# Diamondfan/CTC_pytorch

Measured on AMD Instinct MI355X. Metric: acoustic frames/sec/GPU (train) + utterances/sec beam-decode (`decode` object), TIMIT 4x320 BiLSTM, higher is better.
Workload: dtype f32 via bf16x3 split-operand MFMA (f32 accumulate); 1 GPU; cfg2: 4x320 BiLSTM + BN + Linear(62) + CTC, B=32/GPU, T=800, F=40, dropout 0.1, Adam; global_batch=32, seq_len=800, parallelism=dp1, full_length_utterances=True, sync_bn=False

## Files before the change

### ctc_pytorch_amd/_lib.py

```python
import ctypes
import glob
import os
import subprocess

import torch

_HERE = os.path.dirname(os.path.abspath(__file__))
_CSRC = os.path.join(_HERE, "csrc")
SO_PATH = os.environ.get("CTCN_LIBCTCN") or os.path.join(_HERE, "libctcn.so")
_lib = None

c_void_p, c_int, c_float, c_double, c_size_t, c_u64 = (ctypes.c_void_p, ctypes.c_int, ctypes.c_float,
                                                      ctypes.c_double, ctypes.c_size_t, ctypes.c_uint64)

P, I, F, D, Z, U = c_void_p, c_int, c_float, c_double, c_size_t, c_u64
_SIGS = {
    "ctcn_version": (I, []),
    "ctcn_last_error": (ctypes.c_char_p, []),
    "ctcn_device_cus": (I, []),
    "ctcn_device_xcds": (I, []),
    "ctcn_set_option": (I, [ctypes.c_char_p, I]),
    "ctcn_get_option": (I, [ctypes.c_char_p]),
    "ctcn_option_name": (ctypes.c_char_p, [I]),
    "ctcn_set_status_buffer": (I, [P]),
    "ctcn_gemm": (I, [I, I, I, I, I, P, I, P, I, P, I, F, I, P, Z, P]),
    "ctcn_transpose01": (I, [P, P, I, I, I, P]),
    "ctcn_copy_strided4": (I, [P, P, I, I, I, I, Z, Z, Z, Z, P]),
    "ctcn_relu_fwd": (I, [P, P, Z, P]),
    "ctcn_relu_bwd": (I, [P, P, P, Z, P]),
    "ctcn_maxpool2d_fwd": (I, [P, P, P, Z, I, I, I, I, P]),
    "ctcn_maxpool2d_bwd": (I, [P, P, P, Z, I, I, I, I, P]),
    "ctcn_rnn_scratch_bytes": (Z, [I, I, I, I]),
    "ctcn_rnn_fwd": (I, [I, I, I, I, I, I, P, P, P, P, P, P, P, P, I, P, Z, P]),
    "ctcn_rnn_fwd_dropout": (I, [I, I, I, I, I, I, P, P, P, P, P, P, P, P, P, F, U, U, I, P, Z, P]),
    "ctcn_rnn_bwd": (I, [I, I, I, I, I, I, P, P, P, P, P, P, P, P, P, P, P, P, P, P, F, I, P, P, Z, P]),
    "ctcn_rnn_bwd_dropout": (I, [I, I, I, I, I, I, P, P, P, P, P, P, P, P, P, P, P, P, P, P, F, I, P, P, Z, P, F, U, U, P]),
    "ctcn_rnn_bwd_weights": (I, [I, I, I, I, I, I, P, P, P, P, P, P, P, P, F, I, ctypes.c_uint, P, Z, P]),
    "ctcn_bn_ws_bytes": (Z, [I, I, I]),
    "ctcn_bn_fwd_train": (I, [P, P, P, P, P, P, P, P, I, I, I, F, F, I, P, Z, P, P]),
    "ctcn_bn_fwd_eval": (I, [P, P, P, P, P, P, I, I, I, F, I, P]),
    "ctcn_bn_fwd_sums": (I, [P, P, I, I, I, P, Z, P]),
    "ctcn_bn_fwd_finish": (I, [P, P, P, P, P, P, P, P, P, D, I, I, I, F, F, I, P, P]),
    "ctcn_bn_bwd_sums": (I, [P, P, P, P, P, P, I, I, I, I, P, Z, P]),
    "ctcn_bn_bwd_finish": (I, [P, P, P, P, P, P, P, P, P, P, P, D, I, I, I, I, F, P, Z, P]),
    "ctcn_bn_bwd": (I, [P, P, P, P, P, P, P, P, P, I, I, I, I, F, P, Z, P]),
    "ctcn_bn_fwd_train_dropout": (I, [P, P, P, P, P, P, P, P, I, I, I, F, F, I, P, Z, P, P, F, U, U]),
    "ctcn_bn_bwd_dropout": (I, [P, P, P, P, P, P, P, P, P, I, I, I, I, F, P, Z, P, F, U, U]),
    "ctcn_dropout": (I, [P, P, Z, F, U, U, P]),
    "ctcn_bn_masked_ws_bytes": (Z, [I, I, I]),
    "ctcn_mask_frames": (I, [P, P, P, I, I, I, I, I, P]),
    "ctcn_bn_fwd_train_masked": (I, [P, P, P, P, P, P, P, P, P, I, I, I, I, I, F, F, I, P, Z, P, P]),
    "ctcn_bn_fwd_eval_masked": (I, [P, P, P, P, P, P, P, I, I, I, I, I, F, I, P]),
    "ctcn_bn_bwd_masked": (I, [P, P, P, P, P, P, P, P, P, P, I, I, I, I, I, I, F, P, Z, P]),
    "ctcn_conv2d_ws_bytes": (Z, [I] * 11),
    "ctcn_conv2d_fwd": (I, [P, P, P, P] + [I] * 11 + [P]),
    "ctcn_conv2d_bwd": (I, [P, P, P, P, P, P] + [I] * 11 + [F, P, Z, P]),
    "ctcn_bctf_to_tbcf": (I, [P, P, I, I, I, I, P]),
    "ctcn_tbcf_to_bctf": (I, [P, P, I, I, I, I, P]),
    "ctcn_log_softmax_fwd": (I, [P, P, P, I, I, P]),
    "ctcn_log_softmax_bwd": (I, [P, P, P, I, I, P]),
    "ctcn_argmax": (I, [P, P, I, I, P]),
    "ctcn_rnn_fwd_ex": (I, [I, I, I, I, I, I, P, P, P, P, P, P, P, P, I, P, Z, P, P]),
    "ctcn_rnn_bwd_ex": (I, [I, I, I, I, I, I, P, P, P, P, P, P, P, P, P, P, P, P, P, P, F, I, P, P, Z, P, P]),
    "ctcn_ctc_fwd": (I, [P, P, P, P, P, P, I, I, I, I, P]),
    "ctcn_ctc_bwd": (I, [P, P, P, P, P, P, P, P, I, I, I, I, P]),
    "ctcn_ctc_fwd_both": (I, [P, P, P, P, P, P, P, I, I, I, I, P]),
    "ctcn_ctc_grad": (I, [P, P, P, P, P, P, P, P, P, I, I, I, I, P]),
    "ctcn_sum_f32": (I, [P, P, I, P]),
    "ctcn_ctc_fwd_ex": (I, [P, P, P, P, P, P, P, I, I, I, I, I, P]),
    "ctcn_ctc_grad_ex": (I, [P, P, P, P, P, P, P, P, I, I, I, I, P, I, I, I, I, P]),
    "ctcn_ctc_reduce": (I, [P, P, P, I, I, I, P]),
    "ctcn_ctc_pack_targets": (I, [P, ctypes.c_int64, P, P, I, I, P]),
    "ctcn_ctc_align_ws_bytes": (Z, [I, I, I]),
    "ctcn_ctc_align": (I, [P, P, P, P, P, P, P, P, P, P, I, I, I, I, I, P, Z, P]),
    "ctcn_adam_step": (I, [P, P, P, P, Z, F, F, F, F, F, I, P]),
    "ctcn_grad_norm_ws_bytes": (Z, [Z, I]),
    "ctcn_grad_norm": (I, [P, Z, I, P, I, P, P, P, I, P, Z, P]),
    "ctcn_clip_control": (I, [P, F, F, F, F, I, P]),
    "ctcn_adam_step_ex": (I, [P, P, P, P, Z, F, F, F, F, P, P]),
    "ctcn_scale_by_device_scalar": (I, [P, Z, P, P]),
    "ctcn_greedy_collapse": (I, [P, Z, Z, P, P, P, I, I, I, P]),
    "ctcn_edit_distance": (I, [P, P, P, P, P, I, I, I, I, P]),
    "ctcn_edit_ops_ws_bytes": (Z, [I, I, I]),
    "ctcn_edit_ops": (I, [P, P, P, P, P, I, P, P, P, P, I, I, I, I, P, Z, P]),
    "ctcn_step_stats": (I, [P, P, P, I, P, P, P]),
    "ctcn_comm_unique_id": (I, [P]),
    "ctcn_comm_init": (I, [P, I, I, ctypes.POINTER(ctypes.c_void_p)]),
    "ctcn_comm_allreduce_sum_f32": (I, [P, P, Z, P]),
    "ctcn_comm_destroy": (I, [P]),
    "ctcn_diag_squat": (I, [I, I, I, ctypes.c_uint, P]),
    "ctcn_diag_pipeline_chunks": (I, [I, I, I, I, I, I, I, I, ctypes.c_uint]),
    "ctcn_rnn_last_kernel": (ctypes.c_char_p, [I]),
    "ctcn_levenshtein": (ctypes.c_longlong, [P, ctypes.c_longlong, P, ctypes.c_longlong]),
    "ctcn_levenshtein_ops": (ctypes.c_longlong, [P, ctypes.c_longlong, P, ctypes.c_longlong, P, P]),
    "ctcn_join_tokens": (ctypes.c_longlong, [P, ctypes.c_longlong, P, I, P, P, P, I, I, P, ctypes.c_longlong, P]),
    "ctcn_beam_ws_bytes": (Z, [I, I, I, I]),
    "ctcn_beam_decode": (I, [P, I, P, P, D, I, I, P, P, P, P, I, I, I, P, Z, P]),
    "ctcn_beam_decode_nbest": (I, [P, I, P, P, D, I, I, I, P, P, P, P, P, I, I, I, P, Z, P]),
}


class RnnCall(ctypes.Structure):
    _fields_ = [("drop_p", ctypes.c_float), ("drop_seed", ctypes.c_uint64), ("drop_offset", ctypes.c_uint64), ("y_drop", ctypes.c_void_p),
                ("dy_tmp", ctypes.c_void_p), ("side_stream", ctypes.c_void_p), ("side_event", ctypes.c_void_p), ("side_ws", ctypes.c_void_p),
                ("side_ws_bytes", ctypes.c_size_t), ("xcd_allow", ctypes.c_uint), ("prelaunch_event", ctypes.c_void_p), ("status", ctypes.c_void_p),
                ("launched", ctypes.POINTER(ctypes.c_char_p))]


def sources():
    return sorted(glob.glob(os.path.join(_CSRC, "*.hip")))


def build(force=False, verbose=False):
    from concurrent.futures import ThreadPoolExecutor
    srcs = sources()
    hdrs = glob.glob(os.path.join(_CSRC, "*.h")) + [os.path.join(os.path.dirname(_HERE), "include", "ctcn.h")]
    hipcc = os.environ.get("HIPCC", "/opt/rocm/bin/hipcc")
    objdir = os.path.join(_CSRC, "_obj")
    os.makedirs(objdir, exist_ok=True)
    hdr_time = max(os.path.getmtime(h) for h in hdrs)
    flags = ["--offload-arch=gfx950", "-O3", "-std=c++17", "-fPIC"]
    jobs, objs = [], []
    for src in srcs:
        obj = os.path.join(objdir, os.path.basename(src)[:-4] + ".o")
        objs.append(obj)
        if force or not os.path.exists(obj) or os.path.getmtime(obj) < max(os.path.getmtime(src), hdr_time):
            jobs.append([hipcc] + flags + ["-c", src, "-o", obj])

    def run(cmd):
        if verbose:
            print(" ".join(cmd), flush=True)
        subprocess.check_call(cmd)

    if jobs:
        with ThreadPoolExecutor(max_workers=min(len(jobs), os.cpu_count() or 4)) as pool:
            list(pool.map(run, jobs))
    if jobs or not os.path.exists(SO_PATH) or any(os.path.getmtime(SO_PATH) < os.path.getmtime(o) for o in objs):
        run([hipcc, "--offload-arch=gfx950", "-fPIC", "-shared", "-o", SO_PATH] + objs)
    return SO_PATH


def lib():
    global _lib
    if _lib is None:
        if not os.path.exists(SO_PATH):
            raise RuntimeError(
                "ctc_pytorch_amd: %s is missing -- run `python -c 'import __graft_entry__ as g; g.build()'` "
                "(hipcc --offload-arch=gfx950). There is no CPU fallback." % SO_PATH)
        l = ctypes.CDLL(SO_PATH)
        for name, (res, args) in _SIGS.items():
            fn = getattr(l, name)
            fn.restype = res
            fn.argtypes = args
        _lib = l
        for var, opt in (("CTCN_RNN_PERSISTENT", b"rnn_persistent"), ("CTCN_HANDOFF", b"handoff"), ("CTCN_GEMM_BIG_TILES", b"gemm_big_tiles"), ("CTCN_BWD_SCATTER", b"bwd_scatter"), ("CTCN_HANDOFF_TAGS", b"handoff_tags"), ("CTCN_SIDE_SPLIT_WGS", b"side_split_wgs")):
            env = os.environ.get(var)
            if env is not None:
                l.ctcn_set_option(opt, int(env))
        for var, val in os.environ.items():
# ... 58 lines not shown
```

### ctc_pytorch_amd/csrc/common.h

```cpp
#pragma once
#include <hip/hip_runtime.h>
#include <stdarg.h>
#include <stdint.h>
#include <stdio.h>
#include <string.h>

#include "../../include/ctcn.h"

void ctcn_set_error(const char *fmt, ...);
int *ctcn_status_word(void);
int ctcn_opt_rnn_persistent(void);
int ctcn_transpose01_pair(const float *in0, const float *in1, float *out0, float *out1, int A, int B, int C, void *stream);
struct GemmPlanes {
  const float *A = nullptr; int lda = 0, M = 0, Ka = 0, transA = 0; void *ws_a = nullptr, *st_a = nullptr; bool a_valid = false;
  const float *B = nullptr; int ldb = 0, N = 0, Kb = 0, transB = 0, shift = 0; void *ws_b = nullptr, *st_b = nullptr; const void *bh = nullptr; bool b_valid = false;
  bool same_a = false, same_b = false;
};
int ctcn_gemm_on_xcds(int transA, int transB, int M, int N, int K, const float *A, int lda, const float *B, int ldb, float *C,
                      int ldc, float beta, int precision, void *ws, size_t ws_bytes, void *stream, unsigned xcd_allow, GemmPlanes *planes = nullptr);
int ctcn_gemm_shift_b(int M, int N, int K, const float *A, int lda, const float *B, int ldb, float *C, int ldc, float beta, int precision,
                      void *ws, size_t ws_bytes, void *stream, unsigned xcd_allow, int shift, GemmPlanes *planes = nullptr);
int ctcn_opt_handoff(void);
int ctcn_opt_poll_depth(void);
int ctcn_opt_bwd_scatter(void);
int ctcn_opt_handoff_tags(void);
int ctcn_opt_side_split_wgs(void);
int ctcn_opt_gemm_big_tiles(void);
int ctcn_opt_recurrence_only(void);

#define CTCN_REQUIRE(cond, ...)          \
  do {                                   \
    if (!(cond)) {                       \
      ctcn_set_error(__VA_ARGS__);       \
      return CTCN_EINVAL;                \
    }                                    \
  } while (0)

#define CTCN_HIP(expr)                                                                   \
  do {                                                                                   \
    hipError_t e__ = (expr);                                                             \
    if (e__ != hipSuccess) {                                                             \
      ctcn_set_error("%s:%d: %s -> %s", __FILE__, __LINE__, #expr, hipGetErrorString(e__)); \
      return CTCN_EHIP;                                                                  \
    }                                                                                    \
  } while (0)

#define CTCN_LAUNCH_CHECK() CTCN_HIP(hipGetLastError())

typedef float f32x4 __attribute__((ext_vector_type(4)));
typedef float f32x16 __attribute__((ext_vector_type(16)));
typedef short bf16x8 __attribute__((ext_vector_type(8)));
typedef unsigned int u32x4 __attribute__((ext_vector_type(4)));

static inline int ceil_div(int a, int b) { return (a + b - 1) / b; }
static inline size_t ceil_div_z(size_t a, size_t b) { return (a + b - 1) / b; }
static inline size_t align_up(size_t a, size_t b) { return (a + b - 1) / b * b; }

__device__ __forceinline__ float wave_max(float v) {
#pragma unroll
  for (int o = 32; o > 0; o >>= 1) v = fmaxf(v, __shfl_xor(v, o, 64));
  return v;
}
__device__ __forceinline__ float wave_sum(float v) {
#pragma unroll
  for (int o = 32; o > 0; o >>= 1) v += __shfl_xor(v, o, 64);
  return v;
}
__device__ __forceinline__ double wave_sum_d(double v) {
#pragma unroll
  for (int o = 32; o > 0; o >>= 1) v += __shfl_xor(v, o, 64);
  return v;
}
__device__ __forceinline__ void lds_barrier() { asm volatile("s_waitcnt lgkmcnt(0)\n\ts_barrier" ::: "memory"); }

__device__ __forceinline__ float sigmoidf_(float x) { return 1.0f / (1.0f + expf(-x)); }

__device__ __forceinline__ void philox_round(uint32_t (&c)[4], uint32_t (&k)[2]) {
  const uint32_t M0 = 0xD2511F53u, M1 = 0xCD9E8D57u;
  const uint32_t hi0 = __umulhi(M0, c[0]), lo0 = M0 * c[0];
  const uint32_t hi1 = __umulhi(M1, c[2]), lo1 = M1 * c[2];
  const uint32_t n0 = hi1 ^ c[1] ^ k[0], n1 = lo1, n2 = hi0 ^ c[3] ^ k[1], n3 = lo0;
  c[0] = n0; c[1] = n1; c[2] = n2; c[3] = n3;
  k[0] += 0x9E3779B9u; k[1] += 0xBB67AE85u;
}
__device__ __forceinline__ void philox4(uint64_t seed, uint64_t ctr, uint32_t (&out)[4]) {
  uint32_t c[4] = {(uint32_t)ctr, (uint32_t)(ctr >> 32), 0u, 0u};
  uint32_t k[2] = {(uint32_t)seed, (uint32_t)(seed >> 32)};
#pragma unroll
  for (int i = 0; i < 10; ++i) philox_round(c, k);
#pragma unroll
  for (int i = 0; i < 4; ++i) out[i] = c[i];
}

__device__ __forceinline__ unsigned short f2bf(float f) {
  return __builtin_bit_cast(unsigned short, (__bf16)f);
}
```

### ctc_pytorch_amd/csrc/core.hip

```cpp
#include "common.h"

static thread_local char g_err[512] = "";

void ctcn_set_error(const char *fmt, ...) {
  va_list ap;
  va_start(ap, fmt);
  vsnprintf(g_err, sizeof(g_err), fmt, ap);
  va_end(ap);
}

extern "C" int ctcn_version(void) { return 100; }
extern "C" const char *ctcn_last_error(void) { return g_err; }
extern "C" int ctcn_device_cus(void) {
  int dev = 0, n = 0;
  if (hipGetDevice(&dev) != hipSuccess) return -1;
  if (hipDeviceGetAttribute(&n, hipDeviceAttributeMultiprocessorCount, dev) != hipSuccess) return -1;
  return n;
}

static int g_opt_rnn_persistent = 1;
static int g_opt_handoff = 1;
static int g_opt_poll_depth = 2;
static int g_opt_recurrence_only = 0;
static int g_opt_bwd_scatter = 1;
static int g_opt_handoff_tags = 1;
static int g_opt_side_split_wgs = 8;
static int g_opt_gemm_big_tiles = 0;
static int g_opt_gemm_tile256 = 1;
static int g_opt_gemm_dbg = 0;
static int g_opt_gemm_a_inline = 1;
static int g_opt_conv_mfma = 1;
static int g_opt_gemm_pingpong = 1;
static int g_opt_rnn_mixed_slices = 0;
static int g_opt_rnn_fwd_tagged = 1;
static int g_opt_rnn_fused_dropout = 1;
static int g_opt_gemm_tn = 1;
static int g_opt_tag_poll_delay = 8;
static int g_opt_edit_wave = 1;
static int g_opt_bwd_item_gather = 1;
static int g_opt_bwd_poll_delay = -1;
static int g_opt_fwd_rsv_lds = 2;
static int g_opt_fwd_pipe_any_chunking = 0;
static int g_opt_fwd_pipe_min_input = 0;
static int g_opt_conv_dbg = 0;
static int g_opt_rnn_rsv_nt = 0;
static int g_opt_gemm_bf16_single = 0;
static int g_opt_xcd_interleave = 1;
static int g_opt_bn_rows4 = 1;
static int g_opt_tn_splits_force = 0;
static int g_opt_tn_splits_xcd = 1;
static int g_opt_beam_generic_threads = 0;
static int g_opt_beam_bitonic = 1;
static int g_opt_beam_cand_global = 0;
static int g_opt_beam_occ2 = 0;
static int g_opt_beam_fast = 1;
static int g_opt_rnn_slow_items = 0;
static int g_opt_rnn_slow_exchange = 0;
static int g_opt_xcd_interleave_force = 0;
static int *g_status_dev = nullptr;

struct OptionRow { const char *name; int *var; int (*norm)(int); };
static const OptionRow k_options[] = {
  {"rnn_persistent", &g_opt_rnn_persistent, [](int value) -> int { return value; }},
  {"handoff", &g_opt_handoff, [](int value) -> int { return value; }},
  {"poll_depth", &g_opt_poll_depth, [](int value) -> int { return value; }},
  {"rnn_recurrence_only", &g_opt_recurrence_only, [](int value) -> int { return value ? 1 : 0; }},
  {"bwd_scatter", &g_opt_bwd_scatter, [](int value) -> int { return value ? 1 : 0; }},
  {"handoff_tags", &g_opt_handoff_tags, [](int value) -> int { return value ? 1 : 0; }},
  {"side_split_wgs", &g_opt_side_split_wgs, [](int value) -> int { return value < 1 ? 1 : (value > 16 ? 16 : value); }},
  {"gemm_big_tiles", &g_opt_gemm_big_tiles, [](int value) -> int { return value ? 1 : 0; }},
  {"beam_fast", &g_opt_beam_fast, [](int value) -> int { return value ? 1 : 0; }},
  {"conv_dbg", &g_opt_conv_dbg, [](int value) -> int { return value & 7; }},
  {"rnn_rsv_nt", &g_opt_rnn_rsv_nt, [](int value) -> int { return value ? 1 : 0; }},
  {"tn_splits_xcd", &g_opt_tn_splits_xcd, [](int value) -> int { return value ? 1 : 0; }},
  {"xcd_interleave", &g_opt_xcd_interleave, [](int value) -> int { return value < 0 ? 0 : (value > 5 ? 5 : value); }},
  {"bn_rows4", &g_opt_bn_rows4, [](int value) -> int { return value ? 1 : 0; }},
  {"tn_splits_force", &g_opt_tn_splits_force, [](int value) -> int { return value < 0 ? 0 : value; }},
  {"gemm_bf16_single", &g_opt_gemm_bf16_single, [](int value) -> int { return value ? 1 : 0; }},
  {"beam_generic_threads", &g_opt_beam_generic_threads, [](int value) -> int { return (value == 256 || value == 512 || value == 1024) ? value : 0; }},
  {"beam_cand_global", &g_opt_beam_cand_global, [](int value) -> int { return value ? 1 : 0; }},
  {"beam_bitonic", &g_opt_beam_bitonic, [](int value) -> int { return value ? 1 : 0; }},
  {"beam_occ2", &g_opt_beam_occ2, [](int value) -> int { return value < 0 ? 0 : (value > 2 ? 2 : value); }},
  {"fwd_pipe_min_input", &g_opt_fwd_pipe_min_input, [](int value) -> int { return value < 0 ? 0 : value; }},
  {"fwd_pipe_any_chunking", &g_opt_fwd_pipe_any_chunking, [](int value) -> int { return value ? 1 : 0; }},
  {"fwd_rsv_lds", &g_opt_fwd_rsv_lds, [](int value) -> int { return value < 0 ? 0 : (value > 2 ? 2 : value); }},
  {"bwd_item_gather", &g_opt_bwd_item_gather, [](int value) -> int { return value < 0 ? 0 : (value > 2 ? 2 : value); }},
  {"bwd_poll_delay", &g_opt_bwd_poll_delay, [](int value) -> int { return value < 0 ? -1 : (value > 256 ? 256 : value); }},
  {"conv_mfma", &g_opt_conv_mfma, [](int value) -> int { return value ? 1 : 0; }},
  {"edit_wave", &g_opt_edit_wave, [](int value) -> int { return value ? 1 : 0; }},
  {"gemm_tn", &g_opt_gemm_tn, [](int value) -> int { return value != 0; }},
  {"rnn_fused_dropout", &g_opt_rnn_fused_dropout, [](int value) -> int { return value != 0; }},
  {"tag_poll_delay", &g_opt_tag_poll_delay, [](int value) -> int { return value < 0 ? 0 : (value > 64 ? 64 : value); }},
  {"rnn_fwd_tagged", &g_opt_rnn_fwd_tagged, [](int value) -> int { return value ? 1 : 0; }},
  {"rnn_mixed_slices", &g_opt_rnn_mixed_slices, [](int value) -> int { return value ? 1 : 0; }},
  {"gemm_pingpong", &g_opt_gemm_pingpong, [](int value) -> int { return value ? 1 : 0; }},
  {"gemm_a_inline", &g_opt_gemm_a_inline, [](int value) -> int { return value ? 1 : 0; }},
  {"gemm_dbg", &g_opt_gemm_dbg, [](int value) -> int { return value; }},
  {"gemm_tile256", &g_opt_gemm_tile256, [](int value) -> int { return value ? 1 : 0; }},
  {"xcd_interleave_force", &g_opt_xcd_interleave_force, [](int value) -> int { return value ? 1 : 0; }},
  {"rnn_slow_exchange", &g_opt_rnn_slow_exchange, [](int value) -> int { return value < 0 ? 0 : (value > 4096 ? 4096 : value); }},
  {"rnn_slow_items", &g_opt_rnn_slow_items, [](int value) -> int { return value < 0 ? 0 : (value > 4096 ? 4096 : value); }},
};
static const int k_noptions = (int)(sizeof(k_options) / sizeof(k_options[0]));
static const OptionRow *find_option(const char *name) {
  if (name)
    for (int i = 0; i < k_noptions; ++i)
      if (!strcmp(name, k_options[i].name)) return &k_options[i];
  return nullptr;
}
extern "C" int ctcn_set_option(const char *name, int value) {
  if (const OptionRow *o = find_option(name)) { *o->var = o->norm(value); return CTCN_OK; }
  ctcn_set_error("ctcn_set_option: unknown option %s", name ? name : "(null)");
  return CTCN_EINVAL;
}
extern "C" int ctcn_get_option(const char *name) {
  const OptionRow *o = find_option(name);
  return o ? *o->var : -1;
}
extern "C" const char *ctcn_option_name(int index) { return index >= 0 && index < k_noptions ? k_options[index].name : nullptr; }
extern "C" int ctcn_set_status_buffer(int *dev_word) { g_status_dev = dev_word; return CTCN_OK; }
int *ctcn_status_word(void) { return g_status_dev; }
int ctcn_opt_rnn_persistent(void) { return g_opt_rnn_persistent; }
int ctcn_opt_handoff(void) { return g_opt_handoff; }
int ctcn_opt_poll_depth(void) { return g_opt_poll_depth; }
int ctcn_opt_recurrence_only(void) { return g_opt_recurrence_only; }
int ctcn_opt_bwd_scatter(void) { return g_opt_bwd_scatter; }
int ctcn_opt_handoff_tags(void) { return g_opt_handoff_tags; }
int ctcn_opt_side_split_wgs(void) { return g_opt_side_split_wgs; }
int ctcn_opt_gemm_big_tiles(void) { return g_opt_gemm_big_tiles; }
// ... 1 lines not shown
```

### ctc_pytorch_amd/csrc/gemm.hip

```cpp
#include <algorithm>
#include <type_traits>

#include "common.h"

namespace {

constexpr int BM = 128, BN = 128, BK = 16, PAD = 4;

__device__ __forceinline__ void g2r_kc(const float *__restrict__ src, int ld, int r0, int R, int k0, int Kend,
                                       bool vec, int tid, float (&reg)[8]) {
#pragma unroll
  for (int j = 0; j < 2; ++j) {
    const int idx = tid + 256 * j;
    const int r = idx >> 2, kq = (idx & 3) * 4;
    const int gr = r0 + r, gk = k0 + kq;
    const float *p = src + (size_t)gr * ld + gk;
    if (vec && gr < R && gk + 3 < Kend) {
      const float4 v = *reinterpret_cast<const float4 *>(p);
      reg[4 * j + 0] = v.x; reg[4 * j + 1] = v.y; reg[4 * j + 2] = v.z; reg[4 * j + 3] = v.w;
    } else {
#pragma unroll
      for (int c = 0; c < 4; ++c) reg[4 * j + c] = (gr < R && gk + c < Kend) ? p[c] : 0.0f;
    }
  }
// ... 250 lines not shown
    else x_g2r_mc(B, ldb, n0, N, k0, kend, vecB, tid, rb);
  };
  if (kbeg < kend) { loadA(kbeg); loadB(kbeg); }
  for (int k0 = kbeg; k0 < kend; k0 += XBK) {
    __syncthreads();
    if (TA) x_r2s_mc(sAh, sAl, tid, ra); else x_r2s_kc(sAh, sAl, tid, ra);
    if (TB) x_r2s_kc(sBh, sBl, tid, rb); else x_r2s_mc(sBh, sBl, tid, rb);
    __syncthreads();
    if (k0 + XBK < kend) { loadA(k0 + XBK); loadB(k0 + XBK); }
    const int ml = lane & 31, kg = (lane >> 5) * 8;
#pragma unroll
    for (int ks = 0; ks < XBK; ks += 16) {
      bf16x8_t ah[2], al[2], bh[2], bl[2];
#pragma unroll
      for (int i = 0; i < 2; ++i) {
        ah[i] = *reinterpret_cast<const bf16x8_t *>(&sAh[wm * 64 + i * 32 + ml][ks + kg]);
        al[i] = *reinterpret_cast<const bf16x8_t *>(&sAl[wm * 64 + i * 32 + ml][ks + kg]);
        bh[i] = *reinterpret_cast<const bf16x8_t *>(&sBh[wn * 64 + i * 32 + ml][ks + kg]);
        bl[i] = *reinterpret_cast<const bf16x8_t *>(&sBl[wn * 64 + i * 32 + ml][ks + kg]);
      }
#pragma unroll
      for (int i = 0; i < 2; ++i)
#pragma unroll
        for (int j = 0; j < 2; ++j) {
          acc[i][j] = __builtin_amdgcn_mfma_f32_32x32x16_bf16(al[i], bh[j], acc[i][j], 0, 0, 0);
          acc[i][j] = __builtin_amdgcn_mfma_f32_32x32x16_bf16(ah[i], bl[j], acc[i][j], 0, 0, 0);
          acc[i][j] = __builtin_amdgcn_mfma_f32_32x32x16_bf16(ah[i], bh[j], acc[i][j], 0, 0, 0);
        }
    }
  }
  float *out = ws ? ws + (size_t)blockIdx.y * M * N : C;
  const int ldo = ws ? N : ldc;
#pragma unroll
  for (int i = 0; i < 2; ++i)
#pragma unroll
    for (int j = 0; j < 2; ++j) {
      const int col = n0 + wn * 64 + j * 32 + (lane & 31);
#pragma unroll
      for (int e = 0; e < 16; ++e) {
        const int row = m0 + wm * 64 + i * 32 + (e & 3) + 8 * (e >> 2) + 4 * (lane >> 5);
        if (row < M && col < N) {
          float v = acc[i][j][e];
          float *p = out + (size_t)row * ldo + col;
          if (!ws && beta != 0.0f) v += beta * *p;
          *p = v;
        }
      }
    }
}

constexpr int PBK = 64;

__global__ void split_rows_kernel(const float *__restrict__ src, int ld, int R, int C, int Cp, unsigned short *__restrict__ hi,
                                  unsigned short *__restrict__ lo) {
  const size_t total = (size_t)R * (Cp / 4);
  for (size_t i = blockIdx.x * (size_t)blockDim.x + threadIdx.x; i < total; i += (size_t)gridDim.x * blockDim.x) {
    const int r = (int)(i / (Cp / 4)), c = (int)(i - (size_t)r * (Cp / 4)) * 4;
    unsigned short h[4], l[4];
#pragma unroll
    for (int k = 0; k < 4; ++k) {
      const float v = (c + k < C) ? src[(size_t)r * ld + c + k] : 0.0f;
      split_bf16(v, h[k], l[k]);
    }
    *reinterpret_cast<uint2 *>(hi + (size_t)r * Cp + c) = make_uint2((unsigned)h[0] | ((unsigned)h[1] << 16), (unsigned)h[2] | ((unsigned)h[3] << 16));
    *reinterpret_cast<uint2 *>(lo + (size_t)r * Cp + c) = make_uint2((unsigned)l[0] | ((unsigned)l[1] << 16), (unsigned)l[2] | ((unsigned)l[3] << 16));
  }
}

__device__ __forceinline__ void split_transpose_tile(float (*t)[65], int bx, int by, const float *__restrict__ src, int ld, int R, int C, int Rp,
                                                     unsigned short *__restrict__ hi, unsigned short *__restrict__ lo, int shift) {
  const int r0 = by * 64, c0 = bx * 64;
  const int tid = threadIdx.x;
  const bool vec = c0 + 64 <= C && (ld & 3) == 0 && ((uintptr_t)src & 15) == 0;
  if (vec) {
#pragma unroll
    for (int j = 0; j < 4; ++j) {
      const int idx = tid + 256 * j, i = idx >> 4, c4 = idx & 15;
      const int r = r0 + i - shift;
      float4 v = make_float4(0.f, 0.f, 0.f, 0.f);
      if (r >= 0 && r < R && r0 + i < R) v = *reinterpret_cast<const float4 *>(src + (size_t)r * ld + c0 + 4 * c4);
      t[i][4 * c4 + 0] = v.x; t[i][4 * c4 + 1] = v.y; t[i][4 * c4 + 2] = v.z; t[i][4 * c4 + 3] = v.w;
    }
    __syncthreads();
#pragma unroll
    for (int j = 0; j < 2; ++j) {
      const int g = tid + 256 * j, c = g >> 3, ro = g & 7;
      unsigned hw[4], lw[4];
#pragma unroll
      for (int e = 0; e < 4; ++e) {
        unsigned short h0, l0, h1, l1;
        split_bf16(t[ro * 8 + 2 * e][c], h0, l0);
        split_bf16(t[ro * 8 + 2 * e + 1][c], h1, l1);
        hw[e] = (unsigned)h0 | ((unsigned)h1 << 16);
        lw[e] = (unsigned)l0 | ((unsigned)l1 << 16);
      }
      const size_t o = (size_t)(c0 + c) * Rp + r0 + ro * 8;
      *reinterpret_cast<uint4 *>(hi + o) = make_uint4(hw[0], hw[1], hw[2], hw[3]);
      *reinterpret_cast<uint4 *>(lo + o) = make_uint4(lw[0], lw[1], lw[2], lw[3]);
    }
    return;
  }
  const int tx = tid & 63, ty = tid >> 6;
  for (int i = ty; i < 64; i += 4) {
    const int r = r0 + i - shift, c = c0 + tx;
    t[i][tx] = (r >= 0 && r < R && r0 + i < R && c < C) ? src[(size_t)r * ld + c] : 0.0f;
  }
  __syncthreads();
  for (int i = ty; i < 64; i += 4) {
    const int c = c0 + i, r = r0 + tx;
    if (c < C && r < Rp) {
      unsigned short h, l;
      split_bf16(t[tx][i], h, l);
      hi[(size_t)c * Rp + r] = h;
      lo[(size_t)c * Rp + r] = l;
    }
  }
}

__global__ __launch_bounds__(256) void split_transpose_kernel(const float *__restrict__ src, int ld, int R, int C, int Rp,
                                                              unsigned short *__restrict__ hi, unsigned short *__restrict__ lo, int shift) {
  __shared__ float t[64][65];
  split_transpose_tile(t, blockIdx.x, blockIdx.y, src, ld, R, C, Rp, hi, lo, shift);
}
__global__ __launch_bounds__(256) void split_transpose_queue_kernel(const float *__restrict__ src, int ld, int R, int C, int Rp,
                                                                    unsigned short *__restrict__ hi, unsigned short *__restrict__ lo, int tiles_x,
                                                                    int tiles_y, unsigned xcd_allow, unsigned *__restrict__ queue, int shift) {
  __shared__ float t[64][65];
  __shared__ int s_item;
  unsigned x;
  asm volatile("s_getreg_b32 %0, hwreg(HW_REG_XCC_ID)" : "=s"(x));
  if (!((xcd_allow >> (x & 15)) & 1u)) return;
  for (;;) {
    if (threadIdx.x == 0) s_item = (int)atomicAdd(queue, 1u);
    __syncthreads();
    const int item = s_item;
    if (item >= tiles_x * tiles_y) return;
    split_transpose_tile(t, item % tiles_x, item / tiles_x, src, ld, R, C, Rp, hi, lo, shift);
    __syncthreads();
  }
}

__device__ __forceinline__ int pswz(int row, int kc) { return row * 128 + ((kc ^ ((row >> 1) & 7)) << 4); }

template <int TI, int TJ>
__device__ __forceinline__ void plane_tile(unsigned char *sm, int bid, int split, int M, int N, int Kp,
                                           const unsigned short *__restrict__ Ah, const unsigned short *__restrict__ Al,
                                           const unsigned short *__restrict__ Bh, const unsigned short *__restrict__ Bl,
                                           float *__restrict__ C, int ldc, float beta, int kchunk, float *__restrict__ ws, int tiles_n) {
  constexpr int TBM = 64 * TI, TBN = 64 * TJ;
  constexpr int CA = TBM * 8 / 256, CB = TBN * 8 / 256;
  unsigned char *sAh = sm, *sAl = sm + TBM * 128, *sBh = sm + 2 * TBM * 128, *sBl = sBh + TBN * 128;
  const int tid = threadIdx.x, lane = tid & 63, wave = tid >> 6;
  const int wm = wave >> 1, wn = wave & 1;
  const int tm = bid / tiles_n, tn = bid - tm * tiles_n;
  const int m0 = tm * TBM, n0 = tn * TBN;
  const int kbeg = split * kchunk;
  const int kend = min(Kp, kbeg + kchunk);

  f32x16 acc[TI][TJ];
#pragma unroll
  for (int i = 0; i < TI; ++i)
#pragma unroll
    for (int j = 0; j < TJ; ++j)
#pragma unroll
      for (int e = 0; e < 16; ++e) acc[i][j][e] = 0.0f;

  unsigned offA[CA], offB[CB];
#pragma unroll
  for (int j = 0; j < CA; ++j) offA[j] = (unsigned)min(m0 + ((tid + 256 * j) >> 3), M - 1) * (unsigned)Kp + ((tid + 256 * j) & 7) * 8;
#pragma unroll
  for (int j = 0; j < CB; ++j) offB[j] = (unsigned)min(n0 + ((tid + 256 * j) >> 3), N - 1) * (unsigned)Kp + ((tid + 256 * j) & 7) * 8;
  u32x4 pAh[CA], pAl[CA], pBh[CB], pBl[CB];
  auto gload = [&](int k0) {
#pragma unroll
    for (int j = 0; j < CA; ++j) {
      pAh[j] = *reinterpret_cast<const u32x4 *>(Ah + offA[j] + k0);
      pAl[j] = *reinterpret_cast<const u32x4 *>(Al + offA[j] + k0);
    }
#pragma unroll
    for (int j = 0; j < CB; ++j) {
      pBh[j] = *reinterpret_cast<const u32x4 *>(Bh + offB[j] + k0);
      pBl[j] = *reinterpret_cast<const u32x4 *>(Bl + offB[j] + k0);
    }
  };
  if (kbeg < kend) gload(kbeg);
  for (int k0 = kbeg; k0 < kend; k0 += PBK) {
    __syncthreads();
#pragma unroll
    for (int j = 0; j < CA; ++j) {
      const int so = pswz((tid + 256 * j) >> 3, (tid + 256 * j) & 7);
// ... 1145 lines not shown
        for (int u = 0; u < 8; ++u) { s.x += v[u].x; s.y += v[u].y; s.z += v[u].z; s.w += v[u].w; }
      }
      for (; z < splits; ++z) { const float4 v = w4[(size_t)z * total4 + i]; s.x += v.x; s.y += v.y; s.z += v.z; s.w += v.w; }
      const unsigned m = i / n4, n = (i - m * n4) << 2;
      float4 *p = reinterpret_cast<float4 *>(C + (size_t)m * ldc + n);
      if (beta != 0.0f) { const float4 o = *p; s.x += beta * o.x; s.y += beta * o.y; s.z += beta * o.z; s.w += beta * o.w; }
      *p = s;
    }
    return;
  }
  for (size_t i = blockIdx.x * (size_t)blockDim.x + threadIdx.x; i < total; i += (size_t)gridDim.x * blockDim.x) {
    float s = 0.0f;
    int z = 0;
    for (; z + 8 <= splits; z += 8) {
      float v[8];
#pragma unroll
      for (int u = 0; u < 8; ++u) v[u] = ws[(size_t)(z + u) * total + i];
#pragma unroll
      for (int u = 0; u < 8; ++u) s += v[u];
    }
    for (; z < splits; ++z) s += ws[(size_t)z * total + i];
    const size_t m = i / N, n = i - m * N;
    float *p = C + m * ldc + n;
    if (beta != 0.0f) s += beta * *p;
    *p = s;
  }
}

__global__ void transpose01_kernel(const float *__restrict__ in, float *__restrict__ out, int A, int B, int C) {
  const size_t total = (size_t)A * B * C;
  for (size_t i = blockIdx.x * (size_t)blockDim.x + threadIdx.x; i < total; i += (size_t)gridDim.x * blockDim.x) {
    const int c = i % C;
    const size_t ab = i / C;
    const int a = ab % A;
    const int b = ab / A;
    out[i] = in[((size_t)a * B + b) * C + c];
  }
}

}

static bool tn_eligible(int transA, int transB, int M, int N, int K, const float *A, int lda, const float *B, int ldb, int precision, const void *ws,
                        size_t ws_bytes) {
  return precision == 1 && transA && !transB && ws && ws_bytes >= 1024 && ctcn_get_option("gemm_tn") != 0 && M >= 128 && N >= 32 && K >= 1024 &&
         M % 4 == 0 && N % 4 == 0 && lda % 4 == 0 && ldb % 4 == 0 && ((uintptr_t)A & 15) == 0 && ((uintptr_t)B & 15) == 0 &&
         lda < (1 << 24) && ldb < (1 << 24);
}
static int gemm_core(int transA, int transB, int M, int N, int K, const float *A, int lda, const float *B, int ldb, float *C,
                     int ldc, float beta, int precision, void *ws, size_t ws_bytes, void *stream, unsigned xcd_allow, GemmPlanes *planes, int b_shift) {
  GemmPlanes scratch_planes;
  GemmPlanes &pl = planes ? *planes : scratch_planes;
  const bool want_same_a = pl.same_a, want_same_b = pl.same_b;
  pl.same_a = pl.same_b = false;
  CTCN_REQUIRE(precision == 0 || precision == 1, "ctcn_gemm: precision %d (0 = f32 MFMA, 1 = bf16x3 split MFMA)", precision);
  CTCN_REQUIRE(M > 0 && N > 0 && K >= 0, "ctcn_gemm: bad dims M=%d N=%d K=%d", M, N, K);
  CTCN_REQUIRE(A && B && C, "ctcn_gemm: null pointer");
  CTCN_REQUIRE(lda >= (transA ? M : K) && ldb >= (transB ? K : N) && ldc >= N, "ctcn_gemm: leading dim too small");
  CTCN_REQUIRE(!ws || (uintptr_t)ws % 16 == 0, "ctcn_gemm: the workspace must be 16-byte aligned");
  hipStream_t st = (hipStream_t)stream;
  const int tiles_m = ceil_div(M, BM), tiles_n = ceil_div(N, BN);
  const int nt = tiles_m * tiles_n;
  int splits = 1;
  if (nt < 256 && K >= 512 && ws && ws_bytes >= (size_t)2 * M * N * sizeof(float)) {
    splits = ceil_div(512, nt);
    splits = min(splits, K / 256);
    splits = min(splits, (int)(ws_bytes / ((size_t)M * N * sizeof(float))));
    if (splits < 2) splits = 1;
  }
  int kchunk = K;
  if (splits > 1) {
    kchunk = ceil_div(ceil_div(K, splits), XBK) * XBK;
    splits = ceil_div(K, kchunk);
  }
  if (tn_eligible(transA, transB, M, N, K, A, lda, B, ldb, precision, ws, ws_bytes) && b_shift == 0) {
    pl.a_valid = false; pl.b_valid = false;
    const int wnt = ceil_div(N, 256) * 256 == ceil_div(N, 128) * 128 ? 2 : 1;
    unsigned *queue = (unsigned *)((char *)ws + ((ws_bytes - 256) & ~(size_t)255));
    int tn_cus = 256;
    if (xcd_allow && ctcn_get_option("tn_splits_xcd") != 0) {
      const int nx = std::max(1, std::min(ctcn_device_xcds(), 16));
      tn_cus = std::max(ctcn_device_cus() / nx * __builtin_popcount(xcd_allow & ((1u << nx) - 1u)), 32);
    }
    const int tsplits = tn_splits(M, N, K, wnt, ws_bytes - 512, tn_cus);
    return wnt == 2 ? launch_tn<2>(st, M, N, K, A, lda, B, ldb, C, ldc, beta, tsplits, (float *)ws, xcd_allow, queue)
                    : launch_tn<1>(st, M, N, K, A, lda, B, ldb, C, ldc, beta, tsplits, (float *)ws, xcd_allow, queue);
  }
  if (precision == 1 && K >= 64 && ws) {
    const int Kp = ceil_div(K, PBK) * PBK;
    const size_t a_el = (size_t)M * Kp, b_el = (size_t)N * Kp;
    const size_t plane_bytes = align_up(2 * (a_el + b_el) * sizeof(unsigned short), 256);
    if (ws_bytes >= plane_bytes + 1024) {
      unsigned short *ah = (unsigned short *)ws, *al = ah + a_el, *bh = al + a_el, *bl = bh + b_el;
      float *part = (float *)((char *)ws + plane_bytes);
      unsigned *queue = (unsigned *)((char *)ws + ((ws_bytes - 256) & ~(size_t)255));
      const size_t part_bytes = ws_bytes - plane_bytes - 512;
      if (xcd_allow) CTCN_HIP(hipMemsetAsync(queue, 0, 16, st));
      int nq = 0;
      auto split = [&](const float *src, int ld, bool contraction_major, int rows, unsigned short *hi, unsigned short *lo, int shift) {
        if (!contraction_major) {
          const size_t total = (size_t)rows * (Kp / 4);
          hipLaunchKernelGGL(split_rows_kernel, dim3((unsigned)std::min((size_t)8192, ceil_div_z(total, 256))), dim3(256), 0, st, src, ld, rows, K, Kp, hi, lo);
        } else {
          if (xcd_allow)
            hipLaunchKernelGGL(split_transpose_queue_kernel, dim3(ctcn_opt_side_split_wgs() * ctcn_device_cus()), dim3(256), 0, st, src, ld, K, rows, Kp, hi, lo, ceil_div(rows, 64),
                               ceil_div(Kp, 64), xcd_allow, queue + (++nq), shift);
          else
            hipLaunchKernelGGL(split_transpose_kernel, dim3(ceil_div(rows, 64), ceil_div(Kp, 64)), dim3(256), 0, st, src, ld, K, rows, Kp, hi, lo, shift);
        }
      };
      const bool same_a = want_same_a && pl.a_valid && pl.A == A && pl.lda == lda && pl.M == M && pl.Ka == K && pl.transA == transA && pl.ws_a == ws &&
                          pl.st_a == (void *)st;
      const bool same_b = want_same_b && pl.b_valid && pl.B == B && pl.ldb == ldb && pl.N == N && pl.Kb == K && pl.transB == transB && pl.shift == b_shift &&
                          pl.ws_b == ws && pl.st_b == (void *)st && pl.bh == (const void *)bh;
      pl.B = B; pl.ldb = ldb; pl.N = N; pl.Kb = K; pl.transB = transB; pl.shift = b_shift; pl.ws_b = ws;
      pl.st_b = (void *)st; pl.bh = (const void *)bh; pl.b_valid = true;
      const int wnt256 = (N % 256 == 0 || (N > 512 && ceil_div(N, 256) * 256 - N <= N / 8)) ? 2 : 1;
      const bool use256 = !xcd_allow && ctcn_get_option("gemm_tile256") != 0 && M >= 1024 && N >= 96 &&
                          (long)ceil_div(M, 256) * ceil_div(N, 128 * wnt256) * 4 >= (long)ctcn_device_cus() * 3;
      const bool a_inline = use256 && !same_a && !transA && ctcn_get_option("gemm_a_inline") != 0 && K >= 32 && K % 4 == 0 && lda % 4 == 0 &&
                            ((uintptr_t)A & 15) == 0 && ceil_div(N, 128 * wnt256) <= 5;
      if (a_inline) {
        pl.a_valid = false;
        if (!same_b) split(B, ldb, transB == 0, N, bh, bl, b_shift);
        CTCN_LAUNCH_CHECK();
        const int lrc = wnt256 == 2 ? launch_planes256_af32<2>(st, M, N, K, Kp, A, lda, bh, bl, C, ldc, beta)
                                    : launch_planes256_af32<1>(st, M, N, K, Kp, A, lda, bh, bl, C, ldc, beta);
        if (lrc) return lrc;
        CTCN_LAUNCH_CHECK();
        return CTCN_OK;
      }
      if (!same_a) split(A, lda, transA != 0, M, ah, al, 0);
      pl.A = A; pl.lda = lda; pl.M = M; pl.Ka = K; pl.transA = transA; pl.ws_a = ws; pl.st_a = (void *)st;
      pl.a_valid = true;
      if (!same_b) split(B, ldb, transB == 0, N, bh, bl, b_shift);
      CTCN_LAUNCH_CHECK();
      int shape = 0, ptm = tiles_m, ptn = tiles_n;
      {
        const long t22 = (long)tiles_m * tiles_n * 128 * 128;
        const int m42 = ceil_div(M, 256), n42 = ceil_div(N, 128), m24 = ceil_div(M, 128), n24 = ceil_div(N, 256);
        const long t42 = (long)m42 * n42 * 256 * 128, t24 = (long)m24 * n24 * 128 * 256;
        const int min_tiles = ctcn_device_cus();
        const bool ok42 = m42 * n42 >= min_tiles && t42 <= t22 + t22 / 32, ok24 = m24 * n24 >= min_tiles && t24 <= t22 + t22 / 32;
        if (ctcn_opt_gemm_big_tiles() && (ok42 || ok24)) {
          if (ok24 && (!ok42 || t24 <= t42)) { shape = 2; ptm = m24; ptn = n24; }
          else { shape = 1; ptm = m42; ptn = n42; }
        }
      }
      if (use256) {
        const int lrc256 = wnt256 == 2 ? launch_planes256<2>(st, M, N, Kp, ah, al, bh, bl, C, ldc, beta)
                                       : launch_planes256<1>(st, M, N, Kp, ah, al, bh, bl, C, ldc, beta);
        if (lrc256) return lrc256;
        CTCN_LAUNCH_CHECK();
        return CTCN_OK;
      }
      if (xcd_allow && ctcn_get_option("gemm_tile256") != 0 && ctcn_get_option("gemm_pingpong") != 0 && M >= 1024 && N >= 96) {
        const int cus = ctcn_device_cus() / std::max(1, std::min(ctcn_device_xcds(), 16)) * __builtin_popcount(xcd_allow);
        const int t256 = ceil_div(M, 256) * ceil_div(N, 128 * wnt256), rounds = ceil_div(t256, std::max(cus, 1));
        if (cus > 0 && t256 * 4 >= rounds * cus * 3) {
          const int lrc = wnt256 == 2 ? launch_planes256_queue<2>(st, M, N, Kp, ah, al, bh, bl, C, ldc, beta, xcd_allow, queue)
                                      : launch_planes256_queue<1>(st, M, N, Kp, ah, al, bh, bl, C, ldc, beta, xcd_allow, queue);
          if (lrc) return lrc;
          CTCN_LAUNCH_CHECK();
          return CTCN_OK;
        }
      }
      const int pnt = ptm * ptn;
      int psplits = 1;
      if (pnt < 256 && Kp >= 1024 && part_bytes >= (size_t)2 * M * N * sizeof(float)) {
        psplits = std::min(std::min(ceil_div(512, pnt), Kp / 512), (int)(part_bytes / ((size_t)M * N * sizeof(float))));
        if (psplits < 2) psplits = 1;
      }
      int pchunk = Kp;
      if (psplits > 1) {
        pchunk = ceil_div(ceil_div(Kp, psplits), PBK) * PBK;
        psplits = ceil_div(Kp, pchunk);
      }
      float *pp = psplits > 1 ? part : (float *)nullptr;
      int lrc;
      if (shape == 1) lrc = launch_planes<4, 2>(xcd_allow != 0, pnt, psplits, st, M, N, Kp, ah, al, bh, bl, C, ldc, beta, pchunk, pp, ptm, ptn, xcd_allow, queue);
      else if (shape == 2) lrc = launch_planes<2, 4>(xcd_allow != 0, pnt, psplits, st, M, N, Kp, ah, al, bh, bl, C, ldc, beta, pchunk, pp, ptm, ptn, xcd_allow, queue);
      else lrc = launch_planes<2, 2>(xcd_allow != 0, pnt, psplits, st, M, N, Kp, ah, al, bh, bl, C, ldc, beta, pchunk, pp, ptm, ptn, xcd_allow, queue);
      if (lrc) return lrc;
      CTCN_LAUNCH_CHECK();
      if (psplits > 1) {
        const size_t total = (size_t)M * N;
        hipLaunchKernelGGL(splitk_reduce_kernel, dim3((int)std::min((size_t)2048, ceil_div_z(total, 256))), dim3(256), 0, st, (const float *)part, C, M,
                           N, ldc, psplits, beta);
        CTCN_LAUNCH_CHECK();
      }
      return CTCN_OK;
    }
  }
  pl.a_valid = false; pl.b_valid = false;
  const bool vecA = ((uintptr_t)A % 16 == 0) && (lda % 4 == 0);
  const bool vecB = ((uintptr_t)B % 16 == 0) && (ldb % 4 == 0);
  float *wsp = splits > 1 ? (float *)ws : nullptr;
  dim3 grid(nt, splits), block(256);
#define LAUNCH(KERN, TA, TB)                                                                             \
  hipLaunchKernelGGL((KERN<TA, TB>), grid, block, 0, st, M, N, K, A, lda, B, ldb, C, ldc, beta, kchunk, wsp, \
                     tiles_m, tiles_n, vecA, vecB)
  if (precision == 0 && xcd_allow && ws && ws_bytes >= (size_t)splits * M * N * sizeof(float) * (splits > 1 ? 1 : 0) + 512) {
    unsigned *queue = (unsigned *)((char *)ws + ((ws_bytes - 256) & ~(size_t)255));
    CTCN_HIP(hipMemsetAsync(queue, 0, 4, st));
    const dim3 qgrid(2 * ctcn_device_cus());
#define QLAUNCH(TA, TB)                                                                                              \
  hipLaunchKernelGGL((gemm_f32_queue_kernel<TA, TB>), qgrid, block, 0, st, M, N, K, A, lda, B, ldb, C, ldc, beta, kchunk, wsp, \
                     tiles_m, tiles_n, vecA, vecB, splits, xcd_allow, queue)
    if (transA) { if (transB) QLAUNCH(true, true); else QLAUNCH(true, false); }
    else        { if (transB) QLAUNCH(false, true); else QLAUNCH(false, false); }
#undef QLAUNCH
  } else if (precision == 0) {
    if (transA) { if (transB) LAUNCH(gemm_f32_kernel, true, true); else LAUNCH(gemm_f32_kernel, true, false); }
    else        { if (transB) LAUNCH(gemm_f32_kernel, false, true); else LAUNCH(gemm_f32_kernel, false, false); }
  } else {
    if (transA) { if (transB) LAUNCH(gemm_bf16x3_kernel, true, true); else LAUNCH(gemm_bf16x3_kernel, true, false); }
    else        { if (transB) LAUNCH(gemm_bf16x3_kernel, false, true); else LAUNCH(gemm_bf16x3_kernel, false, false); }
  }
#undef LAUNCH
  CTCN_LAUNCH_CHECK();
  if (splits > 1) {
    const size_t total = (size_t)M * N;
    const int blocks = (int)min((size_t)2048, ceil_div_z(total, 256));
    hipLaunchKernelGGL(splitk_reduce_kernel, dim3(blocks), dim3(256), 0, st, (const float *)ws, C, M, N, ldc, splits, beta);
    CTCN_LAUNCH_CHECK();
  }
  return CTCN_OK;
}

int ctcn_gemm_on_xcds(int transA, int transB, int M, int N, int K, const float *A, int lda, const float *B, int ldb, float *C,
                      int ldc, float beta, int precision, void *ws, size_t ws_bytes, void *stream, unsigned xcd_allow, GemmPlanes *planes) {
  return gemm_core(transA, transB, M, N, K, A, lda, B, ldb, C, ldc, beta, precision, ws, ws_bytes, stream, xcd_allow, planes, 0);
}

int ctcn_gemm_shift_b(int M, int N, int K, const float *A, int lda, const float *B, int ldb, float *C, int ldc, float beta, int precision,
                      void *ws, size_t ws_bytes, void *stream, unsigned xcd_allow, int shift, GemmPlanes *planes) {
  const int as = shift < 0 ? -shift : shift;
  CTCN_REQUIRE(as < K, "ctcn_gemm_shift_b: |shift| %d >= K %d", as, K);
  const int Kp = ceil_div(K, PBK) * PBK;
  const size_t plane_bytes = align_up(2 * ((size_t)M * Kp + (size_t)N * Kp) * sizeof(unsigned short), 256);
  const bool plane = precision == 1 && K >= 64 && ws && ws_bytes >= plane_bytes + 1024 &&
                     !tn_eligible(1, 0, M, N, K - as, A, lda, B, ldb, precision, ws, ws_bytes);
  if (!plane) {
    if (planes) planes->same_a = false;
    const float *A2 = shift > 0 ? A + (size_t)as * lda : A, *B2 = shift < 0 ? B + (size_t)as * ldb : B;
    return gemm_core(1, 0, M, N, K - as, A2, lda, B2, ldb, C, ldc, beta, precision, ws, ws_bytes, stream, xcd_allow, planes, 0);
  }
  return gemm_core(1, 0, M, N, K, A, lda, B, ldb, C, ldc, beta, precision, ws, ws_bytes, stream, xcd_allow, planes, shift);
}

extern "C" int ctcn_gemm(int transA, int transB, int M, int N, int K, const float *A, int lda, const float *B,
                         int ldb, float *C, int ldc, float beta, int precision, void *ws, size_t ws_bytes,
                         void *stream) {
  return gemm_core(transA, transB, M, N, K, A, lda, B, ldb, C, ldc, beta, precision, ws, ws_bytes, stream, 0u, nullptr, 0);
}

__global__ void transpose01_pair_kernel(const float *__restrict__ in0, const float *__restrict__ in1, float *__restrict__ out0, float *__restrict__ out1,
                                        int A, int B, int C) {
  const float *in = blockIdx.y ? in1 : in0;
  float *out = blockIdx.y ? out1 : out0;
  const size_t total = (size_t)A * B * C;
  for (size_t i = blockIdx.x * (size_t)blockDim.x + threadIdx.x; i < total; i += (size_t)gridDim.x * blockDim.x) {
    const int c = i % C;
    const size_t ab = i / C;
    const int a = ab % A;
    const int b = ab / A;
    out[i] = in[((size_t)a * B + b) * C + c];
  }
}
__global__ __launch_bounds__(256) void transpose2d_pair_kernel(const float *__restrict__ in0, const float *__restrict__ in1, float *__restrict__ out0,
                                                               float *__restrict__ out1, int A, int B) {
  __shared__ float tile[32][33];
  const float *in = blockIdx.z ? in1 : in0;
  float *out = blockIdx.z ? out1 : out0;
  const int tx = threadIdx.x & 31, ty = threadIdx.x >> 5;
  const int b0 = blockIdx.x * 32, a0 = blockIdx.y * 32;
#pragma unroll
  for (int k = 0; k < 4; ++k) {
    const int a = a0 + ty + 8 * k, b = b0 + tx;
    if (a < A && b < B) tile[ty + 8 * k][tx] = in[(size_t)a * B + b];
  }
  __syncthreads();
#pragma unroll
  for (int k = 0; k < 4; ++k) {
    const int b = b0 + ty + 8 * k, a = a0 + tx;
    if (a < A && b < B) out[(size_t)b * A + a] = tile[tx][ty + 8 * k];
  }
}
int ctcn_transpose01_pair(const float *in0, const float *in1, float *out0, float *out1, int A, int B, int C, void *stream) {
  CTCN_REQUIRE(in0 && in1 && out0 && out1 && A > 0 && B > 0 && C > 0, "ctcn_transpose01_pair: bad args");
  if (C == 1) {
    hipLaunchKernelGGL(transpose2d_pair_kernel, dim3(ceil_div(B, 32), ceil_div(A, 32), 2), dim3(256), 0, (hipStream_t)stream, in0, in1, out0, out1, A, B);
    CTCN_LAUNCH_CHECK();
    return CTCN_OK;
  }
  const size_t total = (size_t)A * B * C;
  const int blocks = (int)min((size_t)4096, ceil_div_z(total, 256));
  hipLaunchKernelGGL(transpose01_pair_kernel, dim3(blocks, 2), dim3(256), 0, (hipStream_t)stream, in0, in1, out0, out1, A, B, C);
  CTCN_LAUNCH_CHECK();
  return CTCN_OK;
}
// ... 10 lines not shown
```

### ctc_pytorch_amd/csrc/norm.hip

```cpp
#include <algorithm>

#include "common.h"

namespace {

struct Pair { double a, b; };

struct StatVal {
  const float *x;
  __device__ __forceinline__ Pair operator()(size_t idx, int) const {
    const double v = x[idx];
    return {v, v * v};
  }
  struct Quad { f32x4 x; };
  __device__ __forceinline__ Quad load4(size_t idx) const { return {*reinterpret_cast<const f32x4 *>(x + idx)}; }
  __device__ __forceinline__ void add4(const Quad &q, int, double &a, double &b) const {
#pragma unroll
    for (int e = 0; e < 4; ++e) { const double v = q.x[e]; a += v; b += v * v; }
  }
  __host__ __device__ __forceinline__ bool aligned16() const { return ((uintptr_t)x & 15) == 0; }
  struct ColK {};
  static constexpr int ROWS_IN_FLIGHT = 8;
  __device__ __forceinline__ ColK colk(int) const { return {}; }
  __device__ __forceinline__ void cols4(const Quad &q, const ColK &, double (&a)[4], double (&b)[4]) const {
#pragma unroll
    for (int e = 0; e < 4; ++e) { const double v = q.x[e]; a[e] += v; b[e] += v * v; }
  }
};
struct DropSpec { float p, scale; uint64_t seed, offset; const float *gamma, *beta; };
__device__ __forceinline__ float bn_value(float x, float m, float rs, float g, float b) { return fmaf((x - m) * rs, g, b); }
__device__ __forceinline__ bool drop_keep(uint32_t word, float p) { return (word >> 8) * (1.0f / 16777216.0f) >= p; }
__device__ __forceinline__ float bn_dx_value(float g, float xh, float ga, float rs, float s0, float s1, float inv_n) {
  return ga * rs * fmaf(-xh, s1 * inv_n, fmaf(-s0, inv_n, g));
}

struct BwdVal {
  const float *x, *y, *dy, *mean, *rstd;
  int relu;
  DropSpec d;
  __device__ __forceinline__ Pair operator()(size_t idx, int c) const {
    float g = dy[idx];
    if (d.p > 0.0f) {
      uint32_t r[4];
      philox4(d.seed, d.offset + (idx >> 2), r);
      g = drop_keep(r[idx & 3], d.p) ? g * d.scale : 0.0f;
      if (relu && !(bn_value(x[idx], mean[c], rstd[c], d.gamma[c], d.beta[c]) > 0.0f)) g = 0.0f;
    } else if (relu && !(y[idx] > 0.0f)) g = 0.0f;
    const float xh = (x[idx] - mean[c]) * rstd[c];
    return {(double)g, (double)g * (double)xh};
  }
  struct Quad { f32x4 x, y, dy; };
  __device__ __forceinline__ Quad load4(size_t idx) const {
    Quad q;
    q.x = *reinterpret_cast<const f32x4 *>(x + idx);
    q.dy = *reinterpret_cast<const f32x4 *>(dy + idx);
    if (d.p > 0.0f) {
      uint32_t r[4];
      philox4(d.seed, d.offset + (idx >> 2), r);
#pragma unroll
      for (int e = 0; e < 4; ++e) q.dy[e] = drop_keep(r[e], d.p) ? q.dy[e] * d.scale : 0.0f;
      q.y = q.x;
    } else q.y = relu ? *reinterpret_cast<const f32x4 *>(y + idx) : q.x;
    return q;
  }
  __device__ __forceinline__ void add4(const Quad &q, int c, double &a, double &b) const {
    const float m = mean[c], rs = rstd[c];
    const bool rec = d.p > 0.0f;
    const float ga = rec ? d.gamma[c] : 0.0f, be = rec ? d.beta[c] : 0.0f;
#pragma unroll
    for (int e = 0; e < 4; ++e) {
      float g = q.dy[e];
      const float yv = rec ? bn_value(q.x[e], m, rs, ga, be) : q.y[e];
      if (relu && !(yv > 0.0f)) g = 0.0f;
      const float xh = (q.x[e] - m) * rs;
      a += (double)g; b += (double)g * (double)xh;
    }
  }
  __host__ __device__ __forceinline__ bool aligned16() const {
    return (((uintptr_t)x | (uintptr_t)dy | ((relu && !(d.p > 0.0f)) ? (uintptr_t)y : 0)) & 15) == 0;
  }
  struct ColK { float m[4], rs[4], ga[4], be[4]; };
  static constexpr int ROWS_IN_FLIGHT = 4;
  __device__ __forceinline__ ColK colk(int c0) const {
// ... 527 lines not shown

template <class G>
int bn_backward(const char *who, const G &g, bool geom, const float *x, const float *y, const float *dy, const float *gamma, const float *save_mean,
                const float *save_rstd, float *dx, float *dgamma, float *dbeta, int outer, int C, int inner, int relu, float beta_acc, void *ws,
                size_t ws_bytes, void *stream, const DropSpec *drop) {
  CTCN_REQUIRE(x && dy && gamma && save_mean && save_rstd && dx && ws && (!drop || drop->beta), "%s: null pointer", who);
  CTCN_REQUIRE(!relu || y || drop, "%s: y required for the fused relu mask", who);
  CTCN_REQUIRE(geom, "%s: bad dims%s", who, G::kAll ? "" : " / geometry");
  CTCN_REQUIRE(!drop || (drop->p > 0.0f && drop->p < 1.0f), "%s: p=%f outside (0,1)", who, (double)drop->p);
  if (ws_bytes < ws_need<G>(outer, C, inner)) { ctcn_set_error("%s: workspace too small", who); return CTCN_EWORKSPACE; }
  hipStream_t st = (hipStream_t)stream;
  double *part = (double *)ws;
  float *sums = (float *)((char *)ws + ws_part_bytes(outer, C, inner));
  int nchunks = 0;
  launch_reduce(BwdVal{x, y, dy, save_mean, save_rstd, relu, drop ? *drop : k_no_drop}, g, outer, C, inner, part, &nchunks, st);
  CTCN_LAUNCH_CHECK();
  hipLaunchKernelGGL(bn_finalize_bwd_kernel<G>, dim3(ceil_div(C, 4)), dim3(256), 0, st, part, nchunks, C, g, dgamma, dbeta, sums, beta_acc);
  CTCN_LAUNCH_CHECK();
  const size_t total = (size_t)outer * C * inner;
  if constexpr (G::kAll) {
    if (drop) {
      hipLaunchKernelGGL(bn_dx_drop_kernel, dim3(stream_blocks((total + 3) / 4)), dim3(256), 0, st, x, dy, gamma, drop->beta, save_mean, save_rstd, sums, dx,
                         total, C, inner, g.inv_n_, relu, *drop);
      CTCN_LAUNCH_CHECK();
      return CTCN_OK;
    }
  }
  launch_bn_dx(st, g, x, y, dy, gamma, save_mean, save_rstd, sums, dx, total, C, inner, relu);
  CTCN_LAUNCH_CHECK();
  return CTCN_OK;
}

DropSpec drop_spec(float p, uint64_t seed, uint64_t offset, const float *gamma, const float *beta) { return {p, 1.0f / (1.0f - p), seed, offset, gamma, beta}; }

}

extern "C" size_t ctcn_bn_ws_bytes(int outer, int C, int inner) {
  if (!dims_ok(outer, C, inner)) return 0;
  return ws_part_bytes(outer, C, inner) + (size_t)2 * C * sizeof(float);
}

extern "C" size_t ctcn_bn_masked_ws_bytes(int outer, int C, int inner) {
  const size_t n = ctcn_bn_ws_bytes(outer, C, inner);
  return n ? n + 256 : 0;
}

extern "C" int ctcn_bn_fwd_train(const float *x, float *y, const float *gamma, const float *beta, float *running_mean,
                                 float *running_var, float *save_mean, float *save_rstd, int outer, int C, int inner,
                                 float eps, float momentum, int relu, void *ws, size_t ws_bytes, void *stream, long long *num_batches_tracked) {
  return bn_forward("ctcn_bn_fwd_train", all_frames((double)outer * inner), dims_ok(outer, C, inner), x, y, gamma, beta, running_mean, running_var,
                    save_mean, save_rstd, outer, C, inner, eps, momentum, relu, ws, ws_bytes, stream, num_batches_tracked, nullptr);
}

extern "C" int ctcn_bn_fwd_train_dropout(const float *x, float *y_drop, const float *gamma, const float *beta, float *running_mean, float *running_var,
                                         float *save_mean, float *save_rstd, int outer, int C, int inner, float eps, float momentum, int relu, void *ws,
                                         size_t ws_bytes, void *stream, long long *num_batches_tracked, float p, uint64_t seed, uint64_t offset) {
  const DropSpec d = drop_spec(p, seed, offset, gamma, beta);
  return bn_forward("ctcn_bn_fwd_train_dropout", all_frames((double)outer * inner), dims_ok(outer, C, inner), x, y_drop, gamma, beta, running_mean,
                    running_var, save_mean, save_rstd, outer, C, inner, eps, momentum, relu, ws, ws_bytes, stream, num_batches_tracked, &d);
}

extern "C" int ctcn_bn_fwd_train_masked(const float *x, float *y, const float *gamma, const float *beta, float *running_mean, float *running_var,
                                        float *save_mean, float *save_rstd, const int *lens, int batch, int frame, int outer, int C, int inner,
                                        float eps, float momentum, int relu, void *ws, size_t ws_bytes, void *stream, long long *num_batches_tracked) {
  Frames g = {};
  const bool geom = geom_ok(outer, C, inner, lens, batch, frame, &g);
  return bn_forward("ctcn_bn_fwd_train_masked", g, geom, x, y, gamma, beta, running_mean, running_var, save_mean, save_rstd, outer, C, inner, eps,
                    momentum, relu, ws, ws_bytes, stream, num_batches_tracked, nullptr);
}

extern "C" int ctcn_bn_bwd(const float *x, const float *y, const float *dy, const float *gamma, const float *save_mean,
                           const float *save_rstd, float *dx, float *dgamma, float *dbeta, int outer, int C, int inner,
                           int relu, float beta_acc, void *ws, size_t ws_bytes, void *stream) {
  return bn_backward("ctcn_bn_bwd", all_frames((double)outer * inner), dims_ok(outer, C, inner), x, y, dy, gamma, save_mean, save_rstd, dx, dgamma, dbeta,
                     outer, C, inner, relu, beta_acc, ws, ws_bytes, stream, nullptr);
}

extern "C" int ctcn_bn_bwd_dropout(const float *x, const float *dy_drop, const float *gamma, const float *beta, const float *save_mean,
                                   const float *save_rstd, float *dx, float *dgamma, float *dbeta, int outer, int C, int inner, int relu, float beta_acc,
                                   void *ws, size_t ws_bytes, void *stream, float p, uint64_t seed, uint64_t offset) {
  const DropSpec d = drop_spec(p, seed, offset, gamma, beta);
  return bn_backward("ctcn_bn_bwd_dropout", all_frames((double)outer * inner), dims_ok(outer, C, inner), x, nullptr, dy_drop, gamma, save_mean, save_rstd,
                     dx, dgamma, dbeta, outer, C, inner, relu, beta_acc, ws, ws_bytes, stream, &d);
}

extern "C" int ctcn_bn_bwd_masked(const float *x, const float *y, const float *dy, const float *gamma, const float *save_mean, const float *save_rstd,
                                  float *dx, float *dgamma, float *dbeta, const int *lens, int batch, int frame, int outer, int C, int inner, int relu,
                                  float beta_acc, void *ws, size_t ws_bytes, void *stream) {
  Frames g = {};
  const bool geom = geom_ok(outer, C, inner, lens, batch, frame, &g);
  return bn_backward("ctcn_bn_bwd_masked", g, geom, x, y, dy, gamma, save_mean, save_rstd, dx, dgamma, dbeta, outer, C, inner, relu, beta_acc, ws,
                     ws_bytes, stream, nullptr);
}

extern "C" int ctcn_bn_fwd_eval(const float *x, float *y, const float *gamma, const float *beta, const float *running_mean,
                                const float *running_var, int outer, int C, int inner, float eps, int relu, void *stream) {
  CTCN_REQUIRE(x && y && gamma && beta && running_mean && running_var, "ctcn_bn_fwd_eval: null pointer");
  CTCN_REQUIRE(dims_ok(outer, C, inner), "ctcn_bn_fwd_eval: bad dims");
  launch_bn_apply((hipStream_t)stream, all_frames((double)outer * inner), x, y, gamma, beta, running_mean, running_var, eps, 1, (size_t)outer * C * inner, C,
                  inner, relu);
  CTCN_LAUNCH_CHECK();
  return CTCN_OK;
}

extern "C" int ctcn_bn_fwd_eval_masked(const float *x, float *y, const float *gamma, const float *beta, const float *running_mean,
                                       const float *running_var, const int *lens, int batch, int frame, int outer, int C, int inner, float eps,
// ... 80 lines not shown
```

### ctc_pytorch_amd/csrc/rnn.hip

```cpp
#include <algorithm>
#include <stdlib.h>

#include <atomic>

#include "common.h"
#include <type_traits>

namespace {

__device__ __forceinline__ float act_sigmoid(float x) { return __builtin_amdgcn_rcpf(1.0f + __builtin_amdgcn_exp2f(-1.4426950408889634f * x)); }
__device__ __forceinline__ float act_tanh(float x) {
  const float e = __builtin_amdgcn_exp2f(-2.8853900817779268f * fabsf(x));
  return copysignf((1.0f - e) * __builtin_amdgcn_rcpf(1.0f + e), x);
}

typedef __bf16 bf16x8_t __attribute__((ext_vector_type(8)));
union Bf16Pack { u32x4 u; bf16x8_t v; };
__device__ __forceinline__ void split8(const f32x4 &a, const f32x4 &b, bf16x8_t &hi, bf16x8_t &lo) {
  unsigned h[8], l[8];
#pragma unroll
  for (int e = 0; e < 8; ++e) {
    const float x = e < 4 ? a[e] : b[e - 4];
    h[e] = f2bf(x);
    l[e] = f2bf(x - __uint_as_float(h[e] << 16));
// ... 2149 lines not shown
  CTCN_REQUIRE(x && w_ih0 && w_hh0 && y && gates && (dirs == 1 || (w_ih1 && w_hh1)), "ctcn_rnn_fwd: null pointer");
  CTCN_REQUIRE(cell == CTCN_CELL_TANH || aux, "ctcn_rnn_fwd: aux reserve required for LSTM/GRU");
  CTCN_REQUIRE(((uintptr_t)w_hh0 % 16 == 0) && ((uintptr_t)y % 16 == 0) && (dirs == 1 || (uintptr_t)w_hh1 % 16 == 0),
               "ctcn_rnn_fwd: w_hh / y must be 16-byte aligned");
  CTCN_REQUIRE((uintptr_t)ws % 16 == 0, "ctcn_rnn_fwd: the workspace must be 16-byte aligned (hand-off tiles)");
  return CTCN_OK;
}

static void fwd_begin(FwdCall &c, const float *w_hh0, const float *w_hh1, float *y, float *aux) {
  c.G = gates_of(c.cell); c.GH = c.G * c.H; c.nbt = ceil_div(c.B, 16); c.groups = c.dirs * c.nbt;
  RnnArgs &a = c.a;
  a.cell = c.cell; a.T = c.T; a.B = c.B; a.H = c.H; a.D = c.dirs; a.G = c.G; a.step = 0;
  a.w0 = w_hh0; a.w1 = w_hh1; a.y = y; a.gates = c.gates; a.aux = aux; a.dy = nullptr; a.state = nullptr;
  c.status = c.call.status ? c.call.status : ctcn_status_word();
  c.fits32 = (size_t)c.T * c.B * c.dirs * c.GH * sizeof(float) < ((size_t)1 << 32);
  c.nxd = ctcn_opt_handoff() ? ctcn_device_xcds() : 1;
  c.cus = ctcn_device_cus();
  c.recurrence_only = ctcn_opt_recurrence_only() != 0;
  c.persistent = ctcn_opt_rnn_persistent() != 0;
  c.tagged = ctcn_get_option("rnn_fwd_tagged") != 0;
  c.mixed_slices = ctcn_get_option("rnn_mixed_slices") != 0;
  c.any_chunking = ctcn_get_option("fwd_pipe_any_chunking") != 0;
  c.fused_dropout = ctcn_get_option("rnn_fused_dropout") != 0;
  c.min_input = ctcn_get_option("fwd_pipe_min_input");
  c.rsv_lds = ctcn_get_option("fwd_rsv_lds");
  c.tag_poll_delay = ctcn_get_option("tag_poll_delay");
  c.slow_items = ctcn_get_option("rnn_slow_items");
  c.slow_exchange = ctcn_get_option("rnn_slow_exchange");
}

static bool tagged_gather_applies(const FwdCall &c) {
  return c.persistent && c.T > 1 && c.fits32 && c.tagged && c.precision == 1 && c.cell != CTCN_CELL_TANH && c.H % 32 == 0 && c.H / 32 <= 24 && c.nxd > 1;
}

struct PipePlan { bool on, fits; int nchunk, chunk_T; };
static PipePlan decide_pipeline(const FwdCall &c) {
  const ctcn_rnn_call &ov = c.call;
  PipePlan p;
  p.nchunk = ov.xcd_allow && c.nxd > 1 ? plan_projection_pipeline(c.T, c.B, c.I, c.H, c.dirs, c.G, c.nxd, c.cus, ov.xcd_allow, c.min_input) : 0;
  p.fits = p.nchunk > 0;
  if (!p.fits) p.nchunk = 8;
  p.chunk_T = ceil_div(c.T, p.nchunk);
  const int T = c.T, NCHUNK = p.nchunk, chunk_T = p.chunk_T;
  p.on = !c.recurrence_only && ov.side_stream && ov.side_event && ov.side_ws && ov.xcd_allow != 0 && c.dirs == 2 && c.w_ih[1] == c.w_ih[0] + (size_t)c.GH * c.I &&
         tagged_gather_applies(c) && T >= 4 * NCHUNK && chunk_T * (NCHUNK - 1) < T &&
         (p.fits || c.any_chunking) &&
         T - chunk_T * (NCHUNK - 1) >= 2 &&
         ceil_div(c.groups, c.nxd) * (c.H / 16) + 4 <= c.cus / c.nxd;
  return p;
}

static int project_chunk(const FwdCall &c, const PipePlan &p, int chunk, void *ws, size_t ws_bytes, void *stream, unsigned allow, GemmPlanes &pl) {
  const int t0 = chunk * p.chunk_T, t1 = std::min(c.T, t0 + p.chunk_T), N2 = 2 * c.GH;
  return ctcn_gemm_on_xcds(0, 1, (t1 - t0) * c.B, N2, c.I, c.x + (size_t)t0 * c.B * c.I, c.I, c.w_ih[0], c.I, c.gates + (size_t)t0 * c.B * N2, N2, 0.0f, c.precision,
                           ws, ws_bytes, stream, allow, &pl);
}

static int project_first_pair(const FwdCall &c, const PipePlan &p, GemmPlanes &pl_main) {
  int rc = project_chunk(c, p, 0, c.ws, c.ws_bytes, c.stream, 0, pl_main);
  pl_main.same_b = true;
  if (!rc) rc = project_chunk(c, p, p.nchunk - 1, c.ws, c.ws_bytes, c.stream, 0, pl_main);
  return rc;
}

static int project_all(const FwdCall &c) {
  const int TB = c.T * c.B;
  GemmPlanes pl;
  if (c.dirs == 2) {
    StackedWih s;
    if (int rc = stack_w_ih(c.w_ih[0], c.w_ih[1], c.GH, c.I, c.ws, c.ws_bytes, c.st(), s)) return rc;
    if (s.w) return ctcn_gemm_on_xcds(0, 1, TB, 2 * c.GH, c.I, c.x, c.I, s.w, c.I, c.gates, 2 * c.GH, 0.0f, c.precision, s.ws, s.ws_bytes, c.stream, 0u, &pl);
  }
  for (int d = 0; d < c.dirs; ++d)
    if (int rc = ctcn_gemm_on_xcds(0, 1, TB, c.GH, c.I, c.x, c.I, c.w_ih[d], c.I, c.gates + (size_t)d * c.GH, c.dirs * c.GH, 0.0f, c.precision, c.ws, c.ws_bytes,
                                   c.stream, 0u, &pl))
      return rc;
  return CTCN_OK;
}

static int project_side_pairs(const FwdCall &c, const PipePlan &p, unsigned *chunk_ready) {
  const ctcn_rnn_call &ov = c.call;
  hipStream_t sd = (hipStream_t)ov.side_stream;
  GemmPlanes pl_side;
  CTCN_HIP(hipStreamWaitEvent(sd, (hipEvent_t)ov.side_event, 0));
  for (int pr = 1; pr < p.nchunk / 2; ++pr) {
    if (pr > 1) pl_side.same_b = true;
    int rc = project_chunk(c, p, pr, ov.side_ws, ov.side_ws_bytes, ov.side_stream, ov.xcd_allow, pl_side);
    pl_side.same_b = true;
    if (!rc) rc = project_chunk(c, p, p.nchunk - 1 - pr, ov.side_ws, ov.side_ws_bytes, ov.side_stream, ov.xcd_allow, pl_side);
    if (rc) {
      hipLaunchKernelGGL(set_counter_kernel, dim3(1), dim3(1), 0, sd, chunk_ready, (unsigned)p.nchunk);
      return rc;
    }
    hipLaunchKernelGGL(set_counter_kernel, dim3(1), dim3(1), 0, sd, chunk_ready, (unsigned)pr);
  }
  CTCN_LAUNCH_CHECK();
  return CTCN_OK;
}

static int fwd_try_tagged(const FwdCall &c, const PipePlan &p, GemmPlanes &pl_main, bool &drop_pending, bool &launched) {
  const int H = c.H, nsl = H / 16, wpx = ceil_div(c.groups, c.nxd) * nsl;
  hipStream_t st = c.st();
  Handoff h;
  if (carve_handoff(c.ws, c.ws_bytes, align_up((size_t)2 * c.dirs * c.nbt * (H / 32) * 2048, 256), 512, h)) {
    PersistArgs pa = persist_args(c.a, h, c.status, {1, c.nxd, c.groups, nsl, c.nbt, 16, wpx});
    const bool rsv = (c.rsv_lds == 1 || (c.rsv_lds == 2 && nsl > 24)) &&
                     ((uintptr_t)c.a.gates | (uintptr_t)c.a.aux | (uintptr_t)c.a.y | (uintptr_t)(drop_pending ? c.call.y_drop : nullptr)) % 16 == 0;
    pa.poll_depth = 1 | (rsv ? 256 : 0); pa.tagmode = 1; pa.poll_delay = c.tag_poll_delay;
    pa.chunk_T = p.on ? p.chunk_T : 0; pa.nchunk = p.nchunk; pa.chunk_ready = pa.flags;
    const bool fuse_drop = drop_pending && c.fused_dropout;
    if (fuse_drop) {
      pa.ydrop = c.call.y_drop; pa.drop_p = c.call.drop_p; pa.drop_scale = 1.0f / (1.0f - c.call.drop_p);
      pa.drop_seed = c.call.drop_seed; pa.drop_off = c.call.drop_offset;
    }
    pa.slow = c.slow_items; pa.slow_x = c.slow_exchange;
    CTCN_HIP(clear_handoff(h, true, st));
    if (p.on) CTCN_HIP(hipEventRecord((hipEvent_t)c.call.side_event, st));
    launched = launch_fwd_tagged(ceil_div(H / 32, 12), xcd_local_grid(c.nxd, wpx), st, pa, wpx);
    if (launched) {
      CTCN_LAUNCH_CHECK();
// ... 71 lines not shown
                        const float *w_hh0, const float *w_ih1, const float *w_hh1, float *y, float *gates,
                        float *aux, int precision, void *ws, size_t ws_bytes, void *stream, const ctcn_rnn_call &call, bool &drop_pending) {
  if (int rc = fwd_validate(cell, T, B, I, H, dirs, x, w_ih0, w_hh0, w_ih1, w_hh1, y, gates, aux, ws)) return rc;
  FwdCall c = {cell, T, B, I, H, dirs, precision, x, {w_ih0, w_ih1}, gates, ws, ws_bytes, stream, call};
  fwd_begin(c, w_hh0, w_hh1, y, aux);
  const PipePlan plan = decide_pipeline(c);
  if (getenv("CTCN_LOG_PIPE")) fprintf(stderr, "libctcn: rnn_fwd T=%d B=%d I=%d H=%d: projection pipeline %s (chunks %d x %d steps, fits=%d)\n", T, B, I, H, plan.on ? "ON" : "off", plan.nchunk, plan.chunk_T, (int)plan.fits);
  GemmPlanes pl_main;
  if (!c.recurrence_only)
    if (int rc = plan.on ? project_first_pair(c, plan, pl_main) : project_all(c)) return rc;
  if (c.persistent && T > 1 && !c.fits32) {
    log_fallback("ctcn_rnn_fwd", T, B, H, dirs, "a reserve tensor of 4 GB or more");
  } else if (c.persistent && T > 1) {
    bool launched = false;
    const char *why = nullptr;
    if (tagged_gather_applies(c))
      if (int rc = fwd_try_tagged(c, plan, pl_main, drop_pending, launched)) return rc;
    if (!launched)
      if (int rc = fwd_try_persist(c, launched, why)) return rc;
    if (launched) return CTCN_OK;
    log_fallback("ctcn_rnn_fwd", T, B, H, dirs, why);
  }
  return fwd_per_timestep(c);
}

extern "C" int ctcn_dropout(const float *x, float *y, size_t n, float p, uint64_t seed, uint64_t offset, void *stream);
extern "C" int ctcn_rnn_fwd_ex(int cell, int T, int B, int I, int H, int dirs, const float *x, const float *w_ih0, const float *w_hh0,
                               const float *w_ih1, const float *w_hh1, float *y, float *gates, float *aux, int precision, void *ws, size_t ws_bytes,
                               void *stream, const ctcn_rnn_call *call) {
  const ctcn_rnn_call &c = call ? *call : k_plain_call;
  CTCN_REQUIRE(!c.y_drop || (c.drop_p >= 0.0f && c.drop_p < 1.0f), "ctcn_rnn_fwd_ex: dropout p=%f outside [0,1)", (double)c.drop_p);
  bool drop_pending = c.y_drop != nullptr;
  const int rc = rnn_fwd_impl(cell, T, B, I, H, dirs, x, w_ih0, w_hh0, w_ih1, w_hh1, y, gates, aux, precision, ws, ws_bytes, stream, c, drop_pending);
  if (rc) return rc;
  return drop_pending ? ctcn_dropout(y, c.y_drop, (size_t)T * B * dirs * H, c.drop_p, c.drop_seed, c.drop_offset, stream) : CTCN_OK;
}
extern "C" int ctcn_rnn_fwd(int cell, int T, int B, int I, int H, int dirs, const float *x, const float *w_ih0,
                            const float *w_hh0, const float *w_ih1, const float *w_hh1, float *y, float *gates,
                            float *aux, int precision, void *ws, size_t ws_bytes, void *stream) {
  return ctcn_rnn_fwd_ex(cell, T, B, I, H, dirs, x, w_ih0, w_hh0, w_ih1, w_hh1, y, gates, aux, precision, ws, ws_bytes, stream, nullptr);
}
extern "C" int ctcn_rnn_fwd_dropout(int cell, int T, int B, int I, int H, int dirs, const float *x, const float *w_ih0, const float *w_hh0,
                                    const float *w_ih1, const float *w_hh1, float *y, float *gates, float *aux, float *y_drop, float p, uint64_t seed,
                                    uint64_t offset, int precision, void *ws, size_t ws_bytes, void *stream) {
  CTCN_REQUIRE(y_drop && p >= 0.0f && p < 1.0f, "ctcn_rnn_fwd_dropout: y_drop NULL or p=%f outside [0,1)", (double)p);
  ctcn_rnn_call c = {};
  c.y_drop = y_drop; c.drop_p = p; c.drop_seed = seed; c.drop_offset = offset;
  return ctcn_rnn_fwd_ex(cell, T, B, I, H, dirs, x, w_ih0, w_hh0, w_ih1, w_hh1, y, gates, aux, precision, ws, ws_bytes, stream, &c);
}

static int rnn_bwd_gemms(int cell, int T, int B, int I, int H, int dirs, const float *x, const float *w_ih0, const float *w_ih1,
                         const float *y, const float *gates, const float *aux, float *dx, float *dw_ih0, float *dw_hh0, float *dw_ih1,
                         float *dw_hh1, float beta_w, int precision, bool weights, unsigned xcd_allow, void *ws, size_t ws_bytes,
                         void *stream) {
  const int G = gates_of(cell), GH = G * H, TB = T * B;
  const float *w_ih[2] = {w_ih0, w_ih1};
  float *dw_ih[2] = {dw_ih0, dw_ih1};
  float *dw_hh[2] = {dw_hh0, dw_hh1};
  GemmPlanes pl;
  bool dx_done = false;
  if (dx && dirs == 2) {
    StackedWih s;
    if (int rc = stack_w_ih(w_ih0, w_ih1, GH, I, ws, ws_bytes, (hipStream_t)stream, s)) return rc;
    if (s.w) {
      if (int rc = ctcn_gemm_on_xcds(0, 0, TB, I, 2 * GH, gates, 2 * GH, s.w, I, dx, I, 0.0f, precision, s.ws, s.ws_bytes, stream, xcd_allow)) return rc;
      dx_done = true;
    }
  }
  for (int d = 0; d < dirs; ++d) {
    const float *da = gates + (size_t)d * GH;
    const int ldg = dirs * GH;
    int rc;
    if (dx && !dx_done) {
      rc = ctcn_gemm_on_xcds(0, 0, TB, I, GH, da, ldg, w_ih[d], I, dx, I, d == 0 ? 0.0f : 1.0f, precision, ws, ws_bytes, stream, xcd_allow);
      if (rc) return rc;
    }
    if (!weights || !dw_ih[d]) continue;
    rc = ctcn_gemm_on_xcds(1, 0, GH, I, TB, da, ldg, x, I, dw_ih[d], I, beta_w, precision, ws, ws_bytes, stream, xcd_allow, &pl);
    if (rc) return rc;
    const int Kh = (T - 1) * B;
    if (Kh <= 0) {
      if (beta_w == 0.0f) CTCN_HIP(hipMemsetAsync(dw_hh[d], 0, (size_t)GH * H * sizeof(float), (hipStream_t)stream));
      continue;
    }
    const size_t offA = d == 0 ? (size_t)B : 0, offY = d == 0 ? 0 : (size_t)B;
    const float *yh = y + (size_t)d * H + offY * dirs * H;
    if (cell == CTCN_CELL_GRU) {
      rc = ctcn_gemm_on_xcds(1, 0, 2 * H, H, Kh, da + offA * ldg, ldg, yh, dirs * H, dw_hh[d], H, beta_w, precision, ws, ws_bytes, stream, xcd_allow);
      if (rc) return rc;
      const float *dn = aux + (size_t)d * H + offA * dirs * H;
      rc = ctcn_gemm_on_xcds(1, 0, H, H, Kh, dn, dirs * H, yh, dirs * H, dw_hh[d] + (size_t)2 * H * H, H, beta_w, precision, ws, ws_bytes, stream, xcd_allow);
      if (rc) return rc;
    } else {
      pl.same_a = true;
      rc = ctcn_gemm_shift_b(GH, H, TB, da, ldg, y + (size_t)d * H, dirs * H, dw_hh[d], H, beta_w, precision, ws, ws_bytes, stream, xcd_allow,
                             d == 0 ? B : -B, &pl);
      if (rc) return rc;
    }
  }
  return CTCN_OK;
}

struct BwdCall {
  int cell, T, B, I, H, dirs, precision;
  const float *dy;
  void *ws; size_t ws_bytes;
  void *stream;
  const ctcn_rnn_call &call;
// ... 100 lines not shown
  CTCN_REQUIRE(!call.dy_tmp || (call.drop_p >= 0.0f && call.drop_p < 1.0f), "ctcn_rnn_bwd_ex: dropout p=%f outside [0,1)", (double)call.drop_p);
  CTCN_REQUIRE(cell >= 0 && cell <= 2, "ctcn_rnn_bwd: unknown cell %d", cell);
  CTCN_REQUIRE(T > 0 && B > 0 && I > 0 && H > 0 && (dirs == 1 || dirs == 2), "ctcn_rnn_bwd: bad dims");
  if (H % 4 != 0) { ctcn_set_error("ctcn_rnn_bwd: hidden size %d must be a multiple of 4", H); return CTCN_EUNSUPPORTED; }
  CTCN_REQUIRE(x && w_ih0 && w_hh0 && y && gates && dy && scratch, "ctcn_rnn_bwd: null pointer");
  CTCN_REQUIRE((dw_ih0 != nullptr) == (dw_hh0 != nullptr), "ctcn_rnn_bwd: dw_ih0 / dw_hh0 must both be given or both be NULL (weights deferred to ctcn_rnn_bwd_weights)");
  CTCN_REQUIRE(dirs == 1 || (w_ih1 && w_hh1 && (!dw_ih0 || (dw_ih1 && dw_hh1))), "ctcn_rnn_bwd: null pointer (reverse direction)");
  CTCN_REQUIRE(cell == CTCN_CELL_TANH || aux, "ctcn_rnn_bwd: aux reserve required for LSTM/GRU");
  CTCN_REQUIRE((uintptr_t)gates % 16 == 0 && (uintptr_t)scratch % 16 == 0 && (cell == CTCN_CELL_TANH || (uintptr_t)aux % 16 == 0),
               "ctcn_rnn_bwd: gates / aux / scratch must be 16-byte aligned");
  CTCN_REQUIRE((uintptr_t)ws % 16 == 0, "ctcn_rnn_bwd: the workspace must be 16-byte aligned (hand-off tiles)");
  BwdCall c = {cell, T, B, I, H, dirs, precision, dy, ws, ws_bytes, stream, call};
  c.G = gates_of(cell); c.GH = c.G * H;
  const int GH = c.GH;
  c.grid = dim3(ceil_div(H, 16), dirs, ceil_div(B, 16));
  c.status = call.status ? call.status : ctcn_status_word();
  c.fits32 = (size_t)T * B * dirs * GH * sizeof(float) < ((size_t)1 << 32);
  c.dy_dropped = call.dy_tmp == nullptr;
  c.prelaunch_event = call.prelaunch_event;
  c.nxd = ctcn_opt_handoff() ? ctcn_device_xcds() : 1;
  c.persistent = ctcn_opt_rnn_persistent() != 0; c.bwd_scatter = ctcn_opt_bwd_scatter() != 0; c.fused_dropout = ctcn_get_option("rnn_fused_dropout") != 0;
  c.handoff_tags = ctcn_opt_handoff_tags(); c.item_gather = ctcn_get_option("bwd_item_gather"); c.rsv_nt = ctcn_get_option("rnn_rsv_nt");
  c.poll_delay = ctcn_get_option("bwd_poll_delay"); c.slow_items = ctcn_get_option("rnn_slow_items"); c.slow_exchange = ctcn_get_option("rnn_slow_exchange");

  float *whhT = (float *)scratch;
  if (dirs == 2) {
    if (int rc = ctcn_transpose01_pair(w_hh0, w_hh1, whhT, whhT + (size_t)GH * H, GH, H, 1, stream)) return rc;
  } else if (int rc = ctcn_transpose01(w_hh0, whhT, GH, H, 1, stream)) {
    return rc;
  }
  RnnArgs &a = c.a;
  a.cell = cell; a.T = T; a.B = B; a.H = H; a.D = dirs; a.G = c.G; a.step = 0;
  a.w0 = whhT; a.w1 = whhT + (size_t)GH * H; a.y = const_cast<float *>(y); a.gates = gates; a.aux = aux; a.dy = dy;
  a.state = (float *)((char *)scratch + align_up((size_t)dirs * GH * H * sizeof(float), 256));

  bool done = false;
  if (c.persistent && T > 1) {
    const BwdPlan p = bwd_choose_formulation(c);
    Handoff h;
    if (p.feasible && carve_handoff(ws, ws_bytes, p.hx_bytes, p.fl_bytes, h))
      for (int mode = c.nxd > 1 ? 1 : 0; mode >= 0 && !done; --mode)
        if (int rc = bwd_try_persistent(c, p, h, mode, done)) return rc;
    if (!done)
      log_fallback("ctcn_rnn_bwd", T, B, H, dirs, !c.fits32 ? "a reserve tensor of 4 GB or more"
                                                       : (ceil_div(GH, 256) > 8 ? "gate width G*H above 2048" : "not co-resident / workspace too small"));
  }
  record_prelaunch(c);
  if (!done)
    if (int rc = bwd_per_timestep(c)) return rc;
  CTCN_LAUNCH_CHECK();

  if (ctcn_opt_recurrence_only()) return CTCN_OK;
  return rnn_bwd_gemms(cell, T, B, I, H, dirs, x, w_ih0, w_ih1, y, gates, aux, dx, dw_ih0, dw_hh0, dw_ih1, dw_hh1, beta_w, precision,
                       dw_ih0 != nullptr, 0u, ws, ws_bytes, stream);
}

extern "C" int ctcn_rnn_bwd_weights(int cell, int T, int B, int I, int H, int dirs, const float *x, const float *y, const float *gates,
                                    const float *aux, float *dw_ih0, float *dw_hh0, float *dw_ih1, float *dw_hh1, float beta_w,
                                    int precision, unsigned xcd_allow, void *ws, size_t ws_bytes, void *stream) {
  CTCN_REQUIRE(cell >= 0 && cell <= 2, "ctcn_rnn_bwd_weights: unknown cell %d", cell);
  CTCN_REQUIRE(T > 0 && B > 0 && I > 0 && H > 0 && (dirs == 1 || dirs == 2), "ctcn_rnn_bwd_weights: bad dims");
  CTCN_REQUIRE(x && y && gates && (dw_ih0 != nullptr) == (dw_hh0 != nullptr) && (dirs == 1 || (dw_ih1 != nullptr) == (dw_hh1 != nullptr)) &&
                   (dw_ih0 || (dirs == 2 && dw_ih1)), "ctcn_rnn_bwd_weights: null pointer");
  CTCN_REQUIRE(cell != CTCN_CELL_GRU || aux, "ctcn_rnn_bwd_weights: aux (d of the GRU n-gate) required");
  if (ctcn_opt_recurrence_only()) return CTCN_OK;
  return rnn_bwd_gemms(cell, T, B, I, H, dirs, x, nullptr, nullptr, y, gates, aux, nullptr, dw_ih0, dw_hh0, dw_ih1, dw_hh1, beta_w,
                       precision, true, xcd_allow, ws, ws_bytes, stream);
}

extern "C" int ctcn_rnn_bwd(int cell, int T, int B, int I, int H, int dirs, const float *x, const float *w_ih0,
                            const float *w_hh0, const float *w_ih1, const float *w_hh1, const float *y,
                            float *gates, float *aux, const float *dy, float *dx, float *dw_ih0, float *dw_hh0,
                            float *dw_ih1, float *dw_hh1, float beta_w, int precision, void *scratch, void *ws,
                            size_t ws_bytes, void *stream) {
  return ctcn_rnn_bwd_ex(cell, T, B, I, H, dirs, x, w_ih0, w_hh0, w_ih1, w_hh1, y, gates, aux, dy, dx, dw_ih0, dw_hh0, dw_ih1, dw_hh1, beta_w, precision,
                         scratch, ws, ws_bytes, stream, nullptr);
}

extern "C" int ctcn_rnn_bwd_dropout(int cell, int T, int B, int I, int H, int dirs, const float *x, const float *w_ih0, const float *w_hh0,
                                    const float *w_ih1, const float *w_hh1, const float *y, float *gates, float *aux, const float *dy, float *dx,
                                    float *dw_ih0, float *dw_hh0, float *dw_ih1, float *dw_hh1, float beta_w, int precision, void *scratch, void *ws,
                                    size_t ws_bytes, void *stream, float p, uint64_t seed, uint64_t offset, float *dy_tmp) {
  CTCN_REQUIRE(dy_tmp && p >= 0.0f && p < 1.0f, "ctcn_rnn_bwd_dropout: dy_tmp NULL or p=%f outside [0,1)", (double)p);
  ctcn_rnn_call c = {};
  c.dy_tmp = dy_tmp; c.drop_p = p; c.drop_seed = seed; c.drop_offset = offset;
  return ctcn_rnn_bwd_ex(cell, T, B, I, H, dirs, x, w_ih0, w_hh0, w_ih1, w_hh1, y, gates, aux, dy, dx, dw_ih0, dw_hh0, dw_ih1, dw_hh1, beta_w, precision,
                         scratch, ws, ws_bytes, stream, &c);
}
```

### ctc_pytorch_amd/models/model_ctc.py

```python
import math
import os
import sys
from collections import OrderedDict

import numpy as np
import torch

_ROOT = os.path.dirname(os.path.dirname(os.path.dirname(os.path.abspath(__file__))))
if _ROOT not in sys.path:
    sys.path.insert(0, _ROOT)

from ctc_pytorch_amd import nn, ops

F = nn.functional

__author__ = "ctc_pytorch_amd (MI355X-native rebuild; class surface after Ruchao Fan's CTC_pytorch)"


class BatchRNN(nn.Module):

    def __init__(self, input_size, hidden_size, rnn_type=nn.LSTM, bidirectional=False, batch_norm=True, dropout=0.1):
        super().__init__()
        self.input_size = input_size
        self.hidden_size = hidden_size
        self.bidirectional = bidirectional
        self.batch_norm = nn.BatchNorm1d(input_size) if batch_norm else None
        self.rnn = _native_rnn(rnn_type)(input_size=input_size, hidden_size=hidden_size, bidirectional=bidirectional, bias=False)
        self.dropout = nn.Dropout(p=dropout)

    def forward(self, x, lengths=None):
        if self.batch_norm is not None:
            T, B, C = x.shape
            x = ops.batch_norm(ops.contiguous(x), self.batch_norm.weight, self.batch_norm.bias, self.batch_norm.running_mean,
                               self.batch_norm.running_var, T * B, C, 1, self.batch_norm.training,
                               0.1 if self.batch_norm.momentum is None else self.batch_norm.momentum, self.batch_norm.eps,
                               num_batches_tracked=self.batch_norm.num_batches_tracked, lengths=lengths)
        elif lengths is not None:
            x = ops.mask_frames(x, lengths, "tbc")
        if isinstance(self.rnn, (nn.LSTM, nn.GRU, nn.RNN)):
            x, _ = self.rnn(x, drop_p=float(self.dropout.p) if self.dropout.training else 0.0)
            return x
        x, _ = self.rnn(x)
        return self.dropout(x)


def _native_rnn(rnn_type):
    import torch.nn as tnn
    table = {tnn.LSTM: nn.LSTM, tnn.GRU: nn.GRU, tnn.RNN: nn.RNN}
    return table.get(rnn_type, rnn_type)


class LayerCNN(nn.Module):

    def __init__(self, in_channel, out_channel, kernel_size, stride, padding, pooling_size=None, activation_function=nn.ReLU,
                 batch_norm=True, dropout=0.1):
        super().__init__()
        if len(kernel_size) == 2:
            self.conv = nn.Conv2d(in_channel, out_channel, kernel_size=kernel_size, stride=stride, padding=padding)
            self.batch_norm = nn.BatchNorm2d(out_channel) if batch_norm else None
        else:
            self.conv = nn.Conv1d(in_channel, out_channel, kernel_size=kernel_size, stride=stride, padding=padding)
            self.batch_norm = nn.BatchNorm1d(out_channel) if batch_norm else None
        self.activation = _native_act(activation_function)(inplace=True)
        if pooling_size is not None and len(kernel_size) == 2:
            self.pooling = nn.MaxPool2d(pooling_size)
        elif len(kernel_size) == 1:
            self.pooling = nn.MaxPool1d(pooling_size)
        else:
            self.pooling = None
        self.dropout = nn.Dropout(p=dropout)
        self._fused = isinstance(self.activation, nn.ReLU) and self.batch_norm is not None
        if self._fused:
            self.batch_norm.fuse_relu = True

    def out_lengths(self, lengths):
        k, s, p = _pair(self.conv.kernel_size)[0], _pair(self.conv.stride)[0], _pair(self.conv.padding)[0]
        after_conv = (lengths + (2 * p - k)) // s + 1
        pool_t = _pair(self.pooling.kernel_size)[0] if self.pooling is not None else 1
        return after_conv, (after_conv // pool_t if pool_t != 1 else None)

    def _forward_masked(self, x, len_conv, len_pool):
        if self.conv.weight.dim() != 4:
            raise NotImplementedError("input_lengths with the Conv1d front-end")
        x = self.conv(x)
        if self._fused:
            x = self.batch_norm(x, lengths=len_conv)
        else:
            x = self.batch_norm(x, lengths=len_conv) if self.batch_norm is not None else ops.mask_frames(x, len_conv, "bctf")
            x = self.activation(x)
            if not isinstance(self.activation, nn.ReLU):
                x = ops.mask_frames(x, len_conv, "bctf")
        if self.pooling is not None:
            x = self.pooling(x)
            if len_pool is not None:
                x = ops.mask_frames(x, len_pool, "bctf")
        return self.dropout(x)
# ... 100 lines not shown
        rows = [first] + [v for pair in blocks for v in pair if v is not None]
        up = iter(torch.from_numpy(np.stack(rows).astype(np.int32)).to(dev, non_blocking=True).unbind(0))
        first = next(up)
        blocks = [(next(up), None if p is None else next(up)) for _, p in blocks]
        return first, blocks, (blocks[-1][1] if blocks and blocks[-1][1] is not None else blocks[-1][0] if blocks else first)

    def _forward_masked(self, x, visualize, input_lengths):
        B, T = x.shape[0], x.shape[1]
        first, blocks, lens = self._device_stage_lengths(input_lengths, B, T, x.device)
        visual = [x] if visualize else None
        h = ops.mask_frames(x, first, "btf")
        if self.add_cnn:
            c = h.unsqueeze(1)
            for block, stage in zip(self.conv, blocks):
                c = block(c, lengths=stage)
            if visualize:
                visual.append(c)
            h = ops.bctf_to_tbcf(c)
            if visualize:
                visual.append(h)
        else:
            h = ops.contiguous(h.transpose(0, 1))
        for n, block in enumerate(self.rnns):
            h = block(h, lengths=None if n == 0 and block.batch_norm is None else lens)
        Tp = h.shape[0]
        h = h.reshape(Tp * B, -1)
        if isinstance(self.fc, nn.Sequential):
            z = self.fc[1](self.fc[0](h, lengths=lens))
        else:
            z = self.fc(ops.mask_frames(h.view(Tp, B, -1), lens, "tbc").view(Tp * B, -1))
        out = self.log_softmax(z.view(Tp, B, -1))
        if visualize:
            visual.append(out)
            return out, visual
        return out

    def forward(self, x, visualize=False, input_lengths=None):
        if input_lengths is not None:
            return self._forward_masked(x, visualize, input_lengths)
        visual = [x] if visualize else None
        if self.add_cnn:
            c = self.conv(x.unsqueeze(1))
            if visualize:
                visual.append(c)
            if c.dim() != 4:
                raise NotImplementedError("Conv1d front-end")
            h = ops.bctf_to_tbcf(c)
            if visualize:
                visual.append(h)
        else:
            h = ops.contiguous(x.transpose(0, 1))
        h = self.rnns(h)
        T, B, _ = h.shape
        z = self.fc(h.reshape(T * B, -1))
        out = self.log_softmax(z.view(T, B, -1))
        if visualize:
            visual.append(out)
            return out, visual
        return out

    def compute_wer(self, index, input_sizes, targets, target_sizes):
        dev = next(self.parameters()).device
        idx = torch.as_tensor(np.asarray(index) if not torch.is_tensor(index) else index).to(dev).to(torch.int32)
        lens = torch.as_tensor(np.asarray(input_sizes) if not torch.is_tensor(input_sizes) else input_sizes).to(dev)
        tg = torch.as_tensor(np.asarray(targets) if not torch.is_tensor(targets) else targets).to(dev)
        tl = torch.as_tensor(np.asarray(target_sizes) if not torch.is_tensor(target_sizes) else target_sizes).to(dev)
        ids, ids_len = ops.greedy_collapse(idx, lens, blank=0, batch_major=True)
        dist = ops.edit_distance(ids, ids_len, tg, tl)
        return int(dist.sum().item()), int(tl.sum().item())

    def compute_error_ops(self, index, input_sizes, targets, target_sizes, class_map=None):
        dev = next(self.parameters()).device
        idx = torch.as_tensor(np.asarray(index) if not torch.is_tensor(index) else index).to(dev).to(torch.int32)
        lens = torch.as_tensor(np.asarray(input_sizes) if not torch.is_tensor(input_sizes) else input_sizes).to(dev)
        tg = torch.as_tensor(np.asarray(targets) if not torch.is_tensor(targets) else targets).to(dev)
        tl = torch.as_tensor(np.asarray(target_sizes) if not torch.is_tensor(target_sizes) else target_sizes).to(dev)
        ids, ids_len = ops.greedy_collapse(idx, lens, blank=0, batch_major=True)
        counts = ops.edit_ops(ids, ids_len, tg, tl, class_map=class_map, num_classes=None if class_map is None else len(class_map)).counts
        return tuple(int(v) for v in counts.sum(0, dtype=torch.int64).cpu())

    def add_weights_noise(self):
        return None

    @staticmethod
    def save_package(model, optimizer=None, decoder=None, epoch=None, loss_results=None, dev_loss_results=None,
                     dev_cer_results=None):
        package = {"rnn_param": model.rnn_param, "add_cnn": model.add_cnn, "cnn_param": model.cnn_param,
                   "num_class": model.num_class, "_drop_out": model.drop_out, "state_dict": model.state_dict()}
        optional = {"optim_dict": None if optimizer is None else optimizer.state_dict(), "decoder": decoder, "epoch": epoch}
        package.update({k: v for k, v in optional.items() if v is not None})
        if loss_results is not None:
            package.update(loss_results=loss_results, dev_loss_results=dev_loss_results, dev_cer_results=dev_cer_results)
        return package
```

### ctc_pytorch_amd/ops.py

```python
import collections
import ctypes
import os
import numpy as np

import torch

from . import _lib

CELL = {"lstm": 0, "gru": 1, "tanh": 2}
GATES = {0: 4, 1: 3, 2: 1}

def _precision_from_env():
    v = os.environ.get("CTCN_PRECISION", "1").strip()
    if v not in ("0", "1"):
        raise ValueError("CTCN_PRECISION must be 0 (exact f32 MFMA) or 1 (bf16x3 split-operand MFMA), got %r" % v)
    return int(v)


DEFAULT_PRECISION = _precision_from_env()
_precision = [DEFAULT_PRECISION]


def set_precision(p):
    if int(p) not in (0, 1):
# ... 349 lines not shown
        x, w = _f32c(x), _f32c(w)
        M, K = x.shape
        N = w.shape[0]
        y = torch.empty((M, N), dtype=torch.float32, device=x.device)
        gemm(0, 1, M, N, K, x, K, w, K, y, N)
        ctx.save_for_backward(x, w)
        return y

    @staticmethod
    def backward(ctx, gy):
        x, w = ctx.saved_tensors
        gy = _f32c(gy)
        M, K = x.shape
        N = w.shape[0]
        gx = gw = None
        if ctx.needs_input_grad[0]:
            gx = torch.empty((M, K), dtype=torch.float32, device=x.device)
            gemm(0, 0, M, K, N, gy, N, w, K, gx, K)
        if ctx.needs_input_grad[1]:
            if ctx.gw_view is not None:
                gemm(1, 0, N, K, M, gy, N, x, K, ctx.gw_view, K, beta=1.0)
            else:
                gw = torch.empty((N, K), dtype=torch.float32, device=x.device)
                gemm(1, 0, N, K, M, gy, N, x, K, gw, K)
        return gx, gw


def linear(x2d, w):
    return _Linear.apply(x2d, w)


_Saved = collections.namedtuple("_Saved", "x y gates aux w_ih0 w_hh0 w_ih1 w_hh1")


def _new_rnn_call(dev):
    call, launched = _lib.RnnCall(), ctypes.c_char_p(None)
    call.status = _lib.status_word(dev).data_ptr()
    call.launched = ctypes.pointer(launched)
    return call, launched


def _note_launch(launched, step_kernel, cell, T, B, H, dirs):
    _count_kernel(launched)
    if T > 1 and B > 16 and (launched or b"") == step_kernel and get_option("rnn_persistent"):
        _fallback_shapes.add((cell, H, dirs, B))


def _note_rnn_fwd(I, s, y_drop, w):
    adr = lambda t: t.data_ptr() if t is not None else 0
    _debug_note[0]("rnn_fwd", dict(I=int(I), x=adr(s.x), gates=adr(s.gates), aux=adr(s.aux), y=adr(s.y), y_drop=adr(y_drop), ws=adr(w), w_ih=adr(s.w_ih0), w_hh=adr(s.w_hh0)),
                   dict(x=s.x, y=s.y, gates=s.gates, aux=s.aux, y_drop=y_drop, w_ih=(s.w_ih0, s.w_ih1)))


def _weight_grads(cell, dims, s, dws, prec, xcd_allow=0, side=None):
    w, wp, wn = _ws(s.x, tag="main" if side is None else "side")
    _lib.check(_lib.lib().ctcn_rnn_bwd_weights(cell, *dims, _ptr(s.x), _ptr(s.y), _ptr(s.gates), _ptr(s.aux), *[_ptr(d) for d in dws],
                                               1.0, prec, xcd_allow, wp, wn, _lib.stream_ptr()), "rnn_bwd_weights")
    if side is not None:
        for t in (s.x, s.y, s.gates, s.aux):
            if t is not None:
                t.record_stream(side)


class _RNNLayer(torch.autograd.Function):
    @staticmethod
    def forward(ctx, x, w_ih0, w_hh0, w_ih1, w_hh1, cell, training, drop_p=0.0):
        _need_gpu(x, w_ih0, w_hh0, w_ih1, w_hh1)
        ctx.gviews = [_gview(w) for w in (w_ih0, w_hh0, w_ih1, w_hh1)]
        x = _f32c(x)
        ws = [_f32c(w) if w is not None else None for w in (w_ih0, w_hh0, w_ih1, w_hh1)]
        for k in (1, 3):
            if ws[k] is not None and ws[k].data_ptr() % 16:
                ws[k] = ws[k].clone()
        T, B, I = x.shape
        G = GATES[cell]
        H = ws[1].shape[1]
        dirs = 2 if ws[2] is not None else 1
        dev = x.device
        y = torch.empty((T, B, dirs * H), dtype=torch.float32, device=dev)
        gates = torch.empty((T, B, dirs, G * H), dtype=torch.float32, device=dev)
        aux = torch.empty((T, B, dirs, H), dtype=torch.float32, device=dev) if cell != 2 else None
        s = _Saved(x, y, gates, aux, *ws)
        w, wp, wn = _ws(x)
        L = _lib.lib()
        side = _device_side(dev)
        call, launched = _new_rnn_call(dev)
        piped = plan_fwd_pipeline(T, B, H, dirs, L.ctcn_device_xcds())
        if piped:
            st = side.side_stream()
            w2, wp2, wn2 = _ws(x, tag="side")
            call.side_stream, call.side_event, call.side_ws, call.side_ws_bytes, call.xcd_allow = st.cuda_stream, side.prelaunch_event().cuda_event, w2.data_ptr(), wn2, piped
        ctx.drop = None
        y_drop = None
        if training and drop_p > 0.0:
            y_drop = torch.empty_like(y)
            seed, off = _next_dropout_stream(y.numel())
            ctx.drop = (float(drop_p), seed, off)
            call.y_drop, call.drop_p, call.drop_seed, call.drop_offset = y_drop.data_ptr(), float(drop_p), seed, off
        _lib.check(L.ctcn_rnn_fwd_ex(cell, T, B, I, H, dirs, _ptr(x), _ptr(ws[0]), _ptr(ws[1]), _ptr(ws[2]), _ptr(ws[3]),
                                     _ptr(y), _ptr(gates), _ptr(aux), get_precision(), wp, wn, _lib.stream_ptr(), ctypes.byref(call)), "rnn_fwd_ex")
        _note_launch(launched.value, b"rnn_fwd_step", cell, T, B, H, dirs)
        if _debug_note[0] is not None:
            _note_rnn_fwd(I, s, y_drop, w)
        if piped:
            torch.cuda.current_stream(dev).wait_stream(st)
            for t in (x, gates, ws[0], ws[2]):
                if t is not None:
                    t.record_stream(st)
        ctx.cell, ctx.dims = cell, (T, B, I, H, dirs)
        ctx.early_ok = not _chunking[0]
        ctx.consumed = False
        ctx.counted = any(ctx.needs_input_grad)
        if ctx.counted:
            side.live += 1
        ctx.save_for_backward(*s)
        return y if y_drop is None else y_drop

    @staticmethod
    def backward(ctx, gy):
        if ctx.consumed:
            raise RuntimeError("ctc_pytorch_amd RNN layer: backward ran twice (the gate reserve is overwritten in place)")
        ctx.consumed = True
        dims = T, B, I, H, dirs = ctx.dims
        cell = ctx.cell
        s = _Saved(*ctx.saved_tensors)
        wts = (s.w_ih0, s.w_hh0, s.w_ih1, s.w_hh1)
        gy = _f32c(gy)
        dev = s.x.device
        dx = torch.empty_like(s.x) if ctx.needs_input_grad[0] else None
        into_flat = all(g is not None for g, w in zip(ctx.gviews, wts) if w is not None)
        dws = [None if w is None else (g if into_flat else torch.empty_like(w)) for g, w in zip(ctx.gviews, wts)]
        L = _lib.lib()
        scratch = torch.empty(L.ctcn_rnn_scratch_bytes(cell, B, H, dirs), dtype=torch.uint8, device=dev)
        w, wp, wn = _ws(s.x)
        side = _device_side(dev)
        if ctx.counted:
            side.live = max(0, side.live - 1)
        mode, allow = plan_weight_grads(cell, T, B, I, H, dirs, L.ctcn_device_xcds(), L.ctcn_device_cus(), into_flat=into_flat, chunk=not ctx.early_ok,
                                        bottom=dx is None or side.live == 0, above_parked=side.deferred is not None)
        above, side.deferred, ev = side.deferred, None, None
        call, launched = _new_rnn_call(dev)
        if above is not None:
            ev = side.prelaunch_event()
            call.prelaunch_event = ev.cuda_event
        gd = None
        if ctx.drop is not None:
            p_, seed_, off_ = ctx.drop
            gd = torch.empty_like(gy)
            call.dy_tmp, call.drop_p, call.drop_seed, call.drop_offset = gd.data_ptr(), p_, seed_, off_
        prec = get_precision()
        try:
            _lib.check(L.ctcn_rnn_bwd_ex(cell, T, B, I, H, dirs, _ptr(s.x), *[_ptr(t) for t in wts], _ptr(s.y), _ptr(s.gates), _ptr(s.aux), _ptr(gy), _ptr(dx),
                                         *[_ptr(d) if mode == WG_INLINE else None for d in dws],
                                         1.0 if into_flat else 0.0, prec, _ptr(scratch), wp, wn, _lib.stream_ptr(), ctypes.byref(call)), "rnn_bwd_ex")
        except Exception:
            side.deferred = above
            raise
        _note_launch(launched.value, b"rnn_bwd_step", cell, T, B, H, dirs)
        if above is not None:
            above(ev)
        if mode in (WG_SPLIT_END, WG_SPLIT_NOW):
            st, main = side.side_stream(), torch.cuda.current_stream(dev)
            st.wait_stream(main)
            with torch.cuda.stream(st):
                _weight_grads(cell, dims, s, [None, None] + dws[2:], prec, side=st)
            _weight_grads(cell, dims, s, dws[:2] + [None, None], prec)
            if mode == WG_SPLIT_NOW:
                main.wait_stream(st)
            else:
                side.pending = True
                torch.autograd.Variable._execution_engine.queue_callback(side.join_at_end)
        elif mode == WG_DEFERRED:
            st = side.side_stream()

            def weights_on_side_stream(after=None):
                if after is None:
                    st.wait_stream(torch.cuda.current_stream(dev))
                else:
                    st.wait_event(after)
                with torch.cuda.stream(st):
                    _weight_grads(cell, dims, s, dws, prec, allow, side=st)
                    if _grad_ready["hook"] is not None:
                        _grad_ready["hook"]([t for t in dws if t is not None])
                side.pending = True

            side.deferred = weights_on_side_stream
            torch.autograd.Variable._execution_engine.queue_callback(side.join_at_end)
        return (dx,) + ((None,) * 7 if into_flat else tuple(dws) + (None,) * 3)


def persistent_batch_limit(H, dirs, nx, cus):
    nsl = _tiles16(H)
    per_xcd = (cus // max(nx, 1)) // nsl if nsl else 0
    return 16 * ((per_xcd * max(nx, 1)) // dirs) if nx > 1 else 0


def rnn_layer(x, w_ih0, w_hh0, w_ih1, w_hh1, cell, training=True, drop_p=0.0):
    cellc = CELL[cell] if isinstance(cell, str) else cell
    T, B = int(x.shape[0]), int(x.shape[1])
    H, dirs = int(w_hh0.shape[1]), 2 if w_ih1 is not None else 1
    if x.is_cuda and T > 1 and _chunks_on[0] and (cellc, H, dirs, B) in _fallback_shapes and get_option("rnn_persistent"):
        L = _lib.lib()
        bmax = persistent_batch_limit(H, dirs, L.ctcn_device_xcds(), L.ctcn_device_cus())
        if 0 < bmax < B:
            _chunking[0] = True
            try:
                ys = [_RNNLayer.apply(xc, w_ih0, w_hh0, w_ih1, w_hh1, cellc, training, 0.0) for xc in x.split(bmax, dim=1)]
            finally:
                _chunking[0] = False
            return dropout(torch.cat(ys, dim=1), float(drop_p), training)
    return _RNNLayer.apply(x, w_ih0, w_hh0, w_ih1, w_hh1, cellc, training, float(drop_p))


_chunks_on = [os.environ.get("CTCN_BATCH_CHUNKS", "1") != "0"]
_chunking = [False]
_fallback_shapes = set()


def set_batch_chunks(flag):
    _chunks_on[0] = bool(flag)


def mark_batch_chunks(cell, H, dirs, B):
    _fallback_shapes.add((CELL[cell] if isinstance(cell, str) else int(cell), int(H), int(dirs), int(B)))


_sync_bn = {"reduce": None}


def set_sync_bn(reducer):
    _sync_bn["reduce"] = reducer


class _BatchNorm(torch.autograd.Function):
    @staticmethod
    def forward(ctx, x, gamma, beta, rm, rv, outer, C, inner, training, momentum, eps, relu, nbt=None, drop_p=0.0):
        _need_gpu(x, gamma, beta)
        ctx.gviews = (_gview(gamma), _gview(beta))
        x = _f32c(x)
        dev = x.device
        y = torch.empty_like(x)
# ... 11 lines not shown
            ctx.save_for_backward(x, None, gamma, mean, rstd, beta)
            ctx.train_mode = True
            ctx.drop = (float(drop_p), seed, off)
            ctx.geom = (outer, C, inner, relu, eps)
            return y
        if training and _sync_bn["reduce"] is not None:
            mean = torch.empty(C, dtype=torch.float32, device=dev)
            rstd = torch.empty(C, dtype=torch.float32, device=dev)
            sums = torch.empty((C, 2), dtype=torch.float64, device=dev)
            w, wp, wn = _ws(x)
            _lib.check(L.ctcn_bn_fwd_sums(_ptr(x), _ptr(sums), outer, C, inner, wp, wn, _lib.stream_ptr()), "bn_fwd_sums")
            total = float(_sync_bn["reduce"](sums, outer * inner))
            _lib.check(L.ctcn_bn_fwd_finish(_ptr(x), _ptr(y), _ptr(gamma), _ptr(beta), _ptr(rm), _ptr(rv), _ptr(mean), _ptr(rstd),
                                            _ptr(sums), total, outer, C, inner, float(eps), float(momentum), int(relu),
                                            _lib.stream_ptr(), _ptr(nbt)), "bn_fwd_finish")
            ctx.save_for_backward(x, y if relu else None, gamma, mean, rstd)
            ctx.train_mode = True
            ctx.sync = (_sync_bn["reduce"], total)
        elif training:
            mean = torch.empty(C, dtype=torch.float32, device=dev)
            rstd = torch.empty(C, dtype=torch.float32, device=dev)
            w, wp, wn = _ws(x)
            _lib.check(L.ctcn_bn_fwd_train(_ptr(x), _ptr(y), _ptr(gamma), _ptr(beta), _ptr(rm), _ptr(rv), _ptr(mean), _ptr(rstd),
                                           outer, C, inner, float(eps), float(momentum), int(relu), wp, wn, _lib.stream_ptr(), _ptr(nbt)),
                       "bn_fwd_train")
            ctx.save_for_backward(x, y if relu else None, gamma, mean, rstd)
            ctx.train_mode = True
        else:
            _lib.check(L.ctcn_bn_fwd_eval(_ptr(x), _ptr(y), _ptr(gamma), _ptr(beta), _ptr(rm), _ptr(rv), outer, C, inner, float(eps),
                                          int(relu), _lib.stream_ptr()), "bn_fwd_eval")
            ctx.save_for_backward(x, y if relu else None, gamma, rm, rv)
            ctx.train_mode = False
        ctx.geom = (outer, C, inner, relu, eps)
        return y

    @staticmethod
    def backward(ctx, gy):
        outer, C, inner, relu, eps = ctx.geom
        if ctx.drop is not None:
            x, _, gamma, a, b, beta = ctx.saved_tensors
            gy = _f32c(gy)
            dx = torch.empty_like(x)
            into_flat = ctx.gviews[0] is not None and ctx.gviews[1] is not None
            dgamma, dbeta = ctx.gviews if into_flat else (torch.empty(C, dtype=torch.float32, device=x.device), torch.empty(C, dtype=torch.float32, device=x.device))
            w, wp, wn = _ws(x)
            p_, seed_, off_ = ctx.drop
            _lib.check(_lib.lib().ctcn_bn_bwd_dropout(_ptr(x), _ptr(gy), _ptr(gamma), _ptr(beta), _ptr(a), _ptr(b), _ptr(dx), _ptr(dgamma), _ptr(dbeta),
                                                      outer, C, inner, int(relu), 1.0 if into_flat else 0.0, wp, wn, _lib.stream_ptr(), p_, seed_, off_),
                       "bn_bwd_dropout")
            if into_flat:
                dgamma = dbeta = None
            return dx, dgamma, dbeta, None, None, None, None, None, None, None, None, None, None, None
        x, y, gamma, a, b = ctx.saved_tensors
        gy = _f32c(gy)
        dev = x.device
        if not ctx.train_mode:
            raise NotImplementedError("ctc_pytorch_amd: backward through eval-mode BatchNorm is not part of the hot path")
        dx = torch.empty_like(x)
        into_flat = ctx.gviews[0] is not None and ctx.gviews[1] is not None
        if into_flat:
            dgamma, dbeta = ctx.gviews
        else:
            dgamma = torch.empty(C, dtype=torch.float32, device=dev)
            dbeta = torch.empty(C, dtype=torch.float32, device=dev)
        w, wp, wn = _ws(x)
        if ctx.sync is not None:
            reducer, total = ctx.sync
            L = _lib.lib()
            local = torch.empty((C, 2), dtype=torch.float64, device=dev)
            _lib.check(L.ctcn_bn_bwd_sums(_ptr(x), _ptr(y), _ptr(gy), _ptr(a), _ptr(b), _ptr(local), outer, C, inner, int(relu), wp, wn,
                                          _lib.stream_ptr()), "bn_bwd_sums")
            glob = local.clone()
            reducer(glob, outer * inner)
            _lib.check(L.ctcn_bn_bwd_finish(_ptr(x), _ptr(y), _ptr(gy), _ptr(gamma), _ptr(a), _ptr(b), _ptr(dx), _ptr(dgamma), _ptr(dbeta),
                                            _ptr(local), _ptr(glob), total, outer, C, inner, int(relu), 1.0 if into_flat else 0.0,
                                            wp, wn, _lib.stream_ptr()), "bn_bwd_finish")
        else:
            _lib.check(_lib.lib().ctcn_bn_bwd(_ptr(x), _ptr(y), _ptr(gy), _ptr(gamma), _ptr(a), _ptr(b), _ptr(dx), _ptr(dgamma),
                                              _ptr(dbeta), outer, C, inner, int(relu), 1.0 if into_flat else 0.0, wp, wn,
                                              _lib.stream_ptr()), "bn_bwd")
        if into_flat:
            dgamma = dbeta = None
        return dx, dgamma, dbeta, None, None, None, None, None, None, None, None, None, None, None


def batch_norm(x, gamma, beta, running_mean, running_var, outer, C, inner, training, momentum=0.1, eps=1e-5, relu=False, num_batches_tracked=None,
               drop_p=0.0, lengths=None, frame=None):
    if lengths is not None:
        return batch_norm_masked(x, gamma, beta, running_mean, running_var, outer, C, inner, training, lengths, frame, momentum, eps, relu,
                                 num_batches_tracked, drop_p)
    if training and drop_p > 0.0 and (_sync_bn["reduce"] is not None or not _fuse_bn_dropout[0]):
        y = batch_norm(x, gamma, beta, running_mean, running_var, outer, C, inner, training, momentum, eps, relu, num_batches_tracked)
        return dropout(y, drop_p, training)
    if not training:
        drop_p = 0.0
    if num_batches_tracked is not None and (not training or num_batches_tracked.dtype != torch.int64 or not num_batches_tracked.is_cuda):
        if training:
            num_batches_tracked += 1
        num_batches_tracked = None
    return _BatchNorm.apply(x, gamma, beta, running_mean, running_var, outer, C, inner, training, momentum, eps, relu, num_batches_tracked, float(drop_p))


_fuse_bn_dropout = [os.environ.get("CTCN_FUSE_BN_DROPOUT", "1") != "0"]


def set_fuse_bn_dropout(flag):
    _fuse_bn_dropout[0] = bool(flag)


def frame_lengths(lengths, device, batch=None, tmax=None):
    if torch.is_tensor(lengths):
        if lengths.dim() != 1 or lengths.dtype not in (torch.int32, torch.int64, torch.int16, torch.uint8, torch.int8):
            raise ValueError("lengths: expected a 1-D integer tensor, got %s %s" % (lengths.dtype, tuple(lengths.shape)))
        if batch is not None and lengths.numel() != batch:
            raise ValueError("lengths: %d entries for a batch of %d" % (lengths.numel(), batch))
        if lengths.is_cuda:
            return lengths if lengths.dtype == torch.int32 and lengths.is_contiguous() else lengths.to(torch.int32).contiguous()
        host = lengths.detach().numpy().astype(np.int64)
    else:
        host = np.asarray(lengths)
        if host.ndim != 1 or host.dtype.kind not in "iu":
            raise ValueError("lengths: expected a flat sequence of integers")
        host = host.astype(np.int64)
        if batch is not None and host.size != batch:
            raise ValueError("lengths: %d entries for a batch of %d" % (host.size, batch))
    check_frame_lengths(host, tmax)
    return torch.from_numpy(host.astype(np.int32)).to(device, non_blocking=True)


def check_frame_lengths(host, tmax=None):
    if host.size and int(host.min()) < 1:
        raise ValueError("lengths: every utterance needs at least one frame, got %d" % int(host.min()))
    if tmax is not None and host.size and int(host.max()) > tmax:
        raise ValueError("lengths: %d exceeds the %d frames of the batch" % (int(host.max()), tmax))


# ... 772 lines not shown
```

### include/ctcn.h

```cpp
#ifndef CTCN_H
#define CTCN_H
#include <stddef.h>
#include <stdint.h>
#ifdef __cplusplus
extern "C" {
#endif

#define CTCN_OK 0
#define CTCN_EINVAL (-1)
#define CTCN_EHIP (-2)
#define CTCN_EUNSUPPORTED (-3)
#define CTCN_EWORKSPACE (-4)

#define CTCN_REDUCTION_NONE 0
#define CTCN_REDUCTION_MEAN 1
#define CTCN_REDUCTION_SUM 2

#define CTCN_CELL_LSTM 0
#define CTCN_CELL_GRU 1
#define CTCN_CELL_TANH 2

int ctcn_version(void);
const char *ctcn_last_error(void);
int ctcn_device_cus(void);
int ctcn_device_xcds(void);
int ctcn_set_option(const char *name, int value);
int ctcn_get_option(const char *name);
const char *ctcn_option_name(int index);
int ctcn_set_status_buffer(int *dev_word);

int ctcn_gemm(int transA, int transB, int M, int N, int K, const float *A, int lda, const float *B, int ldb,
              float *C, int ldc, float beta, int precision, void *ws, size_t ws_bytes, void *stream);

int ctcn_transpose01(const float *in, float *out, int A, int B, int C, void *stream);
int ctcn_copy_strided4(const float *in, float *out, int d0, int d1, int d2, int d3, size_t s0, size_t s1, size_t s2,
                       size_t s3, void *stream);
int ctcn_relu_fwd(const float *x, float *y, size_t n, void *stream);
int ctcn_relu_bwd(const float *y, const float *dy, float *dx, size_t n, void *stream);
int ctcn_maxpool2d_fwd(const float *x, float *y, unsigned char *arg, size_t planes, int Hi, int Wi, int kh, int kw, void *stream);
int ctcn_maxpool2d_bwd(const float *dy, const unsigned char *arg, float *dx, size_t planes, int Hi, int Wi, int kh, int kw, void *stream);

size_t ctcn_rnn_scratch_bytes(int cell, int B, int H, int dirs);
int ctcn_rnn_fwd(int cell, int T, int B, int I, int H, int dirs, const float *x, const float *w_ih0,
                 const float *w_hh0, const float *w_ih1, const float *w_hh1, float *y, float *gates, float *aux,
                 int precision, void *ws, size_t ws_bytes, void *stream);
int ctcn_rnn_fwd_dropout(int cell, int T, int B, int I, int H, int dirs, const float *x, const float *w_ih0, const float *w_hh0,
                         const float *w_ih1, const float *w_hh1, float *y, float *gates, float *aux, float *y_drop, float p, uint64_t seed,
                         uint64_t offset, int precision, void *ws, size_t ws_bytes, void *stream);
int ctcn_rnn_bwd(int cell, int T, int B, int I, int H, int dirs, const float *x, const float *w_ih0,
                 const float *w_hh0, const float *w_ih1, const float *w_hh1, const float *y, float *gates,
                 float *aux, const float *dy, float *dx, float *dw_ih0, float *dw_hh0, float *dw_ih1,
                 float *dw_hh1, float beta_w, int precision, void *scratch, void *ws, size_t ws_bytes,
                 void *stream);
int ctcn_rnn_bwd_dropout(int cell, int T, int B, int I, int H, int dirs, const float *x, const float *w_ih0, const float *w_hh0,
                         const float *w_ih1, const float *w_hh1, const float *y, float *gates, float *aux, const float *dy, float *dx,
                         float *dw_ih0, float *dw_hh0, float *dw_ih1, float *dw_hh1, float beta_w, int precision, void *scratch, void *ws,
                         size_t ws_bytes, void *stream, float p, uint64_t seed, uint64_t offset, float *dy_tmp);
typedef struct ctcn_rnn_call {
  float drop_p;
  uint64_t drop_seed, drop_offset;
  float *y_drop;
  float *dy_tmp;
  void *side_stream, *side_event, *side_ws;
  size_t side_ws_bytes;
  unsigned xcd_allow;
  void *prelaunch_event;
  int *status;
  const char **launched;
} ctcn_rnn_call;
int ctcn_rnn_fwd_ex(int cell, int T, int B, int I, int H, int dirs, const float *x, const float *w_ih0, const float *w_hh0,
                    const float *w_ih1, const float *w_hh1, float *y, float *gates, float *aux, int precision, void *ws, size_t ws_bytes,
                    void *stream, const ctcn_rnn_call *call);
int ctcn_rnn_bwd_ex(int cell, int T, int B, int I, int H, int dirs, const float *x, const float *w_ih0, const float *w_hh0,
                    const float *w_ih1, const float *w_hh1, const float *y, float *gates, float *aux, const float *dy, float *dx,
                    float *dw_ih0, float *dw_hh0, float *dw_ih1, float *dw_hh1, float beta_w, int precision, void *scratch, void *ws,
                    size_t ws_bytes, void *stream, const ctcn_rnn_call *call);
int ctcn_rnn_bwd_weights(int cell, int T, int B, int I, int H, int dirs, const float *x, const float *y,
                         const float *gates, const float *aux, float *dw_ih0, float *dw_hh0, float *dw_ih1,
                         float *dw_hh1, float beta_w, int precision, unsigned xcd_allow, void *ws, size_t ws_bytes,
                         void *stream);

size_t ctcn_bn_ws_bytes(int outer, int C, int inner);
int ctcn_bn_fwd_train(const float *x, float *y, const float *gamma, const float *beta, float *running_mean,
                      float *running_var, float *save_mean, float *save_rstd, int outer, int C, int inner,
                      float eps, float momentum, int relu, void *ws, size_t ws_bytes, void *stream,
                      long long *num_batches_tracked );
int ctcn_bn_fwd_sums(const float *x, double *sums, int outer, int C, int inner, void *ws, size_t ws_bytes, void *stream);
int ctcn_bn_fwd_finish(const float *x, float *y, const float *gamma, const float *beta, float *running_mean,
                       float *running_var, float *save_mean, float *save_rstd, const double *sums, double count_total,
                       int outer, int C, int inner, float eps, float momentum, int relu, void *stream,
                       long long *num_batches_tracked );
int ctcn_bn_bwd_sums(const float *x, const float *y, const float *dy, const float *save_mean, const float *save_rstd,
                     double *sums, int outer, int C, int inner, int relu, void *ws, size_t ws_bytes, void *stream);
int ctcn_bn_bwd_finish(const float *x, const float *y, const float *dy, const float *gamma, const float *save_mean,
                       const float *save_rstd, float *dx, float *dgamma, float *dbeta, const double *local_sums,
                       const double *global_sums, double count_total, int outer, int C, int inner, int relu,
                       float beta_acc, void *ws, size_t ws_bytes, void *stream);
int ctcn_bn_fwd_eval(const float *x, float *y, const float *gamma, const float *beta, const float *running_mean,
                     const float *running_var, int outer, int C, int inner, float eps, int relu, void *stream);
int ctcn_bn_bwd(const float *x, const float *y, const float *dy, const float *gamma, const float *save_mean,
                const float *save_rstd, float *dx, float *dgamma, float *dbeta, int outer, int C, int inner,
                int relu, float beta_acc, void *ws, size_t ws_bytes, void *stream);
int ctcn_bn_fwd_train_dropout(const float *x, float *y_drop, const float *gamma, const float *beta, float *running_mean, float *running_var,
                              float *save_mean, float *save_rstd, int outer, int C, int inner, float eps, float momentum, int relu, void *ws,
                              size_t ws_bytes, void *stream, long long *num_batches_tracked, float p, uint64_t seed, uint64_t offset);
int ctcn_bn_bwd_dropout(const float *x, const float *dy_drop, const float *gamma, const float *beta, const float *save_mean, const float *save_rstd,
                        float *dx, float *dgamma, float *dbeta, int outer, int C, int inner, int relu, float beta_acc, void *ws, size_t ws_bytes,
                        void *stream, float p, uint64_t seed, uint64_t offset);

size_t ctcn_bn_masked_ws_bytes(int outer, int C, int inner);
int ctcn_mask_frames(const float *x, float *y, const int *lens, int batch, int frame, int outer, int C, int inner, void *stream);
int ctcn_bn_fwd_train_masked(const float *x, float *y, const float *gamma, const float *beta, float *running_mean, float *running_var,
                             float *save_mean, float *save_rstd, const int *lens, int batch, int frame, int outer, int C, int inner,
                             float eps, float momentum, int relu, void *ws, size_t ws_bytes, void *stream, long long *num_batches_tracked);
int ctcn_bn_fwd_eval_masked(const float *x, float *y, const float *gamma, const float *beta, const float *running_mean,
                            const float *running_var, const int *lens, int batch, int frame, int outer, int C, int inner, float eps,
                            int relu, void *stream);
int ctcn_bn_bwd_masked(const float *x, const float *y, const float *dy, const float *gamma, const float *save_mean, const float *save_rstd,
                       float *dx, float *dgamma, float *dbeta, const int *lens, int batch, int frame, int outer, int C, int inner, int relu,
                       float beta_acc, void *ws, size_t ws_bytes, void *stream);

int ctcn_dropout(const float *x, float *y, size_t n, float p, uint64_t seed, uint64_t offset, void *stream);

size_t ctcn_conv2d_ws_bytes(int B, int Ci, int Hi, int Wi, int Co, int kh, int kw, int sh, int sw, int ph, int pw);
int ctcn_conv2d_fwd(const float *x, const float *w, const float *bias, float *y, int B, int Ci, int Hi, int Wi,
                    int Co, int kh, int kw, int sh, int sw, int ph, int pw, void *stream);
int ctcn_conv2d_bwd(const float *x, const float *w, const float *dy, float *dx , float *dw,
                    float *dbias, int B, int Ci, int Hi, int Wi, int Co, int kh, int kw, int sh, int sw, int ph,
                    int pw, float beta_acc, void *ws, size_t ws_bytes, void *stream);
int ctcn_bctf_to_tbcf(const float *in, float *out, int B, int C, int T, int F, void *stream);
int ctcn_tbcf_to_bctf(const float *in, float *out, int B, int C, int T, int F, void *stream);

int ctcn_log_softmax_fwd(const float *logits, float *lp, int32_t *argmax, int rows, int V, void *stream);
int ctcn_log_softmax_bwd(const float *lp, const float *dlp, float *dlogits, int rows, int V, void *stream);
int ctcn_argmax(const float *lp, int32_t *argmax, int rows, int V, void *stream);

int ctcn_ctc_fwd(const float *lp, const int64_t *targets, const int64_t *in_len, const int64_t *tgt_len,
                 float *alpha, float *nll, int T, int B, int V, int Lmax, void *stream);
int ctcn_ctc_bwd(const float *lp, const int64_t *targets, const int64_t *in_len, const int64_t *tgt_len,
// ... 81 lines not shown
```

Measured before the change: 1.968 million frames/s.

## Fold BatchNorm normalisation into GEMM operand split for BN→RNN and BN→Linear

Adds a BatchNorm affine descriptor that the bf16x3 split/transpose kernels apply as they load operands, so the normalised activation never has to be written out before the input-projection GEMM of each RNN layer and the final Linear. New autograd functions fuse BN with the following RNN layer or Linear, computing only the statistics separately and reapplying the affine in backward weight GEMMs. Shapes whose kernels read f32 operands directly fall back to a scratch normalise pass. The saving is one full-activation write and read per BN, paid for with more per-element arithmetic in the split kernels and extra backward complexity.

```diff
diff --git a/ctc_pytorch_amd/_lib.py b/ctc_pytorch_amd/_lib.py
--- a/ctc_pytorch_amd/_lib.py
+++ b/ctc_pytorch_amd/_lib.py
@@ -24,6 +24,9 @@
     "ctcn_option_name": (ctypes.c_char_p, [I]),
     "ctcn_set_status_buffer": (I, [P]),
     "ctcn_gemm": (I, [I, I, I, I, I, P, I, P, I, P, I, F, I, P, Z, P]),
+    "ctcn_gemm_affine": (I, [I, I, I, I, I, P, I, P, I, P, I, F, I, P, Z, P, P, P, P, P]),
+    "ctcn_gemm_affine_f32_operands": (I, [I, I, I, I, I, P, I, P, I, I, P, Z]),
+    "ctcn_sizeof": (I, [I]),
     "ctcn_transpose01": (I, [P, P, I, I, I, P]),
     "ctcn_copy_strided4": (I, [P, P, I, I, I, I, Z, Z, Z, Z, P]),
     "ctcn_relu_fwd": (I, [P, P, Z, P]),
@@ -36,7 +39,10 @@
     "ctcn_rnn_bwd": (I, [I, I, I, I, I, I, P, P, P, P, P, P, P, P, P, P, P, P, P, P, F, I, P, P, Z, P]),
     "ctcn_rnn_bwd_dropout": (I, [I, I, I, I, I, I, P, P, P, P, P, P, P, P, P, P, P, P, P, P, F, I, P, P, Z, P, F, U, U, P]),
     "ctcn_rnn_bwd_weights": (I, [I, I, I, I, I, I, P, P, P, P, P, P, P, P, F, I, ctypes.c_uint, P, Z, P]),
+    "ctcn_rnn_bwd_weights_ex": (I, [I, I, I, I, I, I, P, P, P, P, P, P, P, P, F, I, ctypes.c_uint, P, Z, P, P]),
     "ctcn_bn_ws_bytes": (Z, [I, I, I]),
+    "ctcn_bn_fwd_stats": (I, [P, P, D, P, P, P, P, I, I, I, F, F, P, Z, P, P]),
+    "ctcn_bn_apply_affine": (I, [P, P, P, I, I, P]),
     "ctcn_bn_fwd_train": (I, [P, P, P, P, P, P, P, P, I, I, I, F, F, I, P, Z, P, P]),
     "ctcn_bn_fwd_eval": (I, [P, P, P, P, P, P, I, I, I, F, I, P]),
     "ctcn_bn_fwd_sums": (I, [P, P, I, I, I, P, Z, P]),
@@ -100,11 +106,16 @@
 }
 
 
+class BnAffine(ctypes.Structure):
+    _fields_ = [("mean", ctypes.c_void_p), ("rstd_or_var", ctypes.c_void_p), ("gamma", ctypes.c_void_p), ("beta", ctypes.c_void_p),
+                ("eps", ctypes.c_float), ("var_is_variance", ctypes.c_int)]
+
+
 class RnnCall(ctypes.Structure):
     _fields_ = [("drop_p", ctypes.c_float), ("drop_seed", ctypes.c_uint64), ("drop_offset", ctypes.c_uint64), ("y_drop", ctypes.c_void_p),
                 ("dy_tmp", ctypes.c_void_p), ("side_stream", ctypes.c_void_p), ("side_event", ctypes.c_void_p), ("side_ws", ctypes.c_void_p),
                 ("side_ws_bytes", ctypes.c_size_t), ("xcd_allow", ctypes.c_uint), ("prelaunch_event", ctypes.c_void_p), ("status", ctypes.c_void_p),
-                ("launched", ctypes.POINTER(ctypes.c_char_p))]
+                ("launched", ctypes.POINTER(ctypes.c_char_p)), ("x_affine", BnAffine), ("x_norm", ctypes.c_void_p)]
 
 
 def sources():
diff --git a/ctc_pytorch_amd/csrc/common.h b/ctc_pytorch_amd/csrc/common.h
--- a/ctc_pytorch_amd/csrc/common.h
+++ b/ctc_pytorch_amd/csrc/common.h
@@ -11,7 +11,14 @@
 int *ctcn_status_word(void);
 int ctcn_opt_rnn_persistent(void);
 int ctcn_transpose01_pair(const float *in0, const float *in1, float *out0, float *out1, int A, int B, int C, void *stream);
+typedef ctcn_bn_affine BnAffine;
+static inline bool same_affine(const BnAffine &p, const BnAffine &q) {
+  return p.mean == q.mean && p.rstd_or_var == q.rstd_or_var && p.gamma == q.gamma && p.beta == q.beta && p.eps == q.eps && p.var_is_variance == q.var_is_variance;
+}
 struct GemmPlanes {
+  BnAffine aff_a = {}, aff_b = {}, done_aff_a = {}, done_aff_b = {};
+  float *tmp_a = nullptr, *tmp_b = nullptr;
+  bool dry = false; int f32_ops = 0;
   const float *A = nullptr; int lda = 0, M = 0, Ka = 0, transA = 0; void *ws_a = nullptr, *st_a = nullptr; bool a_valid = false;
   const float *B = nullptr; int ldb = 0, N = 0, Kb = 0, transB = 0, shift = 0; void *ws_b = nullptr, *st_b = nullptr; const void *bh = nullptr; bool b_valid = false;
   bool same_a = false, same_b = false;
@@ -73,6 +80,28 @@
 }
 __device__ __forceinline__ void lds_barrier() { asm volatile("s_waitcnt lgkmcnt(0)\n\ts_barrier" ::: "memory"); }
 
+__device__ __forceinline__ float bn_value(float x, float m, float rs, float g, float b) { return fmaf((x - m) * rs, g, b); }
+__device__ __forceinline__ float bn_rs(float rstd_or_var, float eps, int var_is_variance) { return var_is_variance ? 1.0f / sqrtf(rstd_or_var + eps) : rstd_or_var; }
+__device__ __forceinline__ float bn_affine_value(const BnAffine &a, int c, float x) {
+  return bn_value(x, a.mean[c], bn_rs(a.rstd_or_var[c], a.eps, a.var_is_variance), a.gamma[c], a.beta[c]);
+}
+__device__ __forceinline__ void bn_affine_value4(const BnAffine &a, bool vec, int c, float (&x)[4]) {
+  if (vec) {
+    const float4 m = *reinterpret_cast<const float4 *>(a.mean + c), r = *reinterpret_cast<const float4 *>(a.rstd_or_var + c);
+    const float4 g = *reinterpret_cast<const float4 *>(a.gamma + c), b = *reinterpret_cast<const float4 *>(a.beta + c);
+    x[0] = bn_value(x[0], m.x, bn_rs(r.x, a.eps, a.var_is_variance), g.x, b.x);
+    x[1] = bn_value(x[1], m.y, bn_rs(r.y, a.eps, a.var_is_variance), g.y, b.y);
+    x[2] = bn_value(x[2], m.z, bn_rs(r.z, a.eps, a.var_is_variance), g.z, b.z);
+    x[3] = bn_value(x[3], m.w, bn_rs(r.w, a.eps, a.var_is_variance), g.w, b.w);
+  } else {
+#pragma unroll
+    for (int k = 0; k < 4; ++k) x[k] = bn_affine_value(a, c + k, x[k]);
+  }
+}
+static inline bool affine_vec16(const BnAffine &a) {
+  return (((uintptr_t)a.mean | (uintptr_t)a.rstd_or_var | (uintptr_t)a.gamma | (uintptr_t)a.beta) & 15) == 0;
+}
+
 __device__ __forceinline__ float sigmoidf_(float x) { return 1.0f / (1.0f + expf(-x)); }
 
 __device__ __forceinline__ void philox_round(uint32_t (&c)[4], uint32_t (&k)[2]) {
diff --git a/ctc_pytorch_amd/csrc/core.hip b/ctc_pytorch_amd/csrc/core.hip
--- a/ctc_pytorch_amd/csrc/core.hip
+++ b/ctc_pytorch_amd/csrc/core.hip
@@ -57,6 +57,7 @@
 static int g_opt_rnn_slow_items = 0;
 static int g_opt_rnn_slow_exchange = 0;
 static int g_opt_xcd_interleave_force = 0;
+static int g_opt_bn_on_load = 1;
 static int *g_status_dev = nullptr;
 
 struct OptionRow { const char *name; int *var; int (*norm)(int); };
@@ -75,6 +76,7 @@
   {"tn_splits_xcd", &g_opt_tn_splits_xcd, [](int value) -> int { return value ? 1 : 0; }},
   {"xcd_interleave", &g_opt_xcd_interleave, [](int value) -> int { return value < 0 ? 0 : (value > 5 ? 5 : value); }},
   {"bn_rows4", &g_opt_bn_rows4, [](int value) -> int { return value ? 1 : 0; }},
+  {"bn_on_load", &g_opt_bn_on_load, [](int value) -> int { return value ? 1 : 0; }},
   {"tn_splits_force", &g_opt_tn_splits_force, [](int value) -> int { return value < 0 ? 0 : value; }},
   {"gemm_bf16_single", &g_opt_gemm_bf16_single, [](int value) -> int { return value ? 1 : 0; }},
   {"beam_generic_threads", &g_opt_beam_generic_threads, [](int value) -> int { return (value == 256 || value == 512 || value == 1024) ? value : 0; }},
diff --git a/ctc_pytorch_amd/csrc/gemm.hip b/ctc_pytorch_amd/csrc/gemm.hip
--- a/ctc_pytorch_amd/csrc/gemm.hip
+++ b/ctc_pytorch_amd/csrc/gemm.hip
@@ -326,23 +326,33 @@
 constexpr int PBK = 64;
 
 __global__ void split_rows_kernel(const float *__restrict__ src, int ld, int R, int C, int Cp, unsigned short *__restrict__ hi,
-                                  unsigned short *__restrict__ lo) {
+                                  unsigned short *__restrict__ lo, BnAffine aff, bool aff_vec) {
   const size_t total = (size_t)R * (Cp / 4);
   for (size_t i = blockIdx.x * (size_t)blockDim.x + threadIdx.x; i < total; i += (size_t)gridDim.x * blockDim.x) {
     const int r = (int)(i / (Cp / 4)), c = (int)(i - (size_t)r * (Cp / 4)) * 4;
     unsigned short h[4], l[4];
-#pragma unroll
-    for (int k = 0; k < 4; ++k) {
-      const float v = (c + k < C) ? src[(size_t)r * ld + c + k] : 0.0f;
-      split_bf16(v, h[k], l[k]);
-    }
+    float v[4];
+#pragma unroll
+    for (int k = 0; k < 4; ++k) v[k] = (c + k < C) ? src[(size_t)r * ld + c + k] : 0.0f;
+    if (aff.mean) {
+      if (c + 4 <= C) {
+        bn_affine_value4(aff, aff_vec, c, v);
+      } else {
+#pragma unroll
+        for (int k = 0; k < 4; ++k)
+          if (c + k < C) v[k] = bn_affine_value(aff, c + k, v[k]);
+      }
+    }
+#pragma unroll
+    for (int k = 0; k < 4; ++k) split_bf16(v[k], h[k], l[k]);
     *reinterpret_cast<uint2 *>(hi + (size_t)r * Cp + c) = make_uint2((unsigned)h[0] | ((unsigned)h[1] << 16), (unsigned)h[2] | ((unsigned)h[3] << 16));
     *reinterpret_cast<uint2 *>(lo + (size_t)r * Cp + c) = make_uint2((unsigned)l[0] | ((unsigned)l[1] << 16), (unsigned)l[2] | ((unsigned)l[3] << 16));
   }
 }
 
 __device__ __forceinline__ void split_transpose_tile(float (*t)[65], int bx, int by, const float *__restrict__ src, int ld, int R, int C, int Rp,
-                                                     unsigned short *__restrict__ hi, unsigned short *__restrict__ lo, int shift) {
+                                                     unsigned short *__restrict__ hi, unsigned short *__restrict__ lo, int shift, const BnAffine &aff,
+                                                     bool aff_vec) {
   const int r0 = by * 64, c0 = bx * 64;
   const int tid = threadIdx.x;
   const bool vec = c0 + 64 <= C && (ld & 3) == 0 && ((uintptr_t)src & 15) == 0;
@@ -352,7 +362,14 @@
       const int idx = tid + 256 * j, i = idx >> 4, c4 = idx & 15;
       const int r = r0 + i - shift;
       float4 v = make_float4(0.f, 0.f, 0.f, 0.f);
-      if (r >= 0 && r < R && r0 + i < R) v = *reinterpret_cast<const float4 *>(src + (size_t)r * ld + c0 + 4 * c4);
+      if (r >= 0 && r < R && r0 + i < R) {
+        v = *reinterpret_cast<const float4 *>(src + (size_t)r * ld + c0 + 4 * c4);
+        if (aff.mean) {
+          float q[4] = {v.x, v.y, v.z, v.w};
+          bn_affine_value4(aff, aff_vec, c0 + 4 * c4, q);
+          v = make_float4(q[0], q[1], q[2], q[3]);
+        }
+      }
       t[i][4 * c4 + 0] = v.x; t[i][4 * c4 + 1] = v.y; t[i][4 * c4 + 2] = v.z; t[i][4 * c4 + 3] = v.w;
     }
     __syncthreads();
@@ -377,7 +394,12 @@
   const int tx = tid & 63, ty = tid >> 6;
   for (int i = ty; i < 64; i += 4) {
     const int r = r0 + i - shift, c = c0 + tx;
-    t[i][tx] = (r >= 0 && r < R && r0 + i < R && c < C) ? src[(size_t)r * ld + c] : 0.0f;
+    float v = 0.0f;
+    if (r >= 0 && r < R && r0 + i < R && c < C) {
+      v = src[(size_t)r * ld + c];
+      if (aff.mean) v = bn_affine_value(aff, c, v);
+    }
+    t[i][tx] = v;
   }
   __syncthreads();
   for (int i = ty; i < 64; i += 4) {
@@ -392,13 +414,15 @@
 }
 
 __global__ __launch_bounds__(256) void split_transpose_kernel(const float *__restrict__ src, int ld, int R, int C, int Rp,
-                                                              unsigned short *__restrict__ hi, unsigned short *__restrict__ lo, int shift) {
+                                                              unsigned short *__restrict__ hi, unsigned short *__restrict__ lo, int shift, BnAffine aff,
+                                                              bool aff_vec) {
   __shared__ float t[64][65];
-  split_transpose_tile(t, blockIdx.x, blockIdx.y, src, ld, R, C, Rp, hi, lo, shift);
+  split_transpose_tile(t, blockIdx.x, blockIdx.y, src, ld, R, C, Rp, hi, lo, shift, aff, aff_vec);
 }
 __global__ __launch_bounds__(256) void split_transpose_queue_kernel(const float *__restrict__ src, int ld, int R, int C, int Rp,
                                                                     unsigned short *__restrict__ hi, unsigned short *__restrict__ lo, int tiles_x,
-                                                                    int tiles_y, unsigned xcd_allow, unsigned *__restrict__ queue, int shift) {
+                                                                    int tiles_y, unsigned xcd_allow, unsigned *__restrict__ queue, int shift, BnAffine aff,
+                                                                    bool aff_vec) {
   __shared__ float t[64][65];
   __shared__ int s_item;
   unsigned x;
@@ -409,7 +433,7 @@
     __syncthreads();
     const int item = s_item;
     if (item >= tiles_x * tiles_y) return;
-    split_transpose_tile(t, item % tiles_x, item / tiles_x, src, ld, R, C, Rp, hi, lo, shift);
+    split_transpose_tile(t, item % tiles_x, item / tiles_x, src, ld, R, C, Rp, hi, lo, shift, aff, aff_vec);
     __syncthreads();
   }
 }
@@ -1661,11 +1685,31 @@
   GemmPlanes &pl = planes ? *planes : scratch_planes;
   const bool want_same_a = pl.same_a, want_same_b = pl.same_b;
   pl.same_a = pl.same_b = false;
+  pl.f32_ops = 0;
   CTCN_REQUIRE(precision == 0 || precision == 1, "ctcn_gemm: precision %d (0 = f32 MFMA, 1 = bf16x3 split MFMA)", precision);
   CTCN_REQUIRE(M > 0 && N > 0 && K >= 0, "ctcn_gemm: bad dims M=%d N=%d K=%d", M, N, K);
   CTCN_REQUIRE(A && B && C, "ctcn_gemm: null pointer");
   CTCN_REQUIRE(lda >= (transA ? M : K) && ldb >= (transB ? K : N) && ldc >= N, "ctcn_gemm: leading dim too small");
   CTCN_REQUIRE(!ws || (uintptr_t)ws % 16 == 0, "ctcn_gemm: the workspace must be 16-byte aligned");
+  const BnAffine aff_a = pl.aff_a, aff_b = pl.aff_b;
+  CTCN_REQUIRE(!aff_a.mean || lda == (transA ? M : K), "ctcn_gemm: an operand with a BatchNorm affine must be contiguous (lda %d)", lda);
+  CTCN_REQUIRE(!aff_b.mean || ldb == (transB ? K : N), "ctcn_gemm: an operand with a BatchNorm affine must be contiguous (ldb %d)", ldb);
+  CTCN_REQUIRE((!aff_a.mean || (aff_a.rstd_or_var && aff_a.gamma && aff_a.beta)) && (!aff_b.mean || (aff_b.rstd_or_var && aff_b.gamma && aff_b.beta)),
+               "ctcn_gemm: incomplete BatchNorm affine");
+  const float *A_pre = A, *B_pre = B;
+  if (aff_a.mean && pl.tmp_a) A = pl.tmp_a;
+  if (aff_b.mean && pl.tmp_b) B = pl.tmp_b;
+  auto normalise_f32 = [&](bool a, bool b) -> int {
+    if (a && aff_a.mean) {
+      if (!pl.tmp_a) { ctcn_set_error("ctcn_gemm: this shape's kernel reads A as float32: scratch for the normalised operand required"); return CTCN_EINVAL; }
+      if (int rc = ctcn_bn_apply_affine(A_pre, pl.tmp_a, &aff_a, transA ? K : M, transA ? M : K, stream)) return rc;
+    }
+    if (b && aff_b.mean) {
+      if (!pl.tmp_b) { ctcn_set_error("ctcn_gemm: this shape's kernel reads B as float32: scratch for the normalised operand required"); return CTCN_EINVAL; }
+      if (int rc = ctcn_bn_apply_affine(B_pre, pl.tmp_b, &aff_b, transB ? N : K, transB ? K : N, stream)) return rc;
+    }
+    return CTCN_OK;
+  };
   hipStream_t st = (hipStream_t)stream;
   const int tiles_m = ceil_div(M, BM), tiles_n = ceil_div(N, BN);
   const int nt = tiles_m * tiles_n;
@@ -1683,6 +1727,8 @@
   }
   if (tn_eligible(transA, transB, M, N, K, A, lda, B, ldb, precision, ws, ws_bytes) && b_shift == 0) {
     pl.a_valid = false; pl.b_valid = false;
+    if (pl.dry) { pl.f32_ops = 3; return CTCN_OK; }
+    if (int rc = normalise_f32(true, true)) return rc;
     const int wnt = ceil_div(N, 256) * 256 == ceil_div(N, 128) * 128 ? 2 : 1;
     unsigned *queue = (unsigned *)((char *)ws + ((ws_bytes - 256) & ~(size_t)255));
     int tn_cus = 256;
@@ -1703,34 +1749,37 @@
       float *part = (float *)((char *)ws + plane_bytes);
       unsigned *queue = (unsigned *)((char *)ws + ((ws_bytes - 256) & ~(size_t)255));
       const size_t part_bytes = ws_bytes - plane_bytes - 512;
-      if (xcd_allow) CTCN_HIP(hipMemsetAsync(queue, 0, 16, st));
+      if (xcd_allow && !pl.dry) CTCN_HIP(hipMemsetAsync(queue, 0, 16, st));
       int nq = 0;
-      auto split = [&](const float *src, int ld, bool contraction_major, int rows, unsigned short *hi, unsigned short *lo, int shift) {
+      auto split = [&](const float *src, int ld, bool contraction_major, int rows, unsigned short *hi, unsigned short *lo, int shift, const BnAffine &aff) {
+        const bool av = aff.mean && affine_vec16(aff);
         if (!contraction_major) {
           const size_t total = (size_t)rows * (Kp / 4);
-          hipLaunchKernelGGL(split_rows_kernel, dim3((unsigned)std::min((size_t)8192, ceil_div_z(total, 256))), dim3(256), 0, st, src, ld, rows, K, Kp, hi, lo);
+          hipLaunchKernelGGL(split_rows_kernel, dim3((unsigned)std::min((size_t)8192, ceil_div_z(total, 256))), dim3(256), 0, st, src, ld, rows, K, Kp, hi, lo, aff, av);
         } else {
           if (xcd_allow)
             hipLaunchKernelGGL(split_transpose_queue_kernel, dim3(ctcn_opt_side_split_wgs() * ctcn_device_cus()), dim3(256), 0, st, src, ld, K, rows, Kp, hi, lo, ceil_div(rows, 64),
-                               ceil_div(Kp, 64), xcd_allow, queue + (++nq), shift);
+                               ceil_div(Kp, 64), xcd_allow, queue + (++nq), shift, aff, av);
           else
-            hipLaunchKernelGGL(split_transpose_kernel, dim3(ceil_div(rows, 64), ceil_div(Kp, 64)), dim3(256), 0, st, src, ld, K, rows, Kp, hi, lo, shift);
+            hipLaunchKernelGGL(split_transpose_kernel, dim3(ceil_div(rows, 64), ceil_div(Kp, 64)), dim3(256), 0, st, src, ld, K, rows, Kp, hi, lo, shift, aff, av);
         }
       };
-      const bool same_a = want_same_a && pl.a_valid && pl.A == A && pl.lda == lda && pl.M == M && pl.Ka == K && pl.transA == transA && pl.ws_a == ws &&
-                          pl.st_a == (void *)st;
-      const bool same_b = want_same_b && pl.b_valid && pl.B == B && pl.ldb == ldb && pl.N == N && pl.Kb == K && pl.transB == transB && pl.shift == b_shift &&
-                          pl.ws_b == ws && pl.st_b == (void *)st && pl.bh == (const void *)bh;
-      pl.B = B; pl.ldb = ldb; pl.N = N; pl.Kb = K; pl.transB = transB; pl.shift = b_shift; pl.ws_b = ws;
+      const bool same_a = want_same_a && pl.a_valid && pl.A == A_pre && pl.lda == lda && pl.M == M && pl.Ka == K && pl.transA == transA && pl.ws_a == ws &&
+                          pl.st_a == (void *)st && same_affine(pl.done_aff_a, aff_a);
+      const bool same_b = want_same_b && pl.b_valid && pl.B == B_pre && pl.ldb == ldb && pl.N == N && pl.Kb == K && pl.transB == transB && pl.shift == b_shift &&
+                          pl.ws_b == ws && pl.st_b == (void *)st && pl.bh == (const void *)bh && same_affine(pl.done_aff_b, aff_b);
+      pl.B = B_pre; pl.done_aff_b = aff_b; pl.ldb = ldb; pl.N = N; pl.Kb = K; pl.transB = transB; pl.shift = b_shift; pl.ws_b = ws;
       pl.st_b = (void *)st; pl.bh = (const void *)bh; pl.b_valid = true;
       const int wnt256 = (N % 256 == 0 || (N > 512 && ceil_div(N, 256) * 256 - N <= N / 8)) ? 2 : 1;
       const bool use256 = !xcd_allow && ctcn_get_option("gemm_tile256") != 0 && M >= 1024 && N >= 96 &&
                           (long)ceil_div(M, 256) * ceil_div(N, 128 * wnt256) * 4 >= (long)ctcn_device_cus() * 3;
       const bool a_inline = use256 && !same_a && !transA && ctcn_get_option("gemm_a_inline") != 0 && K >= 32 && K % 4 == 0 && lda % 4 == 0 &&
                             ((uintptr_t)A & 15) == 0 && ceil_div(N, 128 * wnt256) <= 5;
+      if (pl.dry) { pl.f32_ops = a_inline ? 1 : 0; return CTCN_OK; }
       if (a_inline) {
         pl.a_valid = false;
-        if (!same_b) split(B, ldb, transB == 0, N, bh, bl, b_shift);
+        if (int rc = normalise_f32(true, false)) return rc;
+        if (!same_b) split(B_pre, ldb, transB == 0, N, bh, bl, b_shift, aff_b);
         CTCN_LAUNCH_CHECK();
         const int lrc = wnt256 == 2 ? launch_planes256_af32<2>(st, M, N, K, Kp, A, lda, bh, bl, C, ldc, beta)
                                     : launch_planes256_af32<1>(st, M, N, K, Kp, A, lda, bh, bl, C, ldc, beta);
@@ -1738,10 +1787,10 @@
         CTCN_LAUNCH_CHECK();
         return CTCN_OK;
       }
-      if (!same_a) split(A, lda, transA != 0, M, ah, al, 0);
-      pl.A = A; pl.lda = lda; pl.M = M; pl.Ka = K; pl.transA = transA; pl.ws_a = ws; pl.st_a = (void *)st;
+      if (!same_a) split(A_pre, lda, transA != 0, M, ah, al, 0, aff_a);
+      pl.A = A_pre; pl.done_aff_a = aff_a; pl.lda = lda; pl.M = M; pl.Ka = K; pl.transA = transA; pl.ws_a = ws; pl.st_a = (void *)st;
       pl.a_valid = true;
-      if (!same_b) split(B, ldb, transB == 0, N, bh, bl, b_shift);
+      if (!same_b) split(B_pre, ldb, transB == 0, N, bh, bl, b_shift, aff_b);
       CTCN_LAUNCH_CHECK();
       int shape = 0, ptm = tiles_m, ptn = tiles_n;
       {
@@ -1801,6 +1850,8 @@
     }
   }
   pl.a_valid = false; pl.b_valid = false;
+  if (pl.dry) { pl.f32_ops = 3; return CTCN_OK; }
+  if (int rc = normalise_f32(true, true)) return rc;
   const bool vecA = ((uintptr_t)A % 16 == 0) && (lda % 4 == 0);
   const bool vecB = ((uintptr_t)B % 16 == 0) && (ldb % 4 == 0);
   float *wsp = splits > 1 ? (float *)ws : nullptr;
@@ -1845,6 +1896,7 @@
                       void *ws, size_t ws_bytes, void *stream, unsigned xcd_allow, int shift, GemmPlanes *planes) {
   const int as = shift < 0 ? -shift : shift;
   CTCN_REQUIRE(as < K, "ctcn_gemm_shift_b: |shift| %d >= K %d", as, K);
+  CTCN_REQUIRE(!planes || (!planes->aff_a.mean && !planes->aff_b.mean), "ctcn_gemm_shift_b: no BatchNorm affine on a shifted product");
   const int Kp = ceil_div(K, PBK) * PBK;
   const size_t plane_bytes = align_up(2 * ((size_t)M * Kp + (size_t)N * Kp) * sizeof(unsigned short), 256);
   const bool plane = precision == 1 && K >= 64 && ws && ws_bytes >= plane_bytes + 1024 &&
@@ -1855,6 +1907,29 @@
     return gemm_core(1, 0, M, N, K - as, A2, lda, B2, ldb, C, ldc, beta, precision, ws, ws_bytes, stream, xcd_allow, planes, 0);
   }
   return gemm_core(1, 0, M, N, K, A, lda, B, ldb, C, ldc, beta, precision, ws, ws_bytes, stream, xcd_allow, planes, shift);
+}
+
+extern "C" int ctcn_gemm_affine(int transA, int transB, int M, int N, int K, const float *A, int lda, const float *B, int ldb, float *C, int ldc, float beta,
+                                int precision, void *ws, size_t ws_bytes, void *stream, const ctcn_bn_affine *aff_a, float *tmp_a, const ctcn_bn_affine *aff_b,
+                                float *tmp_b) {
+  GemmPlanes pl;
+  if (aff_a) { pl.aff_a = *aff_a; pl.tmp_a = tmp_a; }
+  if (aff_b) { pl.aff_b = *aff_b; pl.tmp_b = tmp_b; }
+  return gemm_core(transA, transB, M, N, K, A, lda, B, ldb, C, ldc, beta, precision, ws, ws_bytes, stream, 0u, &pl, 0);
+}
+extern "C" int ctcn_gemm_affine_f32_operands(int transA, int transB, int M, int N, int K, const float *A, int lda, const float *B, int ldb, int precision,
+                                             const void *ws, size_t ws_bytes) {
+  GemmPlanes pl;
+  pl.dry = true;
+  float c_unused = 0.0f;
+  const int rc = gemm_core(transA, transB, M, N, K, A, lda, B, ldb, &c_unused, N, 0.0f, precision, const_cast<void *>(ws), ws_bytes, nullptr, 0u, &pl, 0);
+  return rc ? rc : pl.f32_ops;
+}
+extern "C" int ctcn_sizeof(int which) {
+  if (which == 1) return (int)sizeof(ctcn_bn_affine);
+  if (which == 2) return (int)sizeof(ctcn_rnn_call);
+  ctcn_set_error("ctcn_sizeof: unknown struct %d", which);
+  return CTCN_EINVAL;
 }
 
 extern "C" int ctcn_gemm(int transA, int transB, int M, int N, int K, const float *A, int lda, const float *B,
diff --git a/ctc_pytorch_amd/csrc/norm.hip b/ctc_pytorch_amd/csrc/norm.hip
--- a/ctc_pytorch_amd/csrc/norm.hip
+++ b/ctc_pytorch_amd/csrc/norm.hip
@@ -28,7 +28,6 @@
   }
 };
 struct DropSpec { float p, scale; uint64_t seed, offset; const float *gamma, *beta; };
-__device__ __forceinline__ float bn_value(float x, float m, float rs, float g, float b) { return fmaf((x - m) * rs, g, b); }
 __device__ __forceinline__ bool drop_keep(uint32_t word, float p) { return (word >> 8) * (1.0f / 16777216.0f) >= p; }
 __device__ __forceinline__ float bn_dx_value(float g, float xh, float ga, float rs, float s0, float s1, float inv_n) {
   return ga * rs * fmaf(-xh, s1 * inv_n, fmaf(-s0, inv_n, g));
@@ -662,6 +661,36 @@
                     save_mean, save_rstd, outer, C, inner, eps, momentum, relu, ws, ws_bytes, stream, num_batches_tracked, nullptr);
 }
 
+extern "C" int ctcn_bn_fwd_stats(const float *x, const double *sums, double count_total, float *running_mean, float *running_var, float *save_mean,
+                                 float *save_rstd, int outer, int C, int inner, float eps, float momentum, void *ws, size_t ws_bytes, void *stream,
+                                 long long *num_batches_tracked) {
+  CTCN_REQUIRE(x && save_mean && save_rstd && (sums || ws), "ctcn_bn_fwd_stats: null pointer");
+  CTCN_REQUIRE(dims_ok(outer, C, inner) && (!sums || count_total >= (double)outer * inner), "ctcn_bn_fwd_stats: bad dims / count");
+  hipStream_t st = (hipStream_t)stream;
+  const AllFrames g = all_frames(sums ? count_total : (double)outer * inner);
+  const double *part = sums;
+  int nchunks = 1;
+  if (!sums) {
+    if (ws_bytes < ctcn_bn_ws_bytes(outer, C, inner)) { ctcn_set_error("ctcn_bn_fwd_stats: workspace too small"); return CTCN_EWORKSPACE; }
+    launch_reduce(StatVal{x}, g, outer, C, inner, (double *)ws, &nchunks, st);
+    CTCN_LAUNCH_CHECK();
+    part = (const double *)ws;
+  }
+  hipLaunchKernelGGL(bn_finalize_stats_kernel<AllFrames>, dim3(ceil_div(C, 4)), dim3(256), 0, st, part, nchunks, C, g, eps, momentum, save_mean, save_rstd,
+                     running_mean, running_var, num_batches_tracked);
+  CTCN_LAUNCH_CHECK();
+  return CTCN_OK;
+}
+
+extern "C" int ctcn_bn_apply_affine(const float *x, float *y, const ctcn_bn_affine *affine, int rows, int C, void *stream) {
+  CTCN_REQUIRE(x && y && affine && affine->mean && affine->rstd_or_var && affine->gamma && affine->beta, "ctcn_bn_apply_affine: null pointer");
+  CTCN_REQUIRE(dims_ok(rows, C, 1), "ctcn_bn_apply_affine: bad dims");
+  launch_bn_apply((hipStream_t)stream, all_frames((double)rows), x, y, affine->gamma, affine->beta, affine->mean, affine->rstd_or_var, affine->eps,
+                  affine->var_is_variance, (size_t)rows * C, C, 1, 0);
+  CTCN_LAUNCH_CHECK();
+  return CTCN_OK;
+}
+
 extern "C" int ctcn_bn_fwd_train_dropout(const float *x, float *y_drop, const float *gamma, const float *beta, float *running_mean, float *running_var,
                                          float *save_mean, float *save_rstd, int outer, int C, int inner, float eps, float momentum, int relu, void *ws,
                                          size_t ws_bytes, void *stream, long long *num_batches_tracked, float p, uint64_t seed, uint64_t offset) {
diff --git a/ctc_pytorch_amd/csrc/rnn.hip b/ctc_pytorch_amd/csrc/rnn.hip
--- a/ctc_pytorch_amd/csrc/rnn.hip
+++ b/ctc_pytorch_amd/csrc/rnn.hip
@@ -2225,6 +2225,8 @@
 
 static int project_chunk(const FwdCall &c, const PipePlan &p, int chunk, void *ws, size_t ws_bytes, void *stream, unsigned allow, GemmPlanes &pl) {
   const int t0 = chunk * p.chunk_T, t1 = std::min(c.T, t0 + p.chunk_T), N2 = 2 * c.GH;
+  pl.aff_a = c.call.x_affine;
+  pl.tmp_a = c.call.x_norm ? c.call.x_norm + (size_t)t0 * c.B * c.I : nullptr;
   return ctcn_gemm_on_xcds(0, 1, (t1 - t0) * c.B, N2, c.I, c.x + (size_t)t0 * c.B * c.I, c.I, c.w_ih[0], c.I, c.gates + (size_t)t0 * c.B * N2, N2, 0.0f, c.precision,
                            ws, ws_bytes, stream, allow, &pl);
 }
@@ -2239,6 +2241,7 @@
 static int project_all(const FwdCall &c) {
   const int TB = c.T * c.B;
   GemmPlanes pl;
+  pl.aff_a = c.call.x_affine; pl.tmp_a = c.call.x_norm;
   if (c.dirs == 2) {
     StackedWih s;
     if (int rc = stack_w_ih(c.w_ih[0], c.w_ih[1], c.GH, c.I, c.ws, c.ws_bytes, c.st(), s)) return rc;
@@ -2416,8 +2419,13 @@
 static int rnn_bwd_gemms(int cell, int T, int B, int I, int H, int dirs, const float *x, const float *w_ih0, const float *w_ih1,
                          const float *y, const float *gates, const float *aux, float *dx, float *dw_ih0, float *dw_hh0, float *dw_ih1,
                          float *dw_hh1, float beta_w, int precision, bool weights, unsigned xcd_allow, void *ws, size_t ws_bytes,
-                         void *stream) {
+                         void *stream, const ctcn_rnn_call &call) {
   const int G = gates_of(cell), GH = G * H, TB = T * B;
+  if (weights && call.x_affine.mean && (dw_ih0 || (dirs == 2 && dw_ih1))) {
+    CTCN_REQUIRE(call.x_norm, "ctcn_rnn_bwd: x_affine without x_norm scratch");
+    if (int rc = ctcn_bn_apply_affine(x, call.x_norm, &call.x_affine, TB, I, stream)) return rc;
+    x = call.x_norm;
+  }
   const float *w_ih[2] = {w_ih0, w_ih1};
   float *dw_ih[2] = {dw_ih0, dw_ih1};
   float *dw_hh[2] = {dw_hh0, dw_hh1};
@@ -2624,12 +2632,13 @@
 
   if (ctcn_opt_recurrence_only()) return CTCN_OK;
   return rnn_bwd_gemms(cell, T, B, I, H, dirs, x, w_ih0, w_ih1, y, gates, aux, dx, dw_ih0, dw_hh0, dw_ih1, dw_hh1, beta_w, precision,
-                       dw_ih0 != nullptr, 0u, ws, ws_bytes, stream);
-}
-
-extern "C" int ctcn_rnn_bwd_weights(int cell, int T, int B, int I, int H, int dirs, const float *x, const float *y, const float *gates,
-                                    const float *aux, float *dw_ih0, float *dw_hh0, float *dw_ih1, float *dw_hh1, float beta_w,
-                                    int precision, unsigned xcd_allow, void *ws, size_t ws_bytes, void *stream) {
+                       dw_ih0 != nullptr, 0u, ws, ws_bytes, stream, call);
+}
+
+extern "C" int ctcn_rnn_bwd_weights_ex(int cell, int T, int B, int I, int H, int dirs, const float *x, const float *y, const float *gates,
+                                       const float *aux, float *dw_ih0, float *dw_hh0, float *dw_ih1, float *dw_hh1, float beta_w, int precision,
+                                       unsigned xcd_allow, void *ws, size_t ws_bytes, void *stream, const ctcn_rnn_call *call_p) {
+  const ctcn_rnn_call &call = call_p ? *call_p : k_plain_call;
   CTCN_REQUIRE(cell >= 0 && cell <= 2, "ctcn_rnn_bwd_weights: unknown cell %d", cell);
   CTCN_REQUIRE(T > 0 && B > 0 && I > 0 && H > 0 && (dirs == 1 || dirs == 2), "ctcn_rnn_bwd_weights: bad dims");
   CTCN_REQUIRE(x && y && gates && (dw_ih0 != nullptr) == (dw_hh0 != nullptr) && (dirs == 1 || (dw_ih1 != nullptr) == (dw_hh1 != nullptr)) &&
@@ -2637,7 +2646,13 @@
   CTCN_REQUIRE(cell != CTCN_CELL_GRU || aux, "ctcn_rnn_bwd_weights: aux (d of the GRU n-gate) required");
   if (ctcn_opt_recurrence_only()) return CTCN_OK;
   return rnn_bwd_gemms(cell, T, B, I, H, dirs, x, nullptr, nullptr, y, gates, aux, nullptr, dw_ih0, dw_hh0, dw_ih1, dw_hh1, beta_w,
-                       precision, true, xcd_allow, ws, ws_bytes, stream);
+                       precision, true, xcd_allow, ws, ws_bytes, stream, call);
+}
+extern "C" int ctcn_rnn_bwd_weights(int cell, int T, int B, int I, int H, int dirs, const float *x, const float *y, const float *gates,
+                                    const float *aux, float *dw_ih0, float *dw_hh0, float *dw_ih1, float *dw_hh1, float beta_w,
+                                    int precision, unsigned xcd_allow, void *ws, size_t ws_bytes, void *stream) {
+  return ctcn_rnn_bwd_weights_ex(cell, T, B, I, H, dirs, x, y, gates, aux, dw_ih0, dw_hh0, dw_ih1, dw_hh1, beta_w, precision, xcd_allow, ws, ws_bytes, stream,
+                                 nullptr);
 }
 
 extern "C" int ctcn_rnn_bwd(int cell, int T, int B, int I, int H, int dirs, const float *x, const float *w_ih0,
diff --git a/ctc_pytorch_amd/models/model_ctc.py b/ctc_pytorch_amd/models/model_ctc.py
--- a/ctc_pytorch_amd/models/model_ctc.py
+++ b/ctc_pytorch_amd/models/model_ctc.py
@@ -29,6 +29,14 @@
         self.dropout = nn.Dropout(p=dropout)
 
     def forward(self, x, lengths=None):
+        if _bn_on_load(self.batch_norm, x, lengths) and isinstance(self.rnn, (nn.LSTM, nn.GRU, nn.RNN)) and self.rnn.hidden_size % 4 == 0:
+            bn, rnn = self.batch_norm, self.rnn
+            rnn._check()
+            rev = (rnn.weight_ih_l0_reverse, rnn.weight_hh_l0_reverse) if rnn.bidirectional else (None, None)
+            return ops.bn_rnn_layer(ops.contiguous(x), bn.weight, bn.bias, bn.running_mean, bn.running_var, bn.training,
+                                    0.1 if bn.momentum is None else bn.momentum, bn.eps, bn.num_batches_tracked,
+                                    rnn.weight_ih_l0, rnn.weight_hh_l0, rev[0], rev[1], rnn._cell, rnn.training,
+                                    float(self.dropout.p) if self.dropout.training and rnn.training else 0.0)
         if self.batch_norm is not None:
             T, B, C = x.shape
             x = ops.batch_norm(ops.contiguous(x), self.batch_norm.weight, self.batch_norm.bias, self.batch_norm.running_mean,
@@ -42,6 +50,11 @@
             return x
         x, _ = self.rnn(x)
         return self.dropout(x)
+
+
+def _bn_on_load(bn, x, lengths):
+    return (bn is not None and lengths is None and x.is_cuda and isinstance(bn, nn.BatchNorm1d) and bn.affine and bn.track_running_stats
+            and not bn.fuse_relu and ops.bn_on_load())
 
 
 def _native_rnn(rnn_type):
@@ -248,7 +261,13 @@
             h = ops.contiguous(x.transpose(0, 1))
         h = self.rnns(h)
         T, B, _ = h.shape
-        z = self.fc(h.reshape(T * B, -1))
+        h = h.reshape(T * B, -1)
+        if isinstance(self.fc, nn.Sequential) and self.fc[1].bias is None and _bn_on_load(self.fc[0], h, None):
+            bn = self.fc[0]
+            z = ops.bn_linear(h, bn.weight, bn.bias, bn.running_mean, bn.running_var, bn.training, 0.1 if bn.momentum is None else bn.momentum,
+                              bn.eps, bn.num_batches_tracked, self.fc[1].weight)
+        else:
+            z = self.fc(h)
         out = self.log_softmax(z.view(T, B, -1))
         if visualize:
             visual.append(out)
diff --git a/ctc_pytorch_amd/ops.py b/ctc_pytorch_amd/ops.py
--- a/ctc_pytorch_amd/ops.py
+++ b/ctc_pytorch_amd/ops.py
@@ -425,19 +425,48 @@
                    dict(x=s.x, y=s.y, gates=s.gates, aux=s.aux, y_drop=y_drop, w_ih=(s.w_ih0, s.w_ih1)))
 
 
-def _weight_grads(cell, dims, s, dws, prec, xcd_allow=0, side=None):
+def _weight_grads(cell, dims, s, dws, prec, xcd_allow=0, side=None, bn=None):
     w, wp, wn = _ws(s.x, tag="main" if side is None else "side")
-    _lib.check(_lib.lib().ctcn_rnn_bwd_weights(cell, *dims, _ptr(s.x), _ptr(s.y), _ptr(s.gates), _ptr(s.aux), *[_ptr(d) for d in dws],
-                                               1.0, prec, xcd_allow, wp, wn, _lib.stream_ptr()), "rnn_bwd_weights")
+    if bn is None:
+        _lib.check(_lib.lib().ctcn_rnn_bwd_weights(cell, *dims, _ptr(s.x), _ptr(s.y), _ptr(s.gates), _ptr(s.aux), *[_ptr(d) for d in dws],
+                                                   1.0, prec, xcd_allow, wp, wn, _lib.stream_ptr()), "rnn_bwd_weights")
+    else:
+        call, xn = _lib.RnnCall(), torch.empty_like(s.x)
+        call.x_affine, call.x_norm = bn.struct(), xn.data_ptr()
+        _lib.check(_lib.lib().ctcn_rnn_bwd_weights_ex(cell, *dims, _ptr(s.x), _ptr(s.y), _ptr(s.gates), _ptr(s.aux), *[_ptr(d) for d in dws],
+                                                      1.0, prec, xcd_allow, wp, wn, _lib.stream_ptr(), ctypes.byref(call)), "rnn_bwd_weights_ex")
     if side is not None:
-        for t in (s.x, s.y, s.gates, s.aux):
+        for t in (s.x, s.y, s.gates, s.aux) + (bn.tensors() if bn is not None else ()):
             if t is not None:
                 t.record_stream(side)
 
 
+class _BnSpec(object):
+
+    def __init__(self, mean, rstd_or_var, gamma, beta, eps, var_is_variance):
+        self.mean, self.rstd_or_var, self.gamma, self.beta = mean, rstd_or_var, gamma, beta
+        self.eps, self.var_is_variance = float(eps), int(bool(var_is_variance))
+
+    def tensors(self):
+        return (self.mean, self.rstd_or_var, self.gamma, self.beta)
+
+    def struct(self):
+        return _lib.BnAffine(self.mean.data_ptr(), self.rstd_or_var.data_ptr(), self.gamma.data_ptr(), self.beta.data_ptr(), self.eps, self.var_is_variance)
+
+
+def bn_on_load():
+    return get_option("bn_on_load") != 0
+
+
 class _RNNLayer(torch.autograd.Function):
     @staticmethod
     def forward(ctx, x, w_ih0, w_hh0, w_ih1, w_hh1, cell, training, drop_p=0.0):
+        out, s = _RNNLayer.run_forward(ctx, x, w_ih0, w_hh0, w_ih1, w_hh1, cell, training, drop_p)
+        ctx.save_for_backward(*s)
+        return out
+
+    @staticmethod
+    def run_forward(ctx, x, w_ih0, w_hh0, w_ih1, w_hh1, cell, training, drop_p=0.0, bn=None):
         _need_gpu(x, w_ih0, w_hh0, w_ih1, w_hh1)
         ctx.gviews = [_gview(w) for w in (w_ih0, w_hh0, w_ih1, w_hh1)]
         x = _f32c(x)
@@ -470,6 +499,10 @@
             seed, off = _next_dropout_stream(y.numel())
             ctx.drop = (float(drop_p), seed, off)
             call.y_drop, call.drop_p, call.drop_seed, call.drop_offset = y_drop.data_ptr(), float(drop_p), seed, off
+        xn = None
+        if bn is not None:
+            xn = torch.empty_like(x)
+            call.x_affine, call.x_norm = bn.struct(), xn.data_ptr()
         _lib.check(L.ctcn_rnn_fwd_ex(cell, T, B, I, H, dirs, _ptr(x), _ptr(ws[0]), _ptr(ws[1]), _ptr(ws[2]), _ptr(ws[3]),
                                      _ptr(y), _ptr(gates), _ptr(aux), get_precision(), wp, wn, _lib.stream_ptr(), ctypes.byref(call)), "rnn_fwd_ex")
         _note_launch(launched.value, b"rnn_fwd_step", cell, T, B, H, dirs)
@@ -477,7 +510,7 @@
             _note_rnn_fwd(I, s, y_drop, w)
         if piped:
             torch.cuda.current_stream(dev).wait_stream(st)
-            for t in (x, gates, ws[0], ws[2]):
+            for t in (x, gates, ws[0], ws[2], xn) + (bn.tensors() if bn is not None else ()):
                 if t is not None:
                     t.record_stream(st)
         ctx.cell, ctx.dims = cell, (T, B, I, H, dirs)
@@ -486,21 +519,24 @@
         ctx.counted = any(ctx.needs_input_grad)
         if ctx.counted:
             side.live += 1
-        ctx.save_for_backward(*s)
-        return y if y_drop is None else y_drop
+        return (y if y_drop is None else y_drop), s
 
     @staticmethod
     def backward(ctx, gy):
+        dx, dws, into_flat = _RNNLayer.run_backward(ctx, gy, _Saved(*ctx.saved_tensors), ctx.needs_input_grad[0])
+        return (dx,) + ((None,) * 7 if into_flat else tuple(dws) + (None,) * 3)
+
+    @staticmethod
+    def run_backward(ctx, gy, s, need_dx, bn=None):
         if ctx.consumed:
             raise RuntimeError("ctc_pytorch_amd RNN layer: backward ran twice (the gate reserve is overwritten in place)")
         ctx.consumed = True
         dims = T, B, I, H, dirs = ctx.dims
         cell = ctx.cell
-        s = _Saved(*ctx.saved_tensors)
         wts = (s.w_ih0, s.w_hh0, s.w_ih1, s.w_hh1)
         gy = _f32c(gy)
         dev = s.x.device
-        dx = torch.empty_like(s.x) if ctx.needs_input_grad[0] else None
+        dx = torch.empty_like(s.x) if need_dx else None
         into_flat = all(g is not None for g, w in zip(ctx.gviews, wts) if w is not None)
         dws = [None if w is None else (g if into_flat else torch.empty_like(w)) for g, w in zip(ctx.gviews, wts)]
         L = _lib.lib()
@@ -521,6 +557,10 @@
             p_, seed_, off_ = ctx.drop
             gd = torch.empty_like(gy)
             call.dy_tmp, call.drop_p, call.drop_seed, call.drop_offset = gd.data_ptr(), p_, seed_, off_
+        xn = None
+        if bn is not None and mode == WG_INLINE:
+            xn = torch.empty_like(s.x)
+            call.x_affine, call.x_norm = bn.struct(), xn.data_ptr()
         prec = get_precision()
         try:
             _lib.check(L.ctcn_rnn_bwd_ex(cell, T, B, I, H, dirs, _ptr(s.x), *[_ptr(t) for t in wts], _ptr(s.y), _ptr(s.gates), _ptr(s.aux), _ptr(gy), _ptr(dx),
@@ -536,8 +576,8 @@
             st, main = side.side_stream(), torch.cuda.current_stream(dev)
             st.wait_stream(main)
             with torch.cuda.stream(st):
-                _weight_grads(cell, dims, s, [None, None] + dws[2:], prec, side=st)
-            _weight_grads(cell, dims, s, dws[:2] + [None, None], prec)
+                _weight_grads(cell, dims, s, [None, None] + dws[2:], prec, side=st, bn=bn)
+            _weight_grads(cell, dims, s, dws[:2] + [None, None], prec, bn=bn)
             if mode == WG_SPLIT_NOW:
                 main.wait_stream(st)
             else:
@@ -552,14 +592,14 @@
                 else:
                     st.wait_event(after)
                 with torch.cuda.stream(st):
-                    _weight_grads(cell, dims, s, dws, prec, allow, side=st)
+                    _weight_grads(cell, dims, s, dws, prec, allow, side=st, bn=bn)
                     if _grad_ready["hook"] is not None:
                         _grad_ready["hook"]([t for t in dws if t is not None])
                 side.pending = True
 
             side.deferred = weights_on_side_stream
             torch.autograd.Variable._execution_engine.queue_callback(side.join_at_end)
-        return (dx,) + ((None,) * 7 if into_flat else tuple(dws) + (None,) * 3)
+        return dx, dws, into_flat
 
 
 def persistent_batch_limit(H, dirs, nx, cus):
@@ -677,36 +717,175 @@
                 dgamma = dbeta = None
             return dx, dgamma, dbeta, None, None, None, None, None, None, None, None, None, None, None
         x, y, gamma, a, b = ctx.saved_tensors
+        dx, dgamma, dbeta = _bn_backward(x, y, gy, gamma, a, b, ctx.geom, ctx.gviews, ctx.sync, ctx.train_mode)
+        return dx, dgamma, dbeta, None, None, None, None, None, None, None, None, None, None, None
+
+
+def _bn_backward(x, y, gy, gamma, a, b, geom, gviews, sync, train_mode):
+    outer, C, inner, relu, eps = geom
+    gy = _f32c(gy)
+    dev = x.device
+    if not train_mode:
+        raise NotImplementedError("ctc_pytorch_amd: backward through eval-mode BatchNorm is not part of the hot path")
+    dx = torch.empty_like(x)
+    into_flat = gviews[0] is not None and gviews[1] is not None
+    if into_flat:
+        dgamma, dbeta = gviews
+    else:
+        dgamma = torch.empty(C, dtype=torch.float32, device=dev)
+        dbeta = torch.empty(C, dtype=torch.float32, device=dev)
+    w, wp, wn = _ws(x)
+    if sync is not None:
+        reducer, total = sync
+        L = _lib.lib()
+        local = torch.empty((C, 2), dtype=torch.float64, device=dev)
+        _lib.check(L.ctcn_bn_bwd_sums(_ptr(x), _ptr(y), _ptr(gy), _ptr(a), _ptr(b), _ptr(local), outer, C, inner, int(relu), wp, wn,
+                                      _lib.stream_ptr()), "bn_bwd_sums")
+        glob = local.clone()
+        reducer(glob, outer * inner)
+        _lib.check(L.ctcn_bn_bwd_finish(_ptr(x), _ptr(y), _ptr(gy), _ptr(gamma), _ptr(a), _ptr(b), _ptr(dx), _ptr(dgamma), _ptr(dbeta),
+                                        _ptr(local), _ptr(glob), total, outer, C, inner, int(relu), 1.0 if into_flat else 0.0,
+                                        wp, wn, _lib.stream_ptr()), "bn_bwd_finish")
+    else:
+        _lib.check(_lib.lib().ctcn_bn_bwd(_ptr(x), _ptr(y), _ptr(gy), _ptr(gamma), _ptr(a), _ptr(b), _ptr(dx), _ptr(dgamma),
+                                          _ptr(dbeta), outer, C, inner, int(relu), 1.0 if into_flat else 0.0, wp, wn,
+                                          _lib.stream_ptr()), "bn_bwd")
+    if into_flat:
+        dgamma = dbeta = None
+    return dx, dgamma, dbeta
+
+
+def _bn_stats_or_eval(ctx, x, gamma, beta, rm, rv, outer, C, training, momentum, eps, nbt):
+    _need_gpu(x, gamma, beta)
+    ctx.bn_gviews = (_gview(gamma), _gview(beta))
+    ctx.geom = (outer, C, 1, False, eps)
+    ctx.sync, ctx.train_mode = None, bool(training)
+    if not training:
+        return _BnSpec(rm, rv, gamma, beta, eps, 1)
+    dev, L = x.device, _lib.lib()
+    mean = torch.empty(C, dtype=torch.float32, device=dev)
+    rstd = torch.empty(C, dtype=torch.float32, device=dev)
+    w, wp, wn = _ws(x)
+    if _sync_bn["reduce"] is not None:
+        sums = torch.empty((C, 2), dtype=torch.float64, device=dev)
+        _lib.check(L.ctcn_bn_fwd_sums(_ptr(x), _ptr(sums), outer, C, 1, wp, wn, _lib.stream_ptr()), "bn_fwd_sums")
+        total = float(_sync_bn["reduce"](sums, outer))
+        _lib.check(L.ctcn_bn_fwd_stats(_ptr(x), _ptr(sums), total, _ptr(rm), _ptr(rv), _ptr(mean), _ptr(rstd), outer, C, 1, float(eps), float(momentum),
+                                       None, 0, _lib.stream_ptr(), _ptr(nbt)), "bn_fwd_stats")
+        ctx.sync = (_sync_bn["reduce"], total)
+    else:
+        _lib.check(L.ctcn_bn_fwd_stats(_ptr(x), None, 0.0, _ptr(rm), _ptr(rv), _ptr(mean), _ptr(rstd), outer, C, 1, float(eps), float(momentum),
+                                       wp, wn, _lib.stream_ptr(), _ptr(nbt)), "bn_fwd_stats")
+    return _BnSpec(mean, rstd, gamma, beta, eps, 0)
+
+
+def _nbt_for_kernel(num_batches_tracked, training):
+    if num_batches_tracked is not None and (not training or num_batches_tracked.dtype != torch.int64 or not num_batches_tracked.is_cuda):
+        if training:
+            num_batches_tracked += 1
+        return None
+    return num_batches_tracked
+
+
+class _BnRNNLayer(torch.autograd.Function):
+
+    @staticmethod
+    def forward(ctx, x, gamma, beta, rm, rv, w_ih0, w_hh0, w_ih1, w_hh1, cell, training, drop_p, bn_training, momentum, eps, nbt):
+        x = _f32c(x)
+        T, B, C = x.shape
+        bn = _bn_stats_or_eval(ctx, x, gamma, beta, rm, rv, T * B, C, bn_training, momentum, eps, nbt)
+        out, s = _RNNLayer.run_forward(ctx, x, w_ih0, w_hh0, w_ih1, w_hh1, cell, training, drop_p, bn=bn)
+        ctx.n_rnn = len(s)
+        ctx.save_for_backward(*(tuple(s) + bn.tensors()))
+        return out
+
+    @staticmethod
+    def backward(ctx, gy):
+        saved = ctx.saved_tensors
+        s = _Saved(*saved[:ctx.n_rnn])
+        mean, rstd, gamma, beta = saved[ctx.n_rnn:]
+        outer, C, inner, relu, eps = ctx.geom
+        bn = _BnSpec(mean, rstd, gamma, beta, eps, 0 if ctx.train_mode else 1)
+        need_dx = any(ctx.needs_input_grad[:3])
+        dxn, dws, into_flat = _RNNLayer.run_backward(ctx, gy, s, need_dx, bn=bn)
+        dx = dgamma = dbeta = None
+        if need_dx:
+            dx, dgamma, dbeta = _bn_backward(s.x, None, dxn, gamma, mean, rstd, ctx.geom, ctx.bn_gviews, ctx.sync, ctx.train_mode)
+        return (dx, dgamma, dbeta, None, None) + ((None,) * 4 if into_flat else tuple(dws)) + (None,) * 7
+
+
+class _BnLinear(torch.autograd.Function):
+
+    @staticmethod
+    def forward(ctx, x, gamma, beta, rm, rv, w, bn_training, momentum, eps, nbt):
+        _need_gpu(x, w)
+        ctx.gw_view = _gview(w)
+        x, w = _f32c(x), _f32c(w)
+        M, K = x.shape
+        N = w.shape[0]
+        bn = _bn_stats_or_eval(ctx, x, gamma, beta, rm, rv, M, K, bn_training, momentum, eps, nbt)
+        y = torch.empty((M, N), dtype=torch.float32, device=x.device)
+        _gemm_affine(0, 1, M, N, K, x, K, w, K, y, N, 0.0, bn_a=bn)
+        ctx.save_for_backward(x, w, *bn.tensors())
+        return y
+
+    @staticmethod
+    def backward(ctx, gy):
+        x, w, mean, rstd, gamma, beta = ctx.saved_tensors
+        outer, C, inner, relu, eps = ctx.geom
+        bn = _BnSpec(mean, rstd, gamma, beta, eps, 0 if ctx.train_mode else 1)
         gy = _f32c(gy)
-        dev = x.device
-        if not ctx.train_mode:
-            raise NotImplementedError("ctc_pytorch_amd: backward through eval-mode BatchNorm is not part of the hot path")
-        dx = torch.empty_like(x)
-        into_flat = ctx.gviews[0] is not None and ctx.gviews[1] is not None
-        if into_flat:
-            dgamma, dbeta = ctx.gviews
-        else:
-            dgamma = torch.empty(C, dtype=torch.float32, device=dev)
-            dbeta = torch.empty(C, dtype=torch.float32, device=dev)
-        w, wp, wn = _ws(x)
-        if ctx.sync is not None:
-            reducer, total = ctx.sync
-            L = _lib.lib()
-            local = torch.empty((C, 2), dtype=torch.float64, device=dev)
-            _lib.check(L.ctcn_bn_bwd_sums(_ptr(x), _ptr(y), _ptr(gy), _ptr(a), _ptr(b), _ptr(local), outer, C, inner, int(relu), wp, wn,
-                                          _lib.stream_ptr()), "bn_bwd_sums")
-            glob = local.clone()
-            reducer(glob, outer * inner)
-            _lib.check(L.ctcn_bn_bwd_finish(_ptr(x), _ptr(y), _ptr(gy), _ptr(gamma), _ptr(a), _ptr(b), _ptr(dx), _ptr(dgamma), _ptr(dbeta),
-                                            _ptr(local), _ptr(glob), total, outer, C, inner, int(relu), 1.0 if into_flat else 0.0,
-                                            wp, wn, _lib.stream_ptr()), "bn_bwd_finish")
-        else:
-            _lib.check(_lib.lib().ctcn_bn_bwd(_ptr(x), _ptr(y), _ptr(gy), _ptr(gamma), _ptr(a), _ptr(b), _ptr(dx), _ptr(dgamma),
-                                              _ptr(dbeta), outer, C, inner, int(relu), 1.0 if into_flat else 0.0, wp, wn,
-                                              _lib.stream_ptr()), "bn_bwd")
-        if into_flat:
-            dgamma = dbeta = None
-        return dx, dgamma, dbeta, None, None, None, None, None, None, None, None, None, None, None
+        M, K = x.shape
+        N = w.shape[0]
+        gxn = gw = None
+        need_dx = any(ctx.needs_input_grad[:3])
+        if need_dx:
+            gxn = torch.empty((M, K), dtype=torch.float32, device=x.device)
+            gemm(0, 0, M, K, N, gy, N, w, K, gxn, K)
+        if ctx.needs_input_grad[5]:
+            if ctx.gw_view is not None:
+                _gemm_affine(1, 0, N, K, M, gy, N, x, K, ctx.gw_view, K, 1.0, bn_b=bn)
+            else:
+                gw = torch.empty((N, K), dtype=torch.float32, device=x.device)
+                _gemm_affine(1, 0, N, K, M, gy, N, x, K, gw, K, 0.0, bn_b=bn)
+        dx = dgamma = dbeta = None
+        if need_dx:
+            dx, dgamma, dbeta = _bn_backward(x, None, gxn, gamma, mean, rstd, ctx.geom, ctx.bn_gviews, ctx.sync, ctx.train_mode)
+        return dx, dgamma, dbeta, None, None, gw, None, None, None, None
+
+
+def _gemm_affine(transA, transB, M, N, K, A, lda, Bm, ldb, C, ldc, beta, bn_a=None, bn_b=None):
+    _need_gpu(A, Bm, C)
+    w, wp, wn = _ws(C)
+    L, prec = _lib.lib(), get_precision()
+    f32 = L.ctcn_gemm_affine_f32_operands(int(transA), int(transB), M, N, K, _ptr(A), lda, _ptr(Bm), ldb, prec, wp, wn)
+    _lib.check(min(f32, 0), "gemm_affine_f32_operands")
+    sa = bn_a.struct() if bn_a is not None else None
+    sb = bn_b.struct() if bn_b is not None else None
+    ta = torch.empty_like(A) if bn_a is not None and f32 & 1 else None
+    tb = torch.empty_like(Bm) if bn_b is not None and f32 & 2 else None
+    _lib.check(L.ctcn_gemm_affine(int(transA), int(transB), M, N, K, _ptr(A), lda, _ptr(Bm), ldb, _ptr(C), ldc, float(beta), prec, wp, wn,
+                                  _lib.stream_ptr(), ctypes.byref(sa) if sa is not None else None, _ptr(ta),
+                                  ctypes.byref(sb) if sb is not None else None, _ptr(tb)), "gemm_affine")
+    return C
+
+
+def bn_rnn_layer(x, gamma, beta, running_mean, running_var, bn_training, momentum, eps, num_batches_tracked,
+                 w_ih0, w_hh0, w_ih1, w_hh1, cell, training=True, drop_p=0.0):
+    cellc = CELL[cell] if isinstance(cell, str) else cell
+    T, B, C = (int(v) for v in x.shape)
+    H, dirs = int(w_hh0.shape[1]), 2 if w_ih1 is not None else 1
+    if T > 1 and _chunks_on[0] and (cellc, H, dirs, B) in _fallback_shapes and get_option("rnn_persistent"):
+        y = batch_norm(x, gamma, beta, running_mean, running_var, T * B, C, 1, bn_training, momentum, eps, False, num_batches_tracked)
+        return rnn_layer(y, w_ih0, w_hh0, w_ih1, w_hh1, cellc, training, drop_p)
+    nbt = _nbt_for_kernel(num_batches_tracked, bn_training)
+    return _BnRNNLayer.apply(x, gamma, beta, running_mean, running_var, w_ih0, w_hh0, w_ih1, w_hh1, cellc, training, float(drop_p),
+                             bool(bn_training), momentum, eps, nbt)
+
+
+def bn_linear(x2d, gamma, beta, running_mean, running_var, bn_training, momentum, eps, num_batches_tracked, w):
+    nbt = _nbt_for_kernel(num_batches_tracked, bn_training)
+    return _BnLinear.apply(x2d, gamma, beta, running_mean, running_var, w, bool(bn_training), momentum, eps, nbt)
 
 
 def batch_norm(x, gamma, beta, running_mean, running_var, outer, C, inner, training, momentum=0.1, eps=1e-5, relu=False, num_batches_tracked=None,
diff --git a/include/ctcn.h b/include/ctcn.h
--- a/include/ctcn.h
+++ b/include/ctcn.h
@@ -31,6 +31,18 @@
 
 int ctcn_gemm(int transA, int transB, int M, int N, int K, const float *A, int lda, const float *B, int ldb,
               float *C, int ldc, float beta, int precision, void *ws, size_t ws_bytes, void *stream);
+
+typedef struct ctcn_bn_affine {
+  const float *mean, *rstd_or_var, *gamma, *beta;
+  float eps;
+  int var_is_variance;
+} ctcn_bn_affine;
+int ctcn_gemm_affine(int transA, int transB, int M, int N, int K, const float *A, int lda, const float *B, int ldb, float *C, int ldc, float beta,
+                     int precision, void *ws, size_t ws_bytes, void *stream, const ctcn_bn_affine *aff_a, float *tmp_a, const ctcn_bn_affine *aff_b,
+                     float *tmp_b);
+int ctcn_gemm_affine_f32_operands(int transA, int transB, int M, int N, int K, const float *A, int lda, const float *B, int ldb, int precision,
+                                  const void *ws, size_t ws_bytes);
+int ctcn_sizeof(int which);
 
 int ctcn_transpose01(const float *in, float *out, int A, int B, int C, void *stream);
 int ctcn_copy_strided4(const float *in, float *out, int d0, int d1, int d2, int d3, size_t s0, size_t s1, size_t s2,
@@ -67,6 +79,8 @@
   void *prelaunch_event;
   int *status;
   const char **launched;
+  ctcn_bn_affine x_affine;
+  float *x_norm;
 } ctcn_rnn_call;
 int ctcn_rnn_fwd_ex(int cell, int T, int B, int I, int H, int dirs, const float *x, const float *w_ih0, const float *w_hh0,
                     const float *w_ih1, const float *w_hh1, float *y, float *gates, float *aux, int precision, void *ws, size_t ws_bytes,
@@ -79,12 +93,19 @@
                          const float *gates, const float *aux, float *dw_ih0, float *dw_hh0, float *dw_ih1,
                          float *dw_hh1, float beta_w, int precision, unsigned xcd_allow, void *ws, size_t ws_bytes,
                          void *stream);
+int ctcn_rnn_bwd_weights_ex(int cell, int T, int B, int I, int H, int dirs, const float *x, const float *y, const float *gates,
+                            const float *aux, float *dw_ih0, float *dw_hh0, float *dw_ih1, float *dw_hh1, float beta_w, int precision,
+                            unsigned xcd_allow, void *ws, size_t ws_bytes, void *stream, const ctcn_rnn_call *call);
 
 size_t ctcn_bn_ws_bytes(int outer, int C, int inner);
 int ctcn_bn_fwd_train(const float *x, float *y, const float *gamma, const float *beta, float *running_mean,
                       float *running_var, float *save_mean, float *save_rstd, int outer, int C, int inner,
                       float eps, float momentum, int relu, void *ws, size_t ws_bytes, void *stream,
                       long long *num_batches_tracked );
+int ctcn_bn_fwd_stats(const float *x, const double *sums, double count_total, float *running_mean, float *running_var, float *save_mean,
+                      float *save_rstd, int outer, int C, int inner, float eps, float momentum, void *ws, size_t ws_bytes, void *stream,
+                      long long *num_batches_tracked);
+int ctcn_bn_apply_affine(const float *x, float *y, const ctcn_bn_affine *affine, int rows, int C, void *stream);
 int ctcn_bn_fwd_sums(const float *x, double *sums, int outer, int C, int inner, void *ws, size_t ws_bytes, void *stream);
 int ctcn_bn_fwd_finish(const float *x, float *y, const float *gamma, const float *beta, float *running_mean,
                        float *running_var, float *save_mean, float *save_rstd, const double *sums, double count_total,
```

New measurement: 1.950 million frames/s. No clear change (-0.9%).
